# rust-bio/rust-bio

Measured on NVIDIA H100. Metric: GCUPS, higher is better.
Workload: dtype int32

## Files before the change

### rust_bio_b200/csrc/b2a_common.cuh

```cuda
#pragma once
#include <stddef.h>
#include <stdint.h>

#if defined(__CUDACC__)
#define B2A_HD __host__ __device__ __forceinline__
#else
#define B2A_HD inline
struct int4 { int x, y, z, w; };
struct int2 { int x, y; };
struct uint4 { unsigned x, y, z, w; };
inline int4 make_int4(int x, int y, int z, int w) { return int4{x, y, z, w}; }
inline int2 make_int2(int x, int y) { return int2{x, y}; }
#endif

namespace b2a {

#if defined(B2A_HOST_WARP) && !defined(__CUDACC__)
struct HostWarp {
  long long x[32];
  void (*next_lane)(void*);
  void* harness;
  void (*other_warp)(void*);
};
inline HostWarp* host_warp = nullptr;
inline int host_lane = 0;
inline void host_warp_sync() { host_warp->next_lane(host_warp->harness); }
inline void host_spin_yield() {
  if (host_warp && host_warp->other_warp) host_warp->other_warp(host_warp->harness);
}
template <class Pick>
inline long long host_warp_exchange(long long mine, Pick pick) {
  host_warp->x[host_lane] = mine;
  host_warp_sync();
  const long long r = pick(host_warp->x);
  host_warp_sync();
  return r;
}
#endif

constexpr int32_t MIN_SCORE = -858993459;
constexpr int32_t DEAD_CLIP = MIN_SCORE / 2;

enum : uint32_t {
  TB_START = 0, TB_INS = 1, TB_DEL = 2, TB_SUBST = 3, TB_MATCH = 4,
  TB_XCLIP_PREFIX = 5, TB_XCLIP_SUFFIX = 6, TB_YCLIP_PREFIX = 7, TB_YCLIP_SUFFIX = 8
};

enum : uint32_t { NB_DIAG = 3, NB_INS = 2, NB_DEL = 1, NB_CLIP = 0, NB_IEXT = 4, NB_DEXT = 8 };

enum : int {
  F_TRACK_ROWS = 1,
  F_TRACK_COLS = 2,
  F_CLIPX = 4,
  F_LUT = 8,
  F_PACKTRK = 16,
  F_RELU = 32,
  F_PACKREL = 128,
  F_BND8 = 256,
  F_NOTB = 512,
  F_YSTREAM = 1024,
};
#ifndef B2A_KREL_BITS
#define B2A_KREL_BITS 12
#endif
constexpr int32_t KREL_BITS = B2A_KREL_BITS, KREL_MASK = (1 << KREL_BITS) - 1;

struct DevScoring {
  int32_t gap_open, gap_extend;
  int32_t xclip_prefix, xclip_suffix, yclip_prefix, yclip_suffix;
  int32_t match_score, mismatch_score;
  int32_t alpha;
};

struct Block {
  uint32_t first;
  uint32_t npairs;
  uint32_t maxm, maxn;
  uint32_t uniform;
  uint32_t nstrips;
  uint32_t xwords;
  uint32_t ywords;
  uint32_t K;
  uint32_t rows_pad;
  uint64_t seq_off;
  uint64_t bnd_off;
  uint64_t rows_off;
  uint64_t rowm_off;
  uint64_t tb_off;
  uint64_t ops_off;
  uint64_t strip_task_base;
};

enum { ROWS_SN = 0, ROWS_LY = 1, ROWS_SL = 2, ROWS_IL = 3, ROWS_NL = 4, ROWS_ARRAYS = 5 };

B2A_HD int64_t rows_index(int arr, int32_t rows_pad, int32_t slot) {
  return (int64_t)(arr * rows_pad) * 32 + slot;
}

B2A_HD int32_t imax(int32_t a, int32_t b) { return a > b ? a : b; }


B2A_HD int32_t col0_I(const DevScoring& sc, int32_t i) {
  if (i == 1) return sc.gap_open;
  return imax(sc.gap_open + sc.gap_extend * (i - 1), sc.xclip_prefix + sc.gap_open);
}
B2A_HD uint32_t col0_ibits(const DevScoring& sc, int32_t i) {
  if (i == 1) return TB_START;
  return (sc.gap_open + sc.gap_extend * (i - 1) > sc.xclip_prefix + sc.gap_open) ? TB_INS
                                                                                   : TB_XCLIP_PREFIX;
}
B2A_HD int32_t col0_S(const DevScoring& sc, int32_t i) {
  return imax(col0_I(sc, i), sc.xclip_prefix);
}
B2A_HD uint32_t col0_sbits(const DevScoring& sc, int32_t i) {
  return sc.xclip_prefix > col0_I(sc, i) ? TB_XCLIP_PREFIX : TB_INS;
}
B2A_HD int32_t row0_D(const DevScoring& sc, int32_t j) {
  if (j == 1) return sc.gap_open;
  return imax(sc.gap_open + sc.gap_extend * (j - 1), sc.yclip_prefix + sc.gap_open);
}
B2A_HD uint32_t row0_dbits(const DevScoring& sc, int32_t j) {
  if (j == 1) return TB_START;
  return (sc.gap_open + sc.gap_extend * (j - 1) > sc.yclip_prefix + sc.gap_open) ? TB_DEL
                                                                                   : TB_YCLIP_PREFIX;
}
B2A_HD int32_t row0_S(const DevScoring& sc, int32_t j, int32_t n) {
  int32_t s = imax(row0_D(sc, j), sc.yclip_prefix);
  if (j == n && sc.yclip_suffix > s) s = sc.yclip_suffix;
  return s;
}
B2A_HD uint32_t row0_sbits(const DevScoring& sc, int32_t j, int32_t n) {
  if (j == 0) return TB_START;
  const int32_t d = row0_D(sc, j);
  uint32_t b = d > sc.yclip_prefix ? TB_DEL : TB_YCLIP_PREFIX;
  if (j == n && sc.yclip_suffix > imax(d, sc.yclip_prefix)) b = TB_YCLIP_SUFFIX;
  return b;
}
B2A_HD int32_t xclip_score(const DevScoring& sc, int32_t j) {
  return sc.xclip_prefix + imax(sc.yclip_prefix, sc.gap_open + sc.gap_extend * (j - 1));
}

B2A_HD int64_t bnd_index(int32_t G, int32_t j, int32_t pi, int32_t maxn) {
  return G < 32 ? (int64_t)j * 32 + pi : (int64_t)pi * (maxn + 1) + j;
}

B2A_HD int32_t pack_s16x2(int32_t lo, int32_t hi) {
#if defined(__CUDA_ARCH__)
  return (int32_t)__byte_perm((uint32_t)lo, (uint32_t)hi, 0x5410);
#else
  return (int32_t)(((uint32_t)hi << 16) | ((uint32_t)lo & 0xffffu));
#endif
}
B2A_HD int32_t lo_s16(int32_t w) { return (int32_t)(int16_t)(uint16_t)((uint32_t)w & 0xffffu); }
B2A_HD int32_t hi_s16(int32_t w) { return w >> 16; }

#if defined(__CUDACC__)
__host__ __device__
#endif
constexpr int lut_entries(int alpha) { return (alpha + 1) * alpha; }
#if defined(__CUDACC__)
__host__ __device__
#endif
constexpr uint32_t lut_smem_bytes(int alpha) { return ((uint32_t)lut_entries(alpha) * 4u + 127u) & ~127u; }
constexpr int32_t LUT_POISON = 2;

#ifndef B2A_W_8_20
#define B2A_W_8_20 4
#endif
#if defined(__CUDACC__)
__host__ __device__
#endif
constexpr int fill_warps_of(int G, int R) { return (G == 8 && R == 20) ? B2A_W_8_20 : 4; }
#if defined(__CUDACC__)
__host__ __device__
#endif
constexpr bool cap_dispatch_of(int G) { return G == 8; }

#if defined(__CUDACC__)
__host__ __device__
#endif
constexpr int tbw_of(int R) { return (R + 3) / 4; }

}
```

### rust_bio_b200/csrc/b2a_engine.cu

```cuda
#include <cuda_runtime.h>

#include <chrono>
#include <cstdio>
#include <cstdlib>
#include <cstring>
#include <cub/device/device_scan.cuh>
#include <string>
#include <vector>

#define B2A_DEFINE_WALK_KERNEL
#include "../../include/b200align.h"
#include "b2a_fill_launch.h"
#include "b2a_kernels.cuh"
#include "b2a_plan.h"
#include "b2a_walk.cuh"
#include "b2a_banded.cuh"
#include "b2a_banded_strip.cuh"

using namespace b2a;

namespace {

struct DevBuf {
  void* p = nullptr;
  size_t cap = 0;
  cudaError_t reserve(size_t n) {
    if (n <= cap) return cudaSuccess;
    if (p) cudaFree(p);
    p = nullptr;
    cap = 0;
    size_t want = n + n / 8 + 256;
    cudaError_t e = cudaMalloc(&p, want);
    if (e != cudaSuccess) {
      want = n;
      e = cudaMalloc(&p, want);
    }
    if (e == cudaSuccess) cap = want;
    return e;
  }
  void release() {
    if (p) cudaFree(p);
    p = nullptr;
    cap = 0;
  }
  template <class T>
  T* as() const {
    return reinterpret_cast<T*>(p);
  }
};

const FillLaunch kFillShapes[] = {
    {1, 16, launch_fill_1_16, launch_fill_notb_1_16},
    {1, 8, launch_fill_1_8, nullptr},
    {1, 20, launch_fill_1_20, nullptr},
    {2, 16, launch_fill_2_16, nullptr},
    {2, 20, launch_fill_2_20, nullptr},
    {4, 16, launch_fill_4_16, nullptr},
    {8, 16, launch_fill_8_16, launch_fill_notb_8_16},
    {8, 20, launch_fill_8_20, launch_fill_notb_8_20},
    {32, 8, launch_fill_32_8, launch_fill_notb_32_8},
    {32, 16, launch_fill_32_16, launch_fill_notb_32_16},
};

const FillLaunch* find_shape(int G, int R) {
  for (const FillLaunch& f : kFillShapes)
    if (f.G == G && f.R == R) return &f;
  return nullptr;
}

constexpr uint32_t kMaxStageSmem = 200 * 1024;
constexpr uint64_t kWarpWalkMaxPairs = 16384;
constexpr int kMaxAlpha = 64;
constexpr int kMaxAlphaTable = 128;

}

struct b2a_engine {
  int device = 0;
  int num_sms = 0;
  cudaStream_t stream = nullptr, own_stream = nullptr;
  cudaStream_t tail_stream = nullptr;
  cudaStream_t aux_stream = nullptr;
  std::vector<cudaEvent_t> sub_ev;
  bool overlap_small = true;
  bool overlap_big = false;
  bool no_packrel = false;
  bool tail_split = true;
  bool split_timing = false;
  cudaEvent_t split_ev[5] = {nullptr, nullptr, nullptr, nullptr, nullptr};
  bool split_ran = false;
  uint32_t walk_cta_warps = 0;
  cudaEvent_t ev_fill = nullptr;
  bool tail_used = false;
  bool is_slot = false;
  bool stage_nosync = false;
  uint32_t fill_task_limit = 0;
  uint8_t* h_plan = nullptr;
  size_t h_plan_cap = 0;
  cudaStream_t res_stream() const { return tail_used ? tail_stream : stream; }
  uint64_t compact_hdr[8] = {~0ull, 0, 0, 0, 0, 0, 0, 0};
  uint64_t band_wave_lo = 0;
  std::vector<uint64_t> band_roff;
  std::vector<uint32_t> band_ylen;
  std::string err;
  int tune_G = 0, tune_R = 0;
  int walk_mode = 0;
  bool banded_fast = true;
  bool banded_strip = true;
  bool banded_strip_lastcol = true;
  uint64_t strip_pairs = 0;
  uint32_t packed_width = 0;
  std::vector<uint64_t> eff_xoff, eff_yoff;
  bool last_walk_warp = false;
  uint64_t tb_budget = 0;

  bool staged = false, ran = false;
  bool score_only = false;
  Plan plan;
  DevScoring sc{};
  int flags = 0, mode = 0;
  const FillLaunch* shape = nullptr;
  uint64_t n_pairs = 0, blob_bytes = 0;
  uint64_t h2d_bytes = 0;
  std::vector<int32_t> lut_host;
  std::vector<uint8_t> last_syms;
  uint8_t codemap_host[256];

  DevBuf d_blob, d_xoff, d_xlen, d_yoff, d_ylen, d_order, d_pm, d_pn, d_blocks, d_seq, d_bnd, d_rows,
      d_rowm, d_tb, d_opsscratch, d_lut, d_codemap, d_ctl, d_score, d_xs, d_xe, d_ys, d_ye, d_nops,
      d_opssrc, d_clip, d_status, d_nops64, d_opsoff, d_opsdense, d_scan, d_records, d_prog, d_bcells, d_bstatus,
      d_bopsend, d_bslab, d_branges, d_broff, d_bfill, d_bfoff, d_hmoff, d_hmxy, d_hpoff, d_hpidx, d_raw, d_gnops,
      d_gnops64, d_goff, d_bcols, d_bstrip, d_bsoff, d_belig;
  uint32_t* h_nops = nullptr;
  uint64_t h_nops_cap = 0;
  cudaEvent_t ev[6] = {nullptr, nullptr, nullptr, nullptr, nullptr, nullptr};
  std::vector<cudaEvent_t> wave_ev;
  uint32_t launches = 0;
  int last_grid = 0;

  int pipe_chunks = 5;
  struct PipeSlot {
    b2a_engine* eng = nullptr;
    uint64_t* h_opsoff = nullptr;
    uint32_t* h_ctl = nullptr;
    size_t h_cap = 0;
    std::vector<uint64_t> xoff, yoff;
    std::vector<uint8_t> packed;
    uint64_t lo = 0, n = 0;
    bool busy = false;
  } slots[3];
  static constexpr int kSlots = 3;

  int fail(int code, const std::string& what) {
    err = what;
    return code;
  }
  int cuda_fail(const char* what, cudaError_t e) {
    err = std::string(what) + ": " + cudaGetErrorString(e);
    return B2A_E_CUDA;
  }
};

#define CK(expr)                                              \
  do {                                                        \
    cudaError_t _e = (expr);                                  \
    if (_e != cudaSuccess) return e->cuda_fail(#expr, _e);    \
  } while (0)

namespace {

inline uint64_t bitenc_blocks(uint64_t len, uint32_t width) {
  const uint64_t usable = 32 - 32 % width;
  return (len * width + usable - 1) / usable;
}

__global__ void __launch_bounds__(128) unpack_bitenc_kernel(const uint32_t* __restrict__ blocks,
                                                             const uint64_t* __restrict__ x_block,
                                                             const uint64_t* __restrict__ y_block,
                                                             const uint64_t* __restrict__ x_off,
                                                             const uint64_t* __restrict__ y_off,
                                                             const uint32_t* __restrict__ x_len,
                                                             const uint32_t* __restrict__ y_len, uint64_t n_pairs,
                                                             uint32_t width, uint8_t* __restrict__ out) {
  const uint32_t usable = 32 - 32 % width, per_block = usable / width, mask = (1u << width) - 1u;
  const uint32_t lane = threadIdx.x & 31u;
  const uint64_t nwarps = ((uint64_t)gridDim.x * blockDim.x) >> 5;
  for (uint64_t t = ((uint64_t)blockIdx.x * blockDim.x + threadIdx.x) >> 5; t < 2 * n_pairs; t += nwarps) {
    const uint64_t p = t >> 1;
    const bool isy = t & 1;
    const uint32_t* src = blocks + (isy ? y_block[p] : x_block[p]);
    uint8_t* dst = out + (isy ? y_off[p] : x_off[p]);
    const uint32_t len = isy ? y_len[p] : x_len[p];
    for (uint32_t i = lane; i < len; i += 32) {
      const uint32_t blk = i / per_block, bit = (i % per_block) * width;
      dst[i] = (uint8_t)((src[blk] >> bit) & mask);
    }
  }
}

void choose_shape(const b2a_engine* e, uint32_t maxm, uint32_t maxn, uint64_t n_pairs, int* G, int* R) {
  if (e->tune_G && e->tune_R) {
    *G = e->tune_G;
    *R = e->tune_R;
    return;
  }
  const uint64_t stage1 = (uint64_t)((maxm + 15) / 16 * 16 + 64 + (maxn + 15) / 16 * 16 + 64) * 32 * fill_warps_of(1, 16);
  if (n_pairs >= 49152 && stage1 <= kMaxStageSmem && maxm <= 2048) {
    *G = 1;
    *R = 16;
  } else if ((n_pairs >= 4096 && maxm <= 4096) || maxm <= 161) {
    const uint64_t rows = maxm > 1 ? maxm - 1 : 1;
    const uint64_t pad16 = (rows + 127) / 128 * 128, pad20 = (rows + 159) / 160 * 160;
    *G = 8;
    *R = pad20 < pad16 ? 20 : 16;
  } else {
    *G = 32;
    const uint64_t rows = maxm > 1 ? maxm - 1 : 1;
    const uint64_t pad16 = (rows + 511) / 512 * 512, pad8 = (rows + 255) / 256 * 256;
    *R = (pad16 * 100 <= pad8 * 112) ? 16 : 8;
  }
}

int validate_scoring(b2a_engine* e, const b2a_scoring* s) {
  if (s->gap_open > 0) return e->fail(B2A_E_INVALID, "gap_open can't be positive");
  if (s->gap_extend > 0) return e->fail(B2A_E_INVALID, "gap_extend can't be positive");
  if (s->xclip_prefix > 0) return e->fail(B2A_E_INVALID, "Clipping penalty (x prefix) can't be positive");
  if (s->xclip_suffix > 0) return e->fail(B2A_E_INVALID, "Clipping penalty (x suffix) can't be positive");
  if (s->yclip_prefix > 0) return e->fail(B2A_E_INVALID, "Clipping penalty (y prefix) can't be positive");
  if (s->yclip_suffix > 0) return e->fail(B2A_E_INVALID, "Clipping penalty (y suffix) can't be positive");
  const int32_t clips[4] = {s->xclip_prefix, s->xclip_suffix, s->yclip_prefix, s->yclip_suffix};
  for (int32_t c : clips)
    if (c < B2A_MIN_SCORE) return e->fail(B2A_E_RANGE, "clip penalty below MIN_SCORE");
  return B2A_OK;
}

}

extern "C" {

const char* b2a_version(void) { return "b200align 0.1 (sm_90a)"; }

const char* b2a_last_error(const b2a_engine* e) { return e ? e->err.c_str() : "null engine"; }

int32_t b2a_engine_create(b2a_engine** out, int32_t device_id) {
  if (!out) return B2A_E_INVALID;
  *out = nullptr;
  int count = 0;
  cudaError_t ce = cudaGetDeviceCount(&count);
  if (ce != cudaSuccess || count <= 0 || device_id < 0 || device_id >= count) return B2A_E_NO_DEVICE;
  if (cudaSetDevice(device_id) != cudaSuccess) return B2A_E_NO_DEVICE;
  cudaDeviceProp prop;
  if (cudaGetDeviceProperties(&prop, device_id) != cudaSuccess) return B2A_E_NO_DEVICE;
  if (prop.major != 9 || prop.minor != 0) return B2A_E_NO_DEVICE;
  b2a_engine* e = new b2a_engine();
  e->device = device_id;
  e->num_sms = prop.multiProcessorCount;
  e->overlap_small = false;
  if (const char* env = getenv("B2A_BANDED_LITERAL")) e->banded_fast = atoi(env) == 0;
  if (const char* env = getenv("B2A_BANDED_STRIP")) e->banded_strip = atoi(env) != 0;
  if (const char* env = getenv("B2A_BANDED_STRIP_LASTCOL")) e->banded_strip_lastcol = atoi(env) != 0;
  if (const char* env = getenv("B2A_OVERLAP")) e->overlap_small = atoi(env) != 0;
  if (const char* env = getenv("B2A_OVERLAP_BIG")) e->overlap_big = atoi(env) != 0;
  if (const char* env = getenv("B2A_TAIL_SPLIT")) e->tail_split = atoi(env) != 0;
  if (const char* env = getenv("B2A_NO_PACKREL")) e->no_packrel = atoi(env) != 0;
  if (const char* env = getenv("B2A_SPLIT_TIMING")) e->split_timing = atoi(env) != 0;
  if (const char* env = getenv("B2A_WALK_CTA_WARPS")) {
    const int v = atoi(env);
    if (v == 1 || v == 2 || v == 4 || v == 8 || v == 16 || v == 32) e->walk_cta_warps = (uint32_t)v;
  }
  if (cudaStreamCreateWithFlags(&e->own_stream, cudaStreamNonBlocking) != cudaSuccess) {
    delete e;
    return B2A_E_CUDA;
  }
  e->stream = e->own_stream;
  for (auto& v : e->ev) cudaEventCreate(&v);
  *out = e;
  return B2A_OK;
}

int32_t b2a_engine_destroy(b2a_engine* e) {
  if (!e) return B2A_OK;
  cudaSetDevice(e->device);
  for (auto& sl : e->slots) {
    if (sl.h_opsoff) cudaFreeHost(sl.h_opsoff);
    if (sl.h_ctl) cudaFreeHost(sl.h_ctl);
    if (sl.eng) b2a_engine_destroy(sl.eng);
    sl.eng = nullptr;
  }
  cudaStreamSynchronize(e->stream);
  if (e->tail_stream) {
    cudaStreamSynchronize(e->tail_stream);
    cudaStreamDestroy(e->tail_stream);
  }
  if (e->ev_fill) cudaEventDestroy(e->ev_fill);
  if (e->aux_stream) {
    cudaStreamSynchronize(e->aux_stream);
    cudaStreamDestroy(e->aux_stream);
  }
  for (auto& v : e->sub_ev) cudaEventDestroy(v);
  if (e->h_plan) cudaFreeHost(e->h_plan);
  if (e->h_nops) cudaFreeHost(e->h_nops);
  DevBuf* bufs[] = {&e->d_blob, &e->d_xoff, &e->d_xlen, &e->d_yoff, &e->d_ylen, &e->d_order, &e->d_pm,
                    &e->d_pn, &e->d_blocks, &e->d_seq, &e->d_bnd, &e->d_rows, &e->d_rowm, &e->d_tb,
                    &e->d_opsscratch, &e->d_lut, &e->d_codemap, &e->d_ctl, &e->d_score, &e->d_xs,
                    &e->d_xe, &e->d_ys, &e->d_ye, &e->d_nops, &e->d_opssrc, &e->d_clip, &e->d_status,
                    &e->d_nops64, &e->d_opsoff, &e->d_opsdense, &e->d_scan, &e->d_records, &e->d_prog, &e->d_bcells,
                    &e->d_bstatus, &e->d_bopsend, &e->d_bslab, &e->d_branges, &e->d_broff, &e->d_bfill, &e->d_hmoff, &e->d_hmxy,
                    &e->d_hpoff, &e->d_hpidx, &e->d_raw, &e->d_gnops, &e->d_gnops64, &e->d_goff,
                    &e->d_bfoff, &e->d_bcols, &e->d_bstrip, &e->d_bsoff, &e->d_belig};
  for (DevBuf* b : bufs) b->release();
  for (auto& v : e->ev)
    if (v) cudaEventDestroy(v);
  for (auto& v : e->wave_ev) cudaEventDestroy(v);
  if (e->own_stream) cudaStreamDestroy(e->own_stream);
  delete e;
  return B2A_OK;
}

int32_t b2a_engine_set_stream(b2a_engine* e, void* cuda_stream) {
  if (!e) return B2A_E_INVALID;
  e->stream = cuda_stream ? reinterpret_cast<cudaStream_t>(cuda_stream) : e->own_stream;
  return B2A_OK;
}

int32_t b2a_engine_set_traceback_budget(b2a_engine* e, uint64_t bytes) {
  if (!e) return B2A_E_INVALID;
  e->tb_budget = bytes;
  return B2A_OK;
}

int32_t b2a_engine_set_pipeline(b2a_engine* e, int32_t chunks) {
  if (!e) return B2A_E_INVALID;
  e->pipe_chunks = chunks < 2 ? 0 : (chunks > 64 ? 64 : chunks);
  return B2A_OK;
}

int32_t b2a_engine_last_alphabet(const b2a_engine* e, uint8_t* symbols, uint32_t* n_symbols) {
  if (!e || !symbols || !n_symbols) return B2A_E_INVALID;
  *n_symbols = (uint32_t)e->last_syms.size();
  for (size_t k = 0; k < e->last_syms.size() && k < 256; ++k) symbols[k] = e->last_syms[k];
  return B2A_OK;
}

int32_t b2a_engine_set_walk(b2a_engine* e, int32_t mode) {
  if (!e) return B2A_E_INVALID;
  if (mode < 0 || mode > 2) return e->fail(B2A_E_INVALID, "walk mode must be 0 (automatic), 1 (lane per pair) or 2 (warp per pair)");
  e->walk_mode = mode;
  return B2A_OK;
}

int32_t b2a_engine_set_tuning(b2a_engine* e, int32_t G, int32_t R) {
  if (!e) return B2A_E_INVALID;
  if (G == 0 && R == 0) {
    e->tune_G = e->tune_R = 0;
    return B2A_OK;
  }
  if (!find_shape(G, R)) return e->fail(B2A_E_INVALID, "fill shape (G,R) not built into this library");
  e->tune_G = G;
  e->tune_R = R;
  return B2A_OK;
}

}

static int32_t stage_front(b2a_engine* e, int32_t mode, const b2a_scoring* s, const b2a_pairs* pairs,
                           uint32_t& maxm, uint32_t& maxn, int64_t& score_bound) {
  if (!e || !s || !pairs) return B2A_E_INVALID;
  e->staged = e->ran = false;
  e->score_only = false;
  if (mode < 0 || mode > 3) return e->fail(B2A_E_INVALID, "mode must be B2A_MODE_*");
  int rc = validate_scoring(e, s);
  if (rc) return rc;
  if (cudaSetDevice(e->device) != cudaSuccess) return e->fail(B2A_E_NO_DEVICE, "cudaSetDevice failed");
  if (e->stage_nosync) {
    if (cudaStreamSynchronize(e->stream) != cudaSuccess) return e->fail(B2A_E_CUDA, "cudaStreamSynchronize failed");
  }
  const uint64_t n = pairs->n_pairs;
  if (n > 0x7ffffffeull) return e->fail(B2A_E_INVALID, "more than 2^31 - 2 pairs in one batch");
  e->n_pairs = n;
  e->mode = mode;

  DevScoring sc{};
  sc.gap_open = s->gap_open;
  sc.gap_extend = s->gap_extend;
  sc.xclip_prefix = s->xclip_prefix;
  sc.xclip_suffix = s->xclip_suffix;
  sc.yclip_prefix = s->yclip_prefix;
  sc.yclip_suffix = s->yclip_suffix;
  if (mode == B2A_MODE_GLOBAL) sc.xclip_prefix = sc.xclip_suffix = sc.yclip_prefix = sc.yclip_suffix = MIN_SCORE;
  if (mode == B2A_MODE_SEMIGLOBAL) {
    sc.xclip_prefix = sc.xclip_suffix = MIN_SCORE;
    sc.yclip_prefix = sc.yclip_suffix = 0;
  }
  if (mode == B2A_MODE_LOCAL) sc.xclip_prefix = sc.xclip_suffix = sc.yclip_prefix = sc.yclip_suffix = 0;
  sc.match_score = s->match_score;
  sc.mismatch_score = s->mismatch_score;
  sc.alpha = 0;

  maxm = 0;
  maxn = 0;
  const uint32_t pw = e->packed_width;
  const uint64_t unit_total = pw ? pairs->blob_bytes / 4 : pairs->blob_bytes;
  for (uint64_t p = 0; p < n; ++p) {
    const uint64_t bb = unit_total, xo = pairs->x_off[p], yo = pairs->y_off[p];
    const uint64_t xu = pw ? bitenc_blocks(pairs->x_len[p], pw) : pairs->x_len[p];
    const uint64_t yu = pw ? bitenc_blocks(pairs->y_len[p], pw) : pairs->y_len[p];
    if (xo > bb || xu > bb - xo || yo > bb || yu > bb - yo)
      return e->fail(B2A_E_INVALID, "sequence offset/length outside seq_blob");
    maxm = std::max(maxm, pairs->x_len[p]);
    maxn = std::max(maxn, pairs->y_len[p]);
  }
  if (maxm > (1u << 24) || maxn > (1u << 24)) return e->fail(B2A_E_RANGE, "sequence longer than 2^24");

  cudaStream_t st = e->stream;
  e->blob_bytes = pairs->blob_bytes;
  e->h2d_bytes = 0;
  auto up = [&](DevBuf& bf, const void* src, size_t bytes) -> cudaError_t {
    e->h2d_bytes += bytes;
    return bytes ? cudaMemcpyAsync(bf.p, src, bytes, cudaMemcpyHostToDevice, st) : cudaSuccess;
  };
  CK(e->d_ctl.reserve(2048));
  bool present[256] = {false};
  if (pw) {
    e->eff_xoff.resize(n);
    e->eff_yoff.resize(n);
    uint64_t pos = 0;
    for (uint64_t p = 0; p < n; ++p) {
      e->eff_xoff[p] = pos;
      pos += ((uint64_t)pairs->x_len[p] + 15) & ~15ull;
      e->eff_yoff[p] = pos;
      pos += ((uint64_t)pairs->y_len[p] + 15) & ~15ull;
    }
    e->blob_bytes = pos;
    CK(e->d_raw.reserve(pairs->blob_bytes + 16));
    CK(e->d_blob.reserve(pos + 16));
    CK(e->d_xoff.reserve(n * 8 + 8));
    CK(e->d_yoff.reserve(n * 8 + 8));
    CK(e->d_xlen.reserve(n * 4 + 4));
    CK(e->d_ylen.reserve(n * 4 + 4));
    CK(e->d_opssrc.reserve(n * 8 + 8));
    CK(e->d_nops64.reserve((n + 1) * 8));
    CK(up(e->d_raw, pairs->seq_blob, pairs->blob_bytes));
    CK(up(e->d_opssrc, pairs->x_off, n * 8));
    CK(up(e->d_nops64, pairs->y_off, n * 8));
    CK(up(e->d_xoff, e->eff_xoff.data(), n * 8));
    CK(up(e->d_yoff, e->eff_yoff.data(), n * 8));
    CK(up(e->d_xlen, pairs->x_len, n * 4));
    CK(up(e->d_ylen, pairs->y_len, n * 4));
    if (n) {
      unpack_bitenc_kernel<<<(unsigned)std::min<uint64_t>((2 * n + 3) / 4, 1u << 20), 128, 0, st>>>(
          e->d_raw.as<uint32_t>(), e->d_opssrc.as<uint64_t>(), e->d_nops64.as<uint64_t>(), e->d_xoff.as<uint64_t>(),
          e->d_yoff.as<uint64_t>(), e->d_xlen.as<uint32_t>(), e->d_ylen.as<uint32_t>(), n, pw, e->d_blob.as<uint8_t>());
      CK(cudaGetLastError());
    }
    CK(cudaStreamSynchronize(st));
    if (!(s->alphabet && s->alphabet_len))
      for (uint32_t k = 0; k < (1u << pw); ++k) present[k] = true;
  } else {
    CK(e->d_blob.reserve(pairs->blob_bytes + 16));
    CK(up(e->d_blob, pairs->seq_blob, pairs->blob_bytes));
  }
  if (s->alphabet && s->alphabet_len) {
    for (uint32_t k = 0; k < s->alphabet_len; ++k) present[s->alphabet[k]] = true;
  } else if (!pw) {
    uint32_t* flags = e->d_ctl.as<uint32_t>() + 256;
    CK(cudaMemsetAsync(flags, 0, 1024, st));
    if (pairs->blob_bytes) {
      symbols_kernel<<<e->num_sms * 8, 256, 0, st>>>(e->d_blob.as<uint8_t>(), pairs->blob_bytes, flags);
      CK(cudaGetLastError());
    }
    uint32_t hflags[256];
    CK(cudaMemcpyAsync(hflags, flags, 1024, cudaMemcpyDeviceToHost, st));
    CK(cudaStreamSynchronize(st));
    for (int k = 0; k < 256; ++k) present[k] = hflags[k] != 0;
  }
  std::vector<int> syms;
  for (int k = 0; k < 256; ++k)
    if (present[k]) syms.push_back(k);
  if (syms.empty()) syms.push_back(0);
  e->last_syms.assign(syms.begin(), syms.end());
  int64_t maxabs = std::max<int64_t>(std::llabs((long long)s->match_score), std::llabs((long long)s->mismatch_score));
  for (int k = 0; k < 256; ++k) e->codemap_host[k] = (uint8_t)k;
  e->lut_host.clear();
  if (s->table && (int)syms.size() > kMaxAlphaTable)
    return e->fail(B2A_E_UNSUPPORTED, "MatchFunc table over more than 128 distinct symbols");
  if ((int)syms.size() <= (s->table ? kMaxAlphaTable : kMaxAlpha)) {
    sc.alpha = (int32_t)syms.size();
    for (int k = 0; k < 256; ++k) e->codemap_host[k] = 0xFF;
    for (int a = 0; a < sc.alpha; ++a) e->codemap_host[syms[a]] = (uint8_t)a;
    const size_t aa = (size_t)sc.alpha * sc.alpha;
    e->lut_host.resize(aa + (size_t)lut_entries(sc.alpha));
    if (s->table) maxabs = 0;
    for (int a = 0; a < sc.alpha; ++a)
      for (int b = 0; b < sc.alpha; ++b) {
        const int32_t v = s->table ? s->table[syms[a] * 256 + syms[b]]
                                   : (a == b ? s->match_score : s->mismatch_score);
        e->lut_host[(size_t)a * sc.alpha + b] = v;
        maxabs = std::max<int64_t>(maxabs, std::llabs((long long)v));
      }
    if (maxabs > (1ll << 27)) return e->fail(B2A_E_RANGE, "substitution score magnitude above 2^27");
    for (size_t k = 0; k < aa; ++k) e->lut_host[aa + k] = 4 * e->lut_host[k] + 3 - (4 * sc.gap_open + 1);
    for (size_t k = aa; k < (size_t)lut_entries(sc.alpha); ++k) e->lut_host[aa + k] = LUT_POISON;
  }
  score_bound = 0;
  {
    const int64_t unit = std::max<int64_t>(maxabs, std::max<int64_t>(-(int64_t)sc.gap_open, -(int64_t)sc.gap_extend));
    const int64_t bound = ((int64_t)maxm + maxn + 2) * unit - (int64_t)sc.gap_open;
    score_bound = bound;
    if (bound > (1ll << 27)) return e->fail(B2A_E_RANGE, "scores x lengths exceed the i32-safe range (2^27)");
    const int32_t clips[4] = {sc.xclip_prefix, sc.xclip_suffix, sc.yclip_prefix, sc.yclip_suffix};
    for (int32_t c : clips)
      if (c > DEAD_CLIP && -(int64_t)c > (1ll << 27))
        return e->fail(B2A_E_RANGE, "clip penalty between -2^27 and MIN_SCORE/2 is not supported");
  }
  e->sc = sc;
  e->flags = scoring_flags(sc, score_bound, maxm, maxn);
  if (e->no_packrel) e->flags &= ~F_PACKREL;
  if (boundary8_ok(e->flags, score_bound)) e->flags |= F_BND8;

  return B2A_OK;
}

static int32_t compact_ops(b2a_engine* e, uint64_t scratch_bytes, cudaStream_t st) {
  const uint64_t n = e->n_pairs;
  if (n) {
    if (n <= 65536) {
      scan_small_kernel<<<1, 1024, 0, st>>>(e->d_nops.as<uint32_t>(), e->d_opsoff.as<uint64_t>(), (uint32_t)n);
      CK(cudaGetLastError());
    } else {
    const unsigned g1 = (unsigned)((n + 1 + 255) / 256);
    widen_kernel<<<g1, 256, 0, st>>>(e->d_nops.as<uint32_t>(), e->d_nops64.as<uint64_t>(), n);
    CK(cudaGetLastError());
    size_t tmp = 0;
    CK(cub::DeviceScan::ExclusiveSum(nullptr, tmp, e->d_nops64.as<uint64_t>(), e->d_opsoff.as<uint64_t>(),
                                     (int64_t)(n + 1), st));
    CK(e->d_scan.reserve(tmp + 16));
    CK(cub::DeviceScan::ExclusiveSum(e->d_scan.p, tmp, e->d_nops64.as<uint64_t>(),
                                     e->d_opsoff.as<uint64_t>(), (int64_t)(n + 1), st));
    }
    CK(e->d_opsdense.reserve(scratch_bytes + 16));
    const unsigned g2 = (unsigned)((n * 32 + 255) / 256);
    gather_ops_kernel<<<g2, 256, 0, st>>>(e->d_opsscratch.as<uint8_t>(), e->d_opssrc.as<uint64_t>(),
                                          e->d_opsoff.as<uint64_t>(), e->d_opsdense.as<uint8_t>(), n);
    CK(cudaGetLastError());
    e->launches += n <= 65536 ? 2 : 4;
  }
  return B2A_OK;
}

extern "C" {

static int32_t batch_stage_impl(b2a_engine* e, int32_t mode, const b2a_scoring* s, const b2a_pairs* pairs,
                                bool score_only) {
  if (!e || !s || !pairs) return B2A_E_INVALID;
  uint32_t maxm = 0, maxn = 0;
  int64_t score_bound = 0;
  int rc = stage_front(e, mode, s, pairs, maxm, maxn, score_bound);
  if (rc) return rc;
  if (score_only) e->flags |= F_NOTB;
  const uint64_t n = e->n_pairs;
  const DevScoring sc = e->sc;
  cudaStream_t st = e->stream;
  auto up = [&](DevBuf& bf, const void* src, size_t bytes) -> cudaError_t {
    e->h2d_bytes += bytes;
    return bytes ? cudaMemcpyAsync(bf.p, src, bytes, cudaMemcpyHostToDevice, st) : cudaSuccess;
  };
  int G = 1, R = 16;
  choose_shape(e, maxm, maxn, n, &G, &R);
  uint64_t budget = e->tb_budget;
  if (!budget) {
    size_t fr = 0, tot = 0;
    CK(cudaMemGetInfo(&fr, &tot));
    budget = (uint64_t)((double)fr * 0.6);
  }
  const uint32_t lut_bytes = sc.alpha ? lut_smem_bytes(sc.alpha) : 0u;
  for (int attempt = 0;; ++attempt) {
    e->shape = find_shape(G, R);
    if (!e->shape) return e->fail(B2A_E_INVALID, "no fill kernel for the requested shape");
    build_plan(e->plan, pairs->x_len, pairs->y_len, n, G, R, budget, e->flags);
    if (64 + lut_bytes + (uint64_t)fill_warps_of(G, R) * e->plan.smem_seq_bytes <= kMaxStageSmem) break;
    if (G == 32) {
      e->flags |= F_YSTREAM;
      e->plan.smem_seq_bytes = (uint32_t)(G * R);
      break;
    }
    if ((e->tune_G && e->tune_R) || attempt > 0)
      return e->fail(B2A_E_UNSUPPORTED, "sequences too long for on-chip staging with this fill shape");
    G = 32;
    const uint64_t rows = maxm > 1 ? maxm - 1 : 1;
    const uint64_t pad16 = (rows + 511) / 512 * 512, pad8 = (rows + 255) / 256 * 256;
    R = (pad16 * 100 <= pad8 * 112) ? 16 : 8;
  }
  if (score_only && !e->shape->launch_notb)
    return e->fail(B2A_E_UNSUPPORTED, "score-only batches run only the fill shapes the automatic choice picks (1x16, 8x16, "
                                      "8x20, 32x8, 32x16); the forced shape has no score-only fill kernel");
  const Plan& pl = e->plan;
  if (!score_only && pl.G == 32 && pl.max_tb > budget)
    return e->fail(B2A_E_UNSUPPORTED, "a pair's traceback needs " + std::to_string(pl.max_tb) +
                                          " bytes, above the traceback budget of " + std::to_string(budget) +
                                          " bytes; the score-only calls (b2a_align_batch_scores, b2a_batch_stage_scores) "
                                          "align it without a traceback");

  CK(e->d_xoff.reserve(n * 8 + 8));
  CK(e->d_yoff.reserve(n * 8 + 8));
  CK(e->d_xlen.reserve(n * 4 + 4));
  CK(e->d_ylen.reserve(n * 4 + 4));
  CK(e->d_order.reserve(n * 4 + 4));
  CK(e->d_pm.reserve(n * 4 + 4));
  CK(e->d_pn.reserve(n * 4 + 4));
  CK(e->d_blocks.reserve(pl.blocks.size() * sizeof(Block) + 8));
  CK(e->d_seq.reserve(pl.seq_bytes + 16));
  CK(e->d_bnd.reserve(pl.max_bnd + 16));
  CK(e->d_rows.reserve(pl.max_rows + 16));
  CK(e->d_rowm.reserve(pl.max_rowm + 16));
  CK(e->d_tb.reserve(pl.max_tb + 16));
  CK(e->d_prog.reserve(pl.max_strip_tasks * 4 + 16));
  CK(e->d_opsscratch.reserve(pl.ops_bytes + 16));
  CK(e->d_lut.reserve(e->lut_host.size() * 4 + 16));
  CK(e->d_codemap.reserve(256));
  CK(e->d_score.reserve(n * 4 + 4));
  CK(e->d_xs.reserve(n * 4 + 4));
  CK(e->d_xe.reserve(n * 4 + 4));
  CK(e->d_ys.reserve(n * 4 + 4));
  CK(e->d_ye.reserve(n * 4 + 4));
  CK(e->d_nops.reserve(n * 4 + 4));
  CK(e->d_opssrc.reserve(n * 8 + 8));
  CK(e->d_clip.reserve(n * 16 + 16));
  CK(e->d_status.reserve(n * 4 + 4));
  CK(e->d_nops64.reserve((n + 1) * 8));
  CK(e->d_opsoff.reserve((n + 1) * 8));

  if (!e->packed_width) {
    CK(up(e->d_xoff, pairs->x_off, n * 8));
    CK(up(e->d_yoff, pairs->y_off, n * 8));
    CK(up(e->d_xlen, pairs->x_len, n * 4));
    CK(up(e->d_ylen, pairs->y_len, n * 4));
  }
  {
    const size_t blocks_bytes = pl.blocks.size() * sizeof(Block), lut_b = e->lut_host.size() * 4;
    const size_t need = 3 * n * 4 + blocks_bytes + 256 + lut_b + 64;
    if (e->h_plan_cap < need) {
      if (e->h_plan) cudaFreeHost(e->h_plan);
      e->h_plan = nullptr;
      e->h_plan_cap = 0;
      CK(cudaMallocHost(&e->h_plan, need + need / 4));
      e->h_plan_cap = need + need / 4;
    }
    size_t pos = 0;
    auto up_staged = [&](DevBuf& bf, const void* src, size_t bytes) -> cudaError_t {
      if (!bytes) return cudaSuccess;
      std::memcpy(e->h_plan + pos, src, bytes);
      const cudaError_t ce = up(bf, e->h_plan + pos, bytes);
      pos += (bytes + 15) & ~(size_t)15;
      return ce;
    };
    CK(up_staged(e->d_order, pl.order.data(), n * 4));
    CK(up_staged(e->d_pm, pl.pm.data(), n * 4));
    CK(up_staged(e->d_pn, pl.pn.data(), n * 4));
    CK(up_staged(e->d_blocks, pl.blocks.data(), blocks_bytes));
    CK(up_staged(e->d_codemap, e->codemap_host, 256));
    if (lut_b) CK(up_staged(e->d_lut, e->lut_host.data(), lut_b));
  }
  if (!e->stage_nosync) CK(cudaStreamSynchronize(st));
  e->score_only = score_only;
  e->staged = true;
  return B2A_OK;
}

int32_t b2a_batch_stage(b2a_engine* e, int32_t mode, const b2a_scoring* s, const b2a_pairs* pairs) {
  return batch_stage_impl(e, mode, s, pairs, false);
}

int32_t b2a_batch_stage_scores(b2a_engine* e, int32_t mode, const b2a_scoring* s, const b2a_pairs* pairs) {
  return batch_stage_impl(e, mode, s, pairs, true);
}

int32_t b2a_batch_run(b2a_engine* e) {
  if (!e) return B2A_E_INVALID;
  if (!e->staged) return e->fail(B2A_E_STATE, "b2a_batch_run before b2a_batch_stage");
  if (cudaSetDevice(e->device) != cudaSuccess) return e->fail(B2A_E_NO_DEVICE, "cudaSetDevice failed");
  const Plan& pl = e->plan;
  cudaStream_t st = e->stream;
  const FillLaunchFn fill = e->score_only ? e->shape->launch_notb : e->shape->launch;
  void (*const walk_warp_k)(const WalkParams) = e->score_only ? walk_warp_kernel<true> : walk_warp_kernel<false>;
  void (*const walk_lane_k)(const WalkParams) = e->score_only ? walk_kernel<true> : walk_kernel<false>;
  const bool use_tail = e->is_slot && e->tail_stream != nullptr && pl.waves.size() == 1;
  e->tail_used = use_tail;
  e->launches = 0;
  uint32_t* ctl = e->d_ctl.as<uint32_t>();
  CK(cudaMemsetAsync(ctl, 0, 256, st));
  CK(cudaEventRecord(e->ev[0], st));
  if (!pl.blocks.empty()) {
    PackParams pk{};
    pk.blocks = e->d_blocks.as<Block>();
    pk.order = e->d_order.as<uint32_t>();
    pk.blob = e->d_blob.as<uint8_t>();
    pk.x_off = e->d_xoff.as<uint64_t>();
    pk.x_len = e->d_xlen.as<uint32_t>();
    pk.y_off = e->d_yoff.as<uint64_t>();
    pk.y_len = e->d_ylen.as<uint32_t>();
    pk.codemap = e->d_codemap.as<uint8_t>();
    pk.seq = e->d_seq.as<uint8_t>();
    pk.bad_symbol = ctl;
    pk.G = pl.G;
    pack_kernel<<<(unsigned)pl.blocks.size(), 256, 0, st>>>(pk);
    CK(cudaGetLastError());
    ++e->launches;
  }
  CK(cudaEventRecord(e->ev[1], st));
  size_t wi = 0;
  for (const Wave& w : pl.waves) {
    const uint32_t nb = w.block_hi - w.block_lo;
    if (wi >= 60) return e->fail(B2A_E_UNSUPPORTED, "more than 60 traceback waves; raise the budget");
    FillParams fp{};
    fp.blocks = e->d_blocks.as<Block>() + w.block_lo;
    fp.nblocks = nb;
    fp.pm = e->d_pm.as<uint32_t>();
    fp.pn = e->d_pn.as<uint32_t>();
    fp.seq = e->d_seq.as<uint8_t>();
    fp.bnd = e->d_bnd.as<uint8_t>();
    fp.rows = e->d_rows.as<uint8_t>();
    fp.tb = e->score_only ? nullptr : e->d_tb.as<uint8_t>();
    fp.lut = e->d_lut.as<int32_t>() + (size_t)e->sc.alpha * e->sc.alpha;
    fp.task_counter = ctl + 2 + wi;
    fp.smem_seq_bytes = pl.smem_seq_bytes;
    fp.one = 1;
    fp.ge4 = 4 * e->sc.gap_extend;
    uint32_t fill_tasks = nb * (uint32_t)pl.G;
    if (pl.G == 32 && w.strip_tasks >= 0x7fffffffull) return e->fail(B2A_E_RANGE, "too many strip tasks in one wave");
    if (pl.G == 32 && w.strip_tasks > 0) {
      fp.progress = e->d_prog.as<uint32_t>();
      fp.n_strip_tasks = (uint32_t)w.strip_tasks;
      fill_tasks = fp.n_strip_tasks;
      CK(cudaMemsetAsync(fp.progress, 0, (size_t)w.strip_tasks * 4, st));
    }
    fp.sc = e->sc;
    while (e->wave_ev.size() < 3 * (wi + 1)) {
      cudaEvent_t v;
      CK(cudaEventCreate(&v));
      e->wave_ev.push_back(v);
    }
    WalkParams wp{};
    wp.blocks = fp.blocks;
    wp.nblocks = nb;
    wp.pm = fp.pm;
    wp.pn = fp.pn;
    wp.order = e->d_order.as<uint32_t>();
    wp.seq = fp.seq;
    wp.bnd = fp.bnd;
    wp.rows = fp.rows;
    wp.rowm = e->d_rowm.as<uint8_t>();
    wp.tb = fp.tb;
    wp.ops_scratch = e->d_opsscratch.as<uint8_t>();
    wp.lut = e->d_lut.as<int32_t>();
    wp.sc = e->sc;
    wp.G = pl.G;
    wp.R = pl.R;
    wp.packtrk = (e->flags & F_PACKTRK) ? 1 : 0;
    wp.bnd8 = (e->flags & F_BND8) ? 1 : 0;
    wp.filter_clips = (e->mode == B2A_MODE_SEMIGLOBAL || e->mode == B2A_MODE_LOCAL) ? 1 : 0;
    wp.score = e->d_score.as<int32_t>();
    wp.xstart = e->d_xs.as<uint32_t>();
    wp.xend = e->d_xe.as<uint32_t>();
    wp.ystart = e->d_ys.as<uint32_t>();
    wp.yend = e->d_ye.as<uint32_t>();
    wp.n_ops = e->d_nops.as<uint32_t>();
    wp.ops_src = e->d_opssrc.as<uint64_t>();
    wp.clip_len = e->d_clip.as<uint32_t>();
    wp.status = e->d_status.as<uint32_t>();
    wp.err_flag = ctl + 1;
    const bool fuse = false;
    fp.task_limit = (pl.G == 32) ? 0u : e->fill_task_limit;
    const uint64_t wave_pairs = (uint64_t)nb * 32;
    const bool warp_walk = e->walk_mode == 2 || (e->walk_mode == 0 && wave_pairs <= kWarpWalkMaxPairs);
    uint32_t per_warp_smem = 0;
    uint32_t wcta_warps = e->walk_cta_warps;
    if (warp_walk) {
      const uint32_t per_warp = ((pl.maxm + 3) / 4 + (pl.maxn + 3) / 4) * 4 + 16;
      if (!wcta_warps) wcta_warps = (uint64_t)per_warp * 8 <= 96 * 1024 ? 8u : 4u;
      per_warp_smem = (uint64_t)per_warp * wcta_warps <= 96 * 1024 ? per_warp : 0u;
      if ((size_t)per_warp_smem * wcta_warps > 48 * 1024)
        CK(cudaFuncSetAttribute(walk_warp_k, cudaFuncAttributeMaxDynamicSharedMemorySize, (int)(per_warp_smem * wcta_warps)));
    }
    if (!wcta_warps) wcta_warps = 4;
    wp.seq_smem_per_warp = per_warp_smem;
    const bool overlap_big = e->overlap_big && pl.waves.size() == 1 && !warp_walk && pl.G != 32 && nb >= 4096 && !use_tail;
    const bool overlap = overlap_big || (e->overlap_small && pl.waves.size() == 1 && warp_walk && pl.G != 32 && nb >= 64 &&
                                         !use_tail && e->walk_mode != 1);
    uint32_t split_b = 0;
    if (e->tail_split && !overlap && pl.waves.size() == 1 && warp_walk && pl.G != 32 && !use_tail && e->walk_mode != 1 &&
        fp.task_limit == 0) {
      int resident = 0;
      CK(fill(e->flags, fp, fill_tasks, e->num_sms, st, &resident, 1));
      const uint32_t slots = (uint32_t)resident, tasks = fill_tasks;
      if (slots > 0 && tasks > slots) {
        const uint32_t rounds = tasks / slots, rem = tasks % slots;
        const uint32_t a_blocks = (uint32_t)((uint64_t)rounds * slots / (uint32_t)pl.G);
        if (rem > 0 && rounds <= 6 && rem * 4 <= slots && a_blocks > 0 && a_blocks < nb) split_b = a_blocks;
      }
    }
    if (split_b) {
      if (!e->tail_stream) {
        int lo_pri = 0, hi_pri = 0;
        cudaDeviceGetStreamPriorityRange(&lo_pri, &hi_pri);
        CK(cudaStreamCreateWithPriority(&e->tail_stream, cudaStreamNonBlocking, hi_pri));
        CK(cudaEventCreateWithFlags(&e->ev_fill, cudaEventDisableTiming));
      }
      if (!e->aux_stream) CK(cudaStreamCreateWithFlags(&e->aux_stream, cudaStreamNonBlocking));
      while (e->sub_ev.size() < 6) {
        cudaEvent_t v;
        CK(cudaEventCreateWithFlags(&v, cudaEventDisableTiming));
        e->sub_ev.push_back(v);
      }
      CK(cudaEventRecord(e->wave_ev[3 * wi + 0], st));
      FillParams fa = fp, fb = fp;
      fa.nblocks = split_b;
      fb.blocks = fp.blocks + split_b;
      fb.nblocks = nb - split_b;
      fb.task_counter = ctl + 8;
      WalkParams wa = wp, wb = wp;
      wa.nblocks = split_b;
      wb.blocks = wp.blocks + split_b;
      wb.nblocks = nb - split_b;
      if (e->split_timing && !e->split_ev[0])
        for (auto& v : e->split_ev) CK(cudaEventCreate(&v));
      if (e->split_timing) CK(cudaEventRecord(e->split_ev[0], st));
      CK(fill(e->flags, fa, fa.nblocks * (uint32_t)pl.G, e->num_sms, st, &e->last_grid, 0));
      if (e->split_timing) CK(cudaEventRecord(e->split_ev[1], st));
      CK(cudaEventRecord(e->sub_ev[0], st));
      cudaStream_t sB = e->tail_stream, sA = e->aux_stream;
      CK(cudaStreamWaitEvent(sB, e->sub_ev[0], 0));
      CK(cudaStreamWaitEvent(sA, e->sub_ev[0], 0));
      CK(fill(e->flags, fb, fb.nblocks * (uint32_t)pl.G, e->num_sms, sB, nullptr, 0));
      CK(cudaEventRecord(e->wave_ev[3 * wi + 1], sB));
      if (e->split_timing) CK(cudaEventRecord(e->split_ev[2], sB));
      walk_warp_k<<<wa.nblocks * 32 / wcta_warps, wcta_warps * 32, (size_t)per_warp_smem * wcta_warps, sA>>>(wa);
      CK(cudaGetLastError());
      if (e->split_timing) CK(cudaEventRecord(e->split_ev[3], sA));
      walk_warp_k<<<wb.nblocks * 32 / wcta_warps, wcta_warps * 32, (size_t)per_warp_smem * wcta_warps, sB>>>(wb);
      CK(cudaGetLastError());
      if (e->split_timing) CK(cudaEventRecord(e->split_ev[4], sB));
      e->split_ran = true;
      e->launches += 4;
      CK(cudaEventRecord(e->sub_ev[1], e->aux_stream));
      CK(cudaEventRecord(e->sub_ev[2], e->tail_stream));
      CK(cudaStreamWaitEvent(st, e->sub_ev[1], 0));
      CK(cudaStreamWaitEvent(st, e->sub_ev[2], 0));
      e->last_walk_warp = true;
      CK(cudaEventRecord(e->wave_ev[3 * wi + 2], st));
      ++wi;
      continue;
    }
    if (overlap) {
      constexpr int kSub = 4;
      if (!e->tail_stream) {
        int lo_pri = 0, hi_pri = 0;
        cudaDeviceGetStreamPriorityRange(&lo_pri, &hi_pri);
        CK(cudaStreamCreateWithPriority(&e->tail_stream, cudaStreamNonBlocking, hi_pri));
        CK(cudaEventCreateWithFlags(&e->ev_fill, cudaEventDisableTiming));
      }
      if (!e->aux_stream) CK(cudaStreamCreateWithFlags(&e->aux_stream, cudaStreamNonBlocking));
      while (e->sub_ev.size() < kSub + 2) {
        cudaEvent_t v;
        CK(cudaEventCreateWithFlags(&v, cudaEventDisableTiming));
        e->sub_ev.push_back(v);
      }
      CK(cudaEventRecord(e->wave_ev[3 * wi + 0], st));
      CK(cudaEventRecord(e->sub_ev[kSub], st));
      CK(cudaStreamWaitEvent(e->aux_stream, e->sub_ev[kSub], 0));
      CK(cudaStreamWaitEvent(e->tail_stream, e->sub_ev[kSub], 0));
      for (int sidx = 0; sidx < kSub; ++sidx) {
        const uint32_t lo_b = (uint32_t)((uint64_t)nb * sidx / kSub), hi_b = (uint32_t)((uint64_t)nb * (sidx + 1) / kSub);
        if (hi_b <= lo_b) continue;
        cudaStream_t fs = (sidx & 1) ? e->aux_stream : st;
        FillParams f2 = fp;
        f2.blocks = fp.blocks + lo_b;
        f2.nblocks = hi_b - lo_b;
        f2.task_counter = ctl + 8 + sidx;
        f2.task_limit = 1;
        CK(fill(e->flags, f2, f2.nblocks * (uint32_t)pl.G, e->num_sms, fs, &e->last_grid, 0));
        ++e->launches;
        CK(cudaEventRecord(e->sub_ev[sidx], fs));
        CK(cudaStreamWaitEvent(e->tail_stream, e->sub_ev[sidx], 0));
        if (sidx == kSub - 1) CK(cudaEventRecord(e->wave_ev[3 * wi + 1], e->tail_stream));
        WalkParams w2 = wp;
        w2.blocks = wp.blocks + lo_b;
        w2.nblocks = hi_b - lo_b;
        if (warp_walk) walk_warp_k<<<w2.nblocks * 32 / wcta_warps, wcta_warps * 32, (size_t)per_warp_smem * wcta_warps, e->tail_stream>>>(w2);
        else walk_lane_k<<<(w2.nblocks * 32 + 127) / 128, 128, 0, e->tail_stream>>>(w2);
        CK(cudaGetLastError());
        ++e->launches;
      }
      CK(cudaEventRecord(e->sub_ev[kSub + 1], e->tail_stream));
      CK(cudaStreamWaitEvent(st, e->sub_ev[kSub + 1], 0));
      e->last_walk_warp = warp_walk;
      CK(cudaEventRecord(e->wave_ev[3 * wi + 2], st));
      ++wi;
      continue;
    }
    CK(cudaEventRecord(e->wave_ev[3 * wi + 0], st));
    CK(fill(e->flags, fp, fill_tasks, e->num_sms, st, &e->last_grid, 0));
    ++e->launches;
    CK(cudaEventRecord(e->wave_ev[3 * wi + 1], st));
    if (use_tail) {
      CK(cudaEventRecord(e->ev_fill, st));
      CK(cudaStreamWaitEvent(e->tail_stream, e->ev_fill, 0));
      st = e->tail_stream;
    }
    if (!fuse) {
      if (warp_walk) {
        walk_warp_k<<<nb * 32 / wcta_warps, wcta_warps * 32, (size_t)per_warp_smem * wcta_warps, st>>>(wp);
      } else {
        const unsigned wgrid = (nb * 32 + 127) / 128;
        walk_lane_k<<<wgrid, 128, 0, st>>>(wp);
      }
      CK(cudaGetLastError());
      ++e->launches;
      e->last_walk_warp = warp_walk;
    }
    CK(cudaEventRecord(e->wave_ev[3 * wi + 2], st));
    ++wi;
  }
  CK(cudaEventRecord(e->ev[4], st));
  if (!e->score_only) {
    int rc2 = compact_ops(e, pl.ops_bytes, st);
    if (rc2) return rc2;
  }
  CK(cudaEventRecord(e->ev[5], st));
  e->ran = true;
  return B2A_OK;
}

int32_t b2a_batch_fetch(b2a_engine* e, b2a_results* r, b2a_stats* stats) {
  if (!e) return B2A_E_INVALID;
  if (!e->ran) return e->fail(B2A_E_STATE, "b2a_batch_fetch before b2a_batch_run");
  if (e->score_only && r && (r->xstart || r->ystart || r->ops || r->ops_off || r->clip_len))
    return e->fail(B2A_E_INVALID, "a score-only batch has only score, xend, yend and status: xstart, ystart, ops, "
                                  "ops_off and clip_len must be NULL");
  if (cudaSetDevice(e->device) != cudaSuccess) return e->fail(B2A_E_NO_DEVICE, "cudaSetDevice failed");
  cudaStream_t st = e->res_stream();
  const uint64_t n = e->n_pairs;
  uint64_t d2h = 0;
  uint32_t ctl[2] = {0, 0};
  CK(cudaMemcpyAsync(ctl, e->d_ctl.p, 8, cudaMemcpyDeviceToHost, st));
  if (r && n) {
    auto down = [&](void* dst, const DevBuf& b, size_t bytes) -> cudaError_t {
      if (!dst || !bytes) return cudaSuccess;
      d2h += bytes;
      return cudaMemcpyAsync(dst, b.p, bytes, cudaMemcpyDeviceToHost, st);
    };
    CK(down(r->score, e->d_score, n * 4));
    CK(down(r->xstart, e->d_xs, n * 4));
    CK(down(r->xend, e->d_xe, n * 4));
    CK(down(r->ystart, e->d_ys, n * 4));
    CK(down(r->yend, e->d_ye, n * 4));
    CK(down(r->clip_len, e->d_clip, n * 16));
    CK(down(r->status, e->d_status, n * 4));
    uint64_t total = 0;
    if (e->score_only) {
    } else if (r->ops_off) {
      CK(down(r->ops_off, e->d_opsoff, (n + 1) * 8));
      CK(cudaStreamSynchronize(st));
      total = r->ops_off[n];
    } else {
      CK(cudaMemcpyAsync(&total, e->d_opsoff.as<uint64_t>() + n, 8, cudaMemcpyDeviceToHost, st));
      CK(cudaStreamSynchronize(st));
    }
    if (r->ops) {
      if (total > r->ops_capacity) return e->fail(B2A_E_CAPACITY, "ops buffer too small for this batch");
      CK(down(r->ops, e->d_opsdense, total));
    }
  }
  CK(cudaStreamSynchronize(st));
  if (ctl[0]) return e->fail(B2A_E_INVALID, "a sequence byte is outside the scoring alphabet");
  if (ctl[1] & 4u) return e->fail(B2A_E_INVALID, "a sequence byte is outside the scoring alphabet");
  if (!(r && r->status)) {
    if (ctl[1] & 2u) return e->fail(B2A_E_CAPACITY, "banded: more k-mer matches than the per-pair capacity");
    if (ctl[1] & 8u)
      return e->fail(B2A_E_INVALID, "banded: the reference panics on these caller-supplied matches/path (not strictly ascending, index out of range, or outside the matrix)");
    if (ctl[1]) return e->fail(B2A_E_RANGE, "traceback walk met an impossible move or never terminates (the reference panics / hangs here: mod.rs:905, banded.rs:777-831)");
  }
  if (e->split_timing && e->split_ran) {
    float a = 0, b = 0, c = 0, d = 0;
    cudaEventElapsedTime(&a, e->split_ev[0], e->split_ev[1]);
    cudaEventElapsedTime(&b, e->split_ev[1], e->split_ev[2]);
    cudaEventElapsedTime(&c, e->split_ev[1], e->split_ev[3]);
    cudaEventElapsedTime(&d, e->split_ev[1], e->split_ev[4]);
    fprintf(stderr, "[split] fill A %.1f us; after it: fill B done +%.1f, walk A done +%.1f, walk B done +%.1f us\n", a * 1e3,
            b * 1e3, c * 1e3, d * 1e3);
    e->split_ran = false;
  }
  if (stats) {
    std::memset(stats, 0, sizeof(*stats));
    stats->cells = e->plan.cells;
    stats->h2d_bytes = e->h2d_bytes;
    stats->d2h_bytes = d2h;
    stats->traceback_bytes = e->plan.total_tb;
    cudaEventElapsedTime(&stats->pack_ms, e->ev[0], e->ev[1]);
    for (size_t wv = 0; wv < e->plan.waves.size(); ++wv) {
      float a = 0.f, b = 0.f;
      cudaEventElapsedTime(&a, e->wave_ev[3 * wv + 0], e->wave_ev[3 * wv + 1]);
      cudaEventElapsedTime(&b, e->wave_ev[3 * wv + 1], e->wave_ev[3 * wv + 2]);
      stats->fill_ms += a;
      stats->walk_ms += b;
    }
    float tail = 0.f;
    cudaEventElapsedTime(&tail, e->ev[4], e->ev[5]);
    stats->walk_ms += tail;
    stats->kernel_launches = e->launches;
    stats->waves = (uint32_t)e->plan.waves.size();
    stats->fill_lanes_per_pair = (uint32_t)e->plan.G;
    stats->fill_rows_per_lane = (uint32_t)e->plan.R;
  }
  return B2A_OK;
}

static void collect_stats(b2a_engine* e, b2a_stats* stats) {
  stats->cells += e->plan.cells;
  stats->h2d_bytes += e->h2d_bytes;
  stats->traceback_bytes += e->plan.total_tb;
  float v = 0.f;
  cudaEventElapsedTime(&v, e->ev[0], e->ev[1]);
  stats->pack_ms += v;
  for (size_t wv = 0; wv < e->plan.waves.size(); ++wv) {
    float a = 0.f, b = 0.f;
    cudaEventElapsedTime(&a, e->wave_ev[3 * wv + 0], e->wave_ev[3 * wv + 1]);
    cudaEventElapsedTime(&b, e->wave_ev[3 * wv + 1], e->wave_ev[3 * wv + 2]);
    stats->fill_ms += a;
    stats->walk_ms += b;
  }
  cudaEventElapsedTime(&v, e->ev[4], e->ev[5]);
  stats->walk_ms += v;
  stats->kernel_launches += e->launches;
  stats->waves += (uint32_t)e->plan.waves.size();
  stats->fill_lanes_per_pair = (uint32_t)e->plan.G;
  stats->fill_rows_per_lane = (uint32_t)e->plan.R;
}

static int32_t slot_finish(b2a_engine* e, b2a_engine::PipeSlot& sl, b2a_results* r, uint64_t& base,
                           b2a_stats* agg) {
  b2a_engine* c = sl.eng;
  sl.busy = false;
  cudaError_t ce = cudaStreamSynchronize(c->res_stream());
  if (ce != cudaSuccess) return e->cuda_fail("pipeline: cudaStreamSynchronize", ce);
  if (sl.h_ctl[0]) return e->fail(B2A_E_INVALID, "a sequence byte is outside the scoring alphabet");
  if (sl.h_ctl[1] && !r->status) return e->fail(B2A_E_RANGE, "traceback walk met an impossible move (reference panics at mod.rs:905)");
  const uint64_t total = sl.h_opsoff[sl.n];
  if (r->ops) {
    if (base + total > r->ops_capacity) return e->fail(B2A_E_CAPACITY, "ops buffer too small for this batch");
    if (total) {
      ce = cudaMemcpyAsync(r->ops + base, c->d_opsdense.p, total, cudaMemcpyDeviceToHost, c->res_stream());
      if (ce != cudaSuccess) return e->cuda_fail("pipeline: ops D2H", ce);
      agg->d2h_bytes += total;
    }
  }
  if (r->ops_off)
    for (uint64_t i = 0; i < sl.n; ++i) r->ops_off[sl.lo + i] = base + sl.h_opsoff[i];
  base += total;
  ce = cudaStreamSynchronize(c->res_stream());
  if (ce != cudaSuccess) return e->cuda_fail("pipeline: cudaStreamSynchronize", ce);
  collect_stats(c, agg);
  return B2A_OK;
}

static int32_t align_batch_pipelined(b2a_engine* e, int32_t mode, const b2a_scoring* scoring,
                                     const b2a_pairs* pairs, b2a_results* r, b2a_stats* stats) {
  const uint64_t n = pairs->n_pairs;
  uint64_t K = (uint64_t)e->pipe_chunks;
  std::vector<double> wts(K, 6.0);
  wts[0] = 1.0;
  if (K >= 3) wts[1] = 3.0;
  wts[K - 1] = K >= 4 ? 3.0 : 2.0;
  if (K == 5) wts = {1.0, 3.0, 5.0, 5.0, 5.0};
  if (const char* env = getenv("B2A_PIPE_WEIGHTS")) {
    std::vector<double> w2;
    for (const char* q = env; *q;) {
      char* end = nullptr;
      const double v = strtod(q, &end);
      if (end == q) break;
      if (v > 0) w2.push_back(v);
      q = *end ? end + 1 : end;
    }
    if (w2.size() >= 2) {
      wts = w2;
      K = wts.size();
    }
  }
  std::vector<uint64_t> cut(K + 1, 0);
  {
    double tot = 0, acc = 0;
    for (double w : wts) tot += w;
    for (uint64_t c = 0; c < K; ++c) {
      acc += wts[c] / tot * (double)n;
      cut[c + 1] = std::min<uint64_t>(n, ((uint64_t)acc + 31) / 32 * 32);
    }
    cut[K] = n;
  }
  b2a_stats agg;
  std::memset(&agg, 0, sizeof(agg));
  uint64_t base = 0;
  int32_t rc = B2A_OK;
  std::vector<uint8_t> inferred;
  const bool dbg = getenv("B2A_DEBUG_TIMING") != nullptr;
  auto now = []() { return std::chrono::duration<double, std::milli>(std::chrono::steady_clock::now().time_since_epoch()).count(); };
  const double t00 = now();
  for (uint64_t c = 0; c < K && rc == B2A_OK; ++c) {
    const double tc0 = now();
    if (cut[c + 1] <= cut[c]) continue;
    const uint64_t lo = cut[c], hi = cut[c + 1], nc = hi - lo;
    b2a_engine::PipeSlot& sl = e->slots[c % b2a_engine::kSlots];
    if (sl.busy) {
      rc = slot_finish(e, sl, r, base, &agg);
      if (rc) break;
    }
    if (!sl.eng) {
      rc = b2a_engine_create(&sl.eng, e->device);
      if (rc) {
        e->fail(rc, "pipeline: cannot create a slot engine");
        break;
      }
    }
    if (!sl.eng->tail_stream) {
      int lo_pri = 0, hi_pri = 0;
      cudaDeviceGetStreamPriorityRange(&lo_pri, &hi_pri);
      if (cudaStreamCreateWithPriority(&sl.eng->tail_stream, cudaStreamNonBlocking, hi_pri) != cudaSuccess ||
          cudaEventCreateWithFlags(&sl.eng->ev_fill, cudaEventDisableTiming) != cudaSuccess) {
        rc = e->fail(B2A_E_CUDA, "pipeline: cannot create the slot's tail stream");
        break;
      }
    }
    sl.eng->is_slot = true;
    sl.eng->stage_nosync = true;
    sl.eng->fill_task_limit = 1;
    sl.eng->packed_width = e->packed_width;
    sl.eng->tune_G = e->tune_G;
    sl.eng->tune_R = e->tune_R;
    sl.eng->walk_mode = e->walk_mode;
    sl.eng->tb_budget = e->tb_budget;
    sl.eng->pipe_chunks = 0;
    if (sl.h_cap < nc + 1) {
      if (sl.h_opsoff) cudaFreeHost(sl.h_opsoff);
      sl.h_opsoff = nullptr;
      if (cudaMallocHost(&sl.h_opsoff, (nc + 1) * 8) != cudaSuccess) {
        rc = e->fail(B2A_E_CUDA, "pipeline: cudaMallocHost failed");
        break;
      }
      sl.h_cap = nc + 1;
    }
    if (!sl.h_ctl && cudaMallocHost(&sl.h_ctl, 64) != cudaSuccess) {
      rc = e->fail(B2A_E_CUDA, "pipeline: cudaMallocHost failed");
      break;
    }
    const uint32_t pw = e->packed_width;
    const uint64_t unit = pw ? 4 : 1;
    uint64_t bmin = ~0ull, bmax = 0, seq_sum = 0;
    bool inside = true;
    for (uint64_t p = lo; p < hi; ++p) {
      const uint64_t bb = pairs->blob_bytes / unit, xo = pairs->x_off[p], yo = pairs->y_off[p];
      const uint64_t xu = pw ? bitenc_blocks(pairs->x_len[p], pw) : pairs->x_len[p];
      const uint64_t yu = pw ? bitenc_blocks(pairs->y_len[p], pw) : pairs->y_len[p];
      if (xo > bb || xu > bb - xo || yo > bb || yu > bb - yo) {
        inside = false;
        break;
      }
      bmin = std::min(bmin, std::min(xo, yo));
      bmax = std::max(bmax, std::max(xo + xu, yo + yu));
      seq_sum += xu + yu;
    }
    if (!inside) {
      rc = e->fail(B2A_E_INVALID, "sequence offset/length outside seq_blob");
      break;
    }
    if (bmin > bmax) bmin = bmax = 0;
    sl.xoff.resize(nc);
    sl.yoff.resize(nc);
    const uint8_t* chunk_blob = pairs->seq_blob + bmin * unit;
    uint64_t chunk_bytes = (bmax - bmin) * unit;
    if (!pw && chunk_bytes > 2 * seq_sum + (1ull << 20)) {
      uint64_t pos = 0;
      sl.packed.resize(seq_sum + 32 * nc + 16);
      for (uint64_t i = 0; i < nc; ++i) {
        sl.xoff[i] = pos;
        std::memcpy(sl.packed.data() + pos, pairs->seq_blob + pairs->x_off[lo + i], pairs->x_len[lo + i]);
        pos += ((uint64_t)pairs->x_len[lo + i] + 15) & ~15ull;
        sl.yoff[i] = pos;
        std::memcpy(sl.packed.data() + pos, pairs->seq_blob + pairs->y_off[lo + i], pairs->y_len[lo + i]);
        pos += ((uint64_t)pairs->y_len[lo + i] + 15) & ~15ull;
      }
      chunk_blob = sl.packed.data();
      chunk_bytes = pos;
// ... 833 lines not shown
```

### rust_bio_b200/csrc/b2a_fill.cuh

```cuda
#pragma once
#include "b2a_common.cuh"

namespace b2a {

struct FillParams {
  const Block* blocks;
  uint32_t nblocks;
  const uint32_t* pm;
  const uint32_t* pn;
  const uint8_t* seq;
  uint8_t* bnd;
  uint8_t* rows;
  uint8_t* tb;
  const int32_t* lut;
  uint32_t* task_counter;
  uint32_t smem_seq_bytes;
  int32_t one;
  int32_t ge4;
  uint32_t* progress;
  uint32_t n_strip_tasks;
  uint32_t task_limit;
  DevScoring sc;
};

template <int G>
struct LaneCtx {
  DevScoring sc;
  const int32_t* lut;
  const uint32_t* xs;
  const uint32_t* ys;
  int32_t m, n;
  int32_t maxn;
  int32_t maxm;
  int32_t g;
  int32_t l;
  int32_t lane;
  int32_t pi;
  int32_t nstrips;
  int32_t K;
  int32_t rows_pad;
  bool uniform;
  int4* bnd;
  int32_t* rows;
  uint4* tb;
  uint32_t lut_base;
  uint32_t* prog_mine;
  uint32_t* prog_prev;
  int32_t only_strip;
  int32_t one;
  int32_t ge4;
};

#if defined(__CUDA_ARCH__)
#define B2A_SHFL_UP(v, G) __shfl_up_sync(0xffffffffu, (v), 1, (G))
#elif defined(B2A_HOST_WARP) && !defined(__CUDACC__)
inline int32_t host_shfl_up_group(int32_t v, int G) {
  if (!host_warp) return v;
  const int me = host_lane;
  return (int32_t)host_warp_exchange(v, [&](const long long* x) { return (me % G) ? x[me - 1] : x[me]; });
}
#define B2A_SHFL_UP(v, G) host_shfl_up_group((v), (G))
#define B2A_SPIN_YIELD() host_spin_yield()
#else
#define B2A_SHFL_UP(v, G) (v)
#endif
#ifndef B2A_SPIN_YIELD
#define B2A_SPIN_YIELD() ((void)0)
#endif

constexpr int32_t NEG4 = -(1 << 30);

B2A_HD int32_t max3(int32_t a, int32_t b, int32_t c) {
#if defined(__CUDA_ARCH__)
  return __vimax3_s32(a, b, c);
#else
  return imax(a, imax(b, c));
#endif
}
B2A_HD int32_t max3_relu(int32_t a, int32_t b, int32_t c) {
#if defined(__CUDA_ARCH__)
  return __vimax3_s32_relu(a, b, c);
#else
  return imax(imax(a, imax(b, c)), 0);
#endif
}
B2A_HD int32_t imin(int32_t a, int32_t b) { return a < b ? a : b; }
B2A_HD int32_t addmax(int32_t a, int32_t b, int32_t c) {
#if defined(__CUDA_ARCH__)
  return __viaddmax_s32(a, b, c);
#else
  return imax(a + b, c);
#endif
}
B2A_HD int32_t addmin(int32_t a, int32_t b, int32_t c) {
#if defined(__CUDA_ARCH__)
  return __viaddmin_s32(a, b, c);
#else
  return imin(a + b, c);
#endif
}
B2A_HD int32_t scale4(int32_t v) { return v <= DEAD_CLIP ? NEG4 : 4 * v; }

B2A_HD int32_t fmad(int32_t a, int32_t k, int32_t b) {
#if defined(__CUDA_ARCH__)
  int32_t d;
  asm("mad.lo.s32 %0, %1, %2, %3;" : "=r"(d) : "r"(a), "r"(k), "r"(b));
  return d;
#else
  return a * k + b;
#endif
}
B2A_HD int32_t lut_at(const void* host_base, uint32_t byte_addr) {
#if defined(__CUDA_ARCH__)
  int32_t v;
  asm("ld.shared.s32 %0, [%1];" : "=r"(v) : "r"(byte_addr));
  return v;
#else
  return *reinterpret_cast<const int32_t*>(reinterpret_cast<const char*>(host_base) + byte_addr);
#endif
}

B2A_HD uint32_t ld_progress(const uint32_t* p) {
#if defined(__CUDA_ARCH__)
  return *reinterpret_cast<const volatile uint32_t*>(p);
#else
  return *p;
#endif
}
template <class T>
B2A_HD T ld_boundary(const T* p, bool bypass_l1) {
#if defined(__CUDA_ARCH__)
  return bypass_l1 ? __ldcg(p) : *p;
#else
  (void)bypass_l1;
  return *p;
#endif
}
template <int G>
B2A_HD auto rows_at(int arr, int32_t rows_pad, int32_t slot) {
  if constexpr (G == 32) return rows_index(arr, rows_pad, slot);
  else return arr * rows_pad * 32 + slot;
}
#ifndef B2A_HOST_YREAD
#define B2A_HOST_YREAD(c, w) ((void)0)
#endif
template <int G>
B2A_HD uint32_t ld_yword(const LaneCtx<G>& c, int32_t w) {
  B2A_HOST_YREAD(c, w);
#if defined(__CUDA_ARCH__)
  return __ldg(c.ys + w);
#else
  return c.ys[w];
#endif
}
B2A_HD void fence_device() {
#if defined(__CUDA_ARCH__)
  __threadfence();
#endif
}

constexpr int32_t KEY_NONE = (int32_t)0x80000000;

template <int G, int R, int FLAGS, bool MASKED, bool LAST, int CAPQ>
B2A_HD void column_step(const LaneCtx<G>& c, const int32_t j, const int32_t tstep, const int32_t q, const int32_t rowbase,
                        const int32_t rv, int32_t (&Sp)[R], int32_t (&Dp)[R], int32_t (&SnR)[R],
                        int32_t (&LyR)[R], uint32_t (&tbacc)[R], const int32_t (&xc)[R],
                        int32_t sdiag, int32_t& sup, int32_t& iup, int32_t& Tv, int32_t& Ti,
                        int32_t& cap_s, int32_t& cap_i) {
  constexpr bool TR = (FLAGS & F_TRACK_ROWS) != 0;
  constexpr bool TC = (FLAGS & F_TRACK_COLS) != 0;
  constexpr bool CX = (FLAGS & F_CLIPX) != 0;
  constexpr bool LUT = (FLAGS & F_LUT) != 0;
  constexpr bool PR = (FLAGS & F_PACKREL) != 0;
  constexpr bool PK = (FLAGS & F_PACKTRK) != 0 || PR;
  constexpr bool RELU = (FLAGS & F_RELU) != 0;
  constexpr bool NOTB = (FLAGS & F_NOTB) != 0;
  constexpr bool TMASK = MASKED && !LUT;
  const int32_t go4i = 4 * c.sc.gap_open + 2, go4d = 4 * c.sc.gap_open + 1, ge4 = c.ge4;
  const int32_t ma4 = 4 * c.sc.match_score + 3 - go4d, mi4 = 4 * c.sc.mismatch_score + 3 - go4d;
  const int32_t x4 = CX ? scale4(xclip_score(c.sc, j)) : 0;
  const int32_t xs4 = scale4(c.sc.xclip_suffix), ys4 = scale4(c.sc.yclip_suffix);
  const int32_t cj = 4095 - (PR ? (tstep & KREL_MASK) : j);
  const int32_t one = c.one, k2 = one + one, k16 = k2 * 8, k1024 = k16 * 64;
  const int32_t q4 = q * 4;
  const uint32_t capbit = (MASKED && rv >= 1) ? 1u << (rv - 1) : 0u;
  int32_t Tl = KEY_NONE;
  int32_t key_even = KEY_NONE;
  int32_t sdo = fmad(sdiag, one, go4d);
  int32_t iop = fmad(sup, one, go4i);
  int32_t s4 = sup;
#pragma unroll
  for (int r = 0; r < R; ++r) {
    int32_t sub4;
    if (LUT) {
      sub4 = lut_at(c.lut, (uint32_t)fmad(q4, one, xc[r]));
    } else {
      sub4 = (xc[r] == q) ? ma4 : mi4;
    }
    const int32_t m4 = fmad(sdo, one, sub4);
    const int32_t i4 = addmax(iup, ge4, iop);
    const int32_t dop = Sp[r];
    const int32_t d4 = addmax(Dp[r], ge4, dop);
    int32_t sP;
    if (CX && RELU) {
      sP = max3_relu(m4, i4, d4);
    } else {
      sP = max3(m4, i4, d4);
      if (CX) sP = imax(sP, x4);
    }
    s4 = sP & ~3;
    const int32_t fi = addmin(i4, -iop, 4), fd = addmin(d4, -dop, 4);
    const int32_t nib = fmad(fd, k2, fi) + sP - s4;
    if (!NOTB) tbacc[r] = (uint32_t)(fmad((int32_t)tbacc[r], k16, fmad(fd, k2, fi)) + sP - s4);
    if (TC) {
      if (PK) {
        if (TMASK) {
          if (r < rv) Tl = imax(Tl, fmad(s4, k1024, 4095 - r));
        } else {
          const int32_t key = fmad(s4, k1024, 4095 - r);
          if (r & 1) Tl = max3(Tl, key_even, key);
          else key_even = key;
        }
      } else {
        const int32_t v = s4 + xs4;
        if ((!TMASK || r < rv) && v > Tv) {
          Tv = v;
          Ti = rowbase + 1 + r;
        }
      }
    }
    if (TR) {
      if (PK) {
        SnR[r] = imax(SnR[r], fmad(s4, k1024, cj));
      } else {
        const int32_t v = s4 + ys4;
        if (v > SnR[r]) {
          SnR[r] = v;
          LyR[r] = j;
        }
      }
    }
    if (LAST) {
      const int32_t slot = (rowbase + 1 + r) * 32 + c.pi;
      c.rows[rows_at<G>(ROWS_SL, c.rows_pad, slot)] = s4 >> 2;
      c.rows[rows_at<G>(ROWS_IL, c.rows_pad, slot)] = i4 >> 2;
      c.rows[rows_at<G>(ROWS_NL, c.rows_pad, slot)] = nib;
    }
    if (MASKED && (CAPQ < 0 || (r >> 2) == CAPQ)) {
      if ((capbit >> r) & 1u) {
        cap_s = s4;
        cap_i = i4;
      }
    }
    sdo = dop;
    Sp[r] = fmad(s4, one, go4d);
    iop = fmad(s4, one, go4i);
    Dp[r] = d4;
    iup = i4;
  }
  sup = s4;
  if (TC && PK) {
    if (Tl != KEY_NONE) Tv = imax(Tv, Tl - ((PR ? c.l * R : rowbase) + 1));
  }
}

template <int G, int R, int FLAGS, bool MASKED, int CAPQ>
B2A_HD void run_strip(const LaneCtx<G>& c, const int32_t s) {
  constexpr bool TR = (FLAGS & F_TRACK_ROWS) != 0;
  constexpr bool TC = (FLAGS & F_TRACK_COLS) != 0;
  constexpr bool LUT = (FLAGS & F_LUT) != 0;
  constexpr bool PR = (FLAGS & F_PACKREL) != 0;
  constexpr bool PK = (FLAGS & F_PACKTRK) != 0 || PR;
  constexpr bool B8 = (FLAGS & F_BND8) != 0;
  constexpr bool NOTB = (FLAGS & F_NOTB) != 0;
  constexpr bool YS = (FLAGS & F_YSTREAM) != 0;
  static_assert(!YS || G == 32, "F_YSTREAM is a warp-per-pair form");
  static_assert(!B8 || ((FLAGS & F_PACKTRK) != 0 && !PR), "F_BND8 needs the packed column tracker with absolute rows");
  constexpr int P = 32 / G;
  constexpr int TBW = tbw_of(R);
  int2* const bnd8 = reinterpret_cast<int2*>(c.bnd);
  const int32_t m = c.m, n = c.n;
  const int32_t rowbase = s * (G * R) + c.l * R;
  int32_t rv = m - 1 - rowbase;
  rv = rv < 0 ? 0 : (rv > R ? R : rv);
  const int32_t ys = c.sc.yclip_suffix;

  int32_t Sp[R], Dp[R], SnR[R], LyR[R], xc[R];
  uint32_t tbacc[R];
#pragma unroll
  for (int w = 0; w < R / 4; ++w) {
    const uint32_t xw = c.xs[(rowbase / 4 + w) * P + c.g];
#pragma unroll
    for (int b = 0; b < 4; ++b) {
      const int32_t sym = (int32_t)((xw >> (8 * b)) & 0xffu);
      xc[w * 4 + b] = LUT ? (int32_t)(c.lut_base + (uint32_t)(sym * c.sc.alpha * 4)) : sym;
      if (MASKED && LUT && w * 4 + b >= rv) xc[w * 4 + b] = (int32_t)(c.lut_base + (uint32_t)(c.sc.alpha * c.sc.alpha * 4));
    }
  }
#pragma unroll
  for (int r = 0; r < R; ++r) {
    const int32_t i = rowbase + 1 + r;
    const int32_t s0 = col0_S(c.sc, i);
    Sp[r] = 4 * s0 + (4 * c.sc.gap_open + 1);
    Dp[r] = NEG4;
    tbacc[r] = 0;
    LyR[r] = 0;
    if (TR) {
      if (PK) {
        SnR[r] = s0 * 4096 + 4095;
      } else {
        const int32_t v = s0 + ys;
        SnR[r] = (ys > DEAD_CLIP && v > MIN_SCORE) ? 4 * v : NEG4;
      }
    } else {
      SnR[r] = 0;
    }
  }
  int32_t sup_prev = rowbase == 0 ? 0 : 4 * col0_S(c.sc, rowbase);
  const int32_t t_none = PK ? KEY_NONE : NEG4;
  int32_t in_s = 0, in_i = NEG4, in_tv = t_none, in_ti = m;
  int32_t up_tv = NEG4, up_ti = m;
  const int32_t xs4_pr = scale4(c.sc.xclip_suffix);
  auto flush_rows = [&](const int32_t chunk, int32_t (&SnRr)[R]) {
#pragma unroll
    for (int r = 0; r < R; ++r) {
      const int32_t slot = (rowbase + 1 + r) * 32 + c.pi;
      if (SnRr[r] != KEY_NONE) {
        const int32_t sn = (SnRr[r] >> 12) + ys;
        const int32_t step = (chunk << KREL_BITS) + (4095 - (SnRr[r] & 4095));
        if (sn > c.rows[rows_at<G>(ROWS_SN, c.rows_pad, slot)]) {
          c.rows[rows_at<G>(ROWS_SN, c.rows_pad, slot)] = sn;
          c.rows[rows_at<G>(ROWS_LY, c.rows_pad, slot)] = step - c.l + 1;
        }
      }
      SnRr[r] = KEY_NONE;
    }
  };
  int4 pre = make_int4(0, 0, 0, 0);
  int2 pre8 = make_int2(0, 0);
  const bool top_from_mem = (c.l == 0) && (s > 0);
  const bool top_from_row0 = (c.l == 0) && (s == 0);
  uint32_t avail = 0;
  const bool piped = c.prog_mine != nullptr;
  auto wait_col = [&](int32_t col) {
    if (piped && c.prog_prev && (int32_t)avail < col) {
      do {
        avail = ld_progress(c.prog_prev);
        B2A_SPIN_YIELD();
      } while ((int32_t)avail < col);
      fence_device();
    }
  };
  const bool top_valid = top_from_mem && rv >= 1;
  if (top_valid && n >= 1) {
    wait_col(1);
    if (B8) pre8 = ld_boundary(&bnd8[bnd_index(G, 1, c.pi, c.maxn)], piped);
    else pre = ld_boundary(&c.bnd[bnd_index(G, 1, c.pi, c.maxn)], piped);
  }
  const bool writer =
      MASKED ? (rv >= 1 && (c.l == G - 1 || rowbase + R >= m - 1)) : (c.l == G - 1);
  int32_t cap_s = 0, cap_i = 0;
  uint32_t yw = 0;
  int32_t nyw = 0;
  uint32_t ynext = 0;
  if constexpr (YS) {
    nyw = (n + 3) >> 2;
    if (nyw > 0) ynext = ld_yword(c, 0);
  }
  uint4* tbs = NOTB ? nullptr : c.tb + (size_t)s * c.K * TBW * 32;
  const int32_t nsteps = c.K * 8;

  if (PR && TR) {
#pragma unroll
    for (int r = 0; r < R; ++r) {
      const int32_t slot = (rowbase + 1 + r) * 32 + c.pi;
      c.rows[rows_at<G>(ROWS_SN, c.rows_pad, slot)] = col0_S(c.sc, rowbase + 1 + r) + ys;
      c.rows[rows_at<G>(ROWS_LY, c.rows_pad, slot)] = 0;
      SnR[r] = KEY_NONE;
    }
  }
  for (int32_t t0 = 0; t0 < nsteps; t0 += (PR ? (1 << KREL_BITS) : nsteps)) {
  const int32_t t1 = PR ? ((t0 + (1 << KREL_BITS) < nsteps) ? t0 + (1 << KREL_BITS) : nsteps) : nsteps;
  for (int32_t t = t0; t < t1; ++t) {
    const int32_t j = t - c.l + 1;
    const bool active = (j >= 1) && (j <= n);
    if (active) {
      int32_t q;
      if (G == 1) {
        if ((t & 3) == 0) yw = c.ys[(t >> 2) * P + c.g];
        q = (int32_t)(yw & 0xffu);
        yw >>= 8;
      } else if (YS) {
        if ((j & 3) == 1) {
          yw = ynext;
          const int32_t wn = ((j - 1) >> 2) + 1;
          if (wn < nyw) ynext = ld_yword(c, wn);
        }
        q = (int32_t)(yw & 0xffu);
        yw >>= 8;
      } else {
        const int32_t jb = j - 1;
        q = (int32_t)((c.ys[(jb >> 2) * P + c.g] >> (8 * (jb & 3))) & 0xffu);
      }
      if (top_from_row0) {
        in_s = 4 * row0_S(c.sc, j, n);
        in_i = NEG4;
        in_tv = t_none;
        in_ti = m;
        if (PR) {
          up_tv = NEG4;
          up_ti = m;
        }
      } else if (top_from_mem) {
        if (B8) {
          in_s = lo_s16(pre8.x);
          in_i = hi_s16(pre8.x);
          if (TC) in_tv = fmad(pre8.y, c.one, 0);
        } else {
          in_s = pre.x;
          in_i = pre.y;
        }
        if (TC && !B8) {
          if (PR) {
            up_tv = pre.z;
            up_ti = pre.w;
            in_tv = KEY_NONE;
          } else {
            in_tv = pre.z;
            in_ti = pre.w;
          }
        }
        if (j < n && top_valid) {
          wait_col(j + 1);
          if (B8) pre8 = ld_boundary(&bnd8[bnd_index(G, j + 1, c.pi, c.maxn)], piped);
          else pre = ld_boundary(&c.bnd[bnd_index(G, j + 1, c.pi, c.maxn)], piped);
        }
      }
      int32_t sup = in_s, iup = in_i, Tv = in_tv, Ti = in_ti;
      if (j == n) {
        column_step<G, R, FLAGS, MASKED, true, CAPQ>(c, j, t, q, rowbase, rv, Sp, Dp, SnR, LyR, tbacc, xc,
                                               sup_prev, sup, iup, Tv, Ti, cap_s, cap_i);
      } else {
        column_step<G, R, FLAGS, MASKED, false, CAPQ>(c, j, t, q, rowbase, rv, Sp, Dp, SnR, LyR, tbacc, xc,
                                                sup_prev, sup, iup, Tv, Ti, cap_s, cap_i);
      }
      sup_prev = in_s;
      if (writer) {
        if (B8) {
          const int32_t s4 = (MASKED && rv < R) ? cap_s : sup, i4 = (MASKED && rv < R) ? cap_i : iup;
          bnd8[bnd_index(G, j, c.pi, c.maxn)] = make_int2(pack_s16x2(s4, i4), TC ? Tv : t_none);
        } else {
          int4 o;
          o.x = (MASKED && rv < R) ? cap_s : sup;
          o.y = (MASKED && rv < R) ? cap_i : iup;
          o.z = TC ? Tv : t_none;
          o.w = TC ? Ti : m;
          if (PR) {
            o.z = NEG4;
            o.w = m;
            if (TC) {
              o.z = up_tv;
              o.w = up_ti;
              if (Tv != KEY_NONE) {
                const int32_t loc_v = ((Tv >> 12) << 2) + xs4_pr;
                if (loc_v > up_tv) {
                  o.z = loc_v;
                  o.w = s * (G * R) + (4095 - (Tv & 4095));
                }
              }
            }
          }
          c.bnd[bnd_index(G, j, c.pi, c.maxn)] = o;
        }
        if (piped && ((j & 15) == 0 || j == n)) {
          fence_device();
          *reinterpret_cast<volatile uint32_t*>(c.prog_mine) = (uint32_t)j;
          B2A_SPIN_YIELD();
        }
      }
      in_s = sup;
      in_i = iup;
      in_tv = Tv;
      in_ti = Ti;
    } else if (!NOTB) {
#pragma unroll
      for (int r = 0; r < R; ++r) tbacc[r] <<= 4;
    }
    if (G > 1) {
      in_s = B2A_SHFL_UP(in_s, G);
      in_i = B2A_SHFL_UP(in_i, G);
      if (TC) {
        in_tv = B2A_SHFL_UP(in_tv, G);
        if (!PK) in_ti = B2A_SHFL_UP(in_ti, G);
        if (PR) {
          up_tv = B2A_SHFL_UP(up_tv, G);
          up_ti = B2A_SHFL_UP(up_ti, G);
        }
      }
    }
    if (!NOTB && (t & 7) == 7) {
      uint4* dst = tbs + (size_t)(t >> 3) * TBW * 32 + c.lane;
#pragma unroll
      for (int qd = 0; qd < TBW; ++qd) {
        uint4 v;
        v.x = tbacc[qd * 4 + 0];
        v.y = (qd * 4 + 1 < R) ? tbacc[qd * 4 + 1] : 0u;
        v.z = (qd * 4 + 2 < R) ? tbacc[qd * 4 + 2] : 0u;
        v.w = (qd * 4 + 3 < R) ? tbacc[qd * 4 + 3] : 0u;
        dst[qd * 32] = v;
      }
    }
  }
  if (PR && TR) flush_rows(t0 >> KREL_BITS, SnR);
  }
  if (TR && !PR) {
#pragma unroll
    for (int r = 0; r < R; ++r) {
      const int32_t slot = (rowbase + 1 + r) * 32 + c.pi;
      int32_t sn, ly;
      if (PK) {
        sn = (SnR[r] >> 12) + ys;
        ly = 4095 - (SnR[r] & 4095);
      } else {
        sn = (SnR[r] <= NEG4 / 2) ? MIN_SCORE : (SnR[r] >> 2);
        ly = LyR[r];
      }
      c.rows[rows_at<G>(ROWS_SN, c.rows_pad, slot)] = sn;
      c.rows[rows_at<G>(ROWS_LY, c.rows_pad, slot)] = ly;
    }
  }
}

template <int G, int R, int FLAGS>
B2A_HD void fill_lane(const LaneCtx<G>& c) {
  if (G == 32 && c.m == 0) return;
  const int32_t s_lo = c.only_strip >= 0 ? c.only_strip : 0;
  const int32_t s_hi = c.only_strip >= 0 ? c.only_strip + 1 : c.nstrips;
  for (int32_t s = s_lo; s < s_hi; ++s) {
    const bool full = c.uniform && ((s + 1) * (G * R) <= c.maxm - 1);
    if (full) {
      run_strip<G, R, FLAGS, false, -1>(c, s);
    } else if (cap_dispatch_of(G) && c.uniform) {
      const int32_t left = c.maxm - 1 - s * (G * R);
      const int32_t part = (left > 0 && left < G * R) ? left % R : 0;
      switch (part ? (part - 1) >> 2 : R / 4) {
        case 0: run_strip<G, R, FLAGS, true, 0>(c, s); break;
        case 1: run_strip<G, R, FLAGS, true, (1 <= R / 4 ? 1 : -1)>(c, s); break;
        case 2: run_strip<G, R, FLAGS, true, (2 <= R / 4 ? 2 : -1)>(c, s); break;
        case 3: run_strip<G, R, FLAGS, true, (3 <= R / 4 ? 3 : -1)>(c, s); break;
        case 4: run_strip<G, R, FLAGS, true, (4 <= R / 4 ? 4 : -1)>(c, s); break;
        case 5: run_strip<G, R, FLAGS, true, (5 <= R / 4 ? 5 : -1)>(c, s); break;
        default: run_strip<G, R, FLAGS, true, -1>(c, s); break;
      }
    } else {
      run_strip<G, R, FLAGS, true, -1>(c, s);
    }
  }
}

#if defined(__CUDACC__)

__device__ __forceinline__ uint32_t smem_u32(const void* p) {
  return (uint32_t)__cvta_generic_to_shared(p);
}
__device__ __forceinline__ void mbar_init(uint64_t* bar, uint32_t count) {
  asm volatile("mbarrier.init.shared::cta.b64 [%0], %1;" ::"r"(smem_u32(bar)), "r"(count));
}
__device__ __forceinline__ void mbar_expect_tx(uint64_t* bar, uint32_t bytes) {
  asm volatile("mbarrier.arrive.expect_tx.shared::cta.b64 _, [%0], %1;" ::"r"(smem_u32(bar)),
               "r"(bytes)
               : "memory");
}
__device__ __forceinline__ void tma_bulk_g2s(void* dst_smem, const void* src_gmem, uint32_t bytes,
                                             uint64_t* bar) {
  asm volatile(
      "cp.async.bulk.shared::cluster.global.mbarrier::complete_tx::bytes [%0], [%1], %2, [%3];" ::"r"(
          smem_u32(dst_smem)),
      "l"(src_gmem), "r"(bytes), "r"(smem_u32(bar))
      : "memory");
}
__device__ __forceinline__ bool mbar_try_wait(uint64_t* bar, uint32_t parity) {
  uint32_t done;
  asm volatile(
      "{\n\t.reg .pred p;\n\t"
      "mbarrier.try_wait.parity.shared::cta.b64 p, [%1], %2;\n\t"
      "selp.b32 %0, 1, 0, p;\n\t}"
      : "=r"(done)
      : "r"(smem_u32(bar)), "r"(parity)
      : "memory");
  return done != 0;
}

#ifndef B2A_MINB
#define B2A_MINB 1
#endif

template <int G, int R, int FLAGS>
__global__ void __launch_bounds__(fill_warps_of(G, R) * 32, B2A_MINB) fill_kernel(const FillParams prm) {
  extern __shared__ __align__(128) uint8_t smem[];
  constexpr int P = 32 / G;
  constexpr int FILL_WARPS = fill_warps_of(G, R);
  constexpr bool LUT = (FLAGS & F_LUT) != 0;
  constexpr int TBW = tbw_of(R);
  const int warp = threadIdx.x >> 5, lane = threadIdx.x & 31;
  uint64_t* bars = reinterpret_cast<uint64_t*>(smem);
  int32_t* lut_s = reinterpret_cast<int32_t*>(smem + 64);
  const uint32_t lut_bytes = LUT ? lut_smem_bytes(prm.sc.alpha) : 0u;
  uint8_t* stage = smem + 64 + lut_bytes + (size_t)warp * prm.smem_seq_bytes;
  uint64_t* bar = &bars[warp];
  if (threadIdx.x < FILL_WARPS) mbar_init(&bars[threadIdx.x], 1);
  if (LUT) {
    for (int k = threadIdx.x; k < lut_entries(prm.sc.alpha); k += blockDim.x) lut_s[k] = prm.lut[k];
  }
  asm volatile("fence.mbarrier_init.release.cluster;" ::: "memory");
  __syncthreads();

  const bool strip_tasks = (G == 32) && prm.progress != nullptr;
  const uint32_t ntasks = strip_tasks ? prm.n_strip_tasks : prm.nblocks * G;
  uint32_t parity = 0;

  for (uint32_t done = 0; prm.task_limit == 0 || done < prm.task_limit; ++done) {
    uint32_t task = 0;
    if (lane == 0) task = atomicAdd(prm.task_counter, 1u);
    task = __shfl_sync(0xffffffffu, task, 0);
    if (task >= ntasks) break;
    uint32_t b, sub;
    int32_t only_strip = -1;
    if (strip_tasks) {
      uint32_t lo = 0, hi = prm.nblocks;
      while (hi - lo > 1) {
        const uint32_t mid = (lo + hi) / 2;
        if (prm.blocks[mid].strip_task_base <= task) lo = mid;
        else hi = mid;
      }
      b = lo;
      const uint32_t rel = task - (uint32_t)prm.blocks[b].strip_task_base;
      const uint32_t ns = prm.blocks[b].nstrips;
      sub = rel / ns;
      only_strip = (int32_t)(rel % ns);
    } else {
      b = task / G;
      sub = task % G;
    }
    const Block blk = prm.blocks[b];
    if (strip_tasks && sub >= blk.npairs) continue;
    const uint32_t xbytes = blk.xwords * P * 4, ybytes = blk.ywords * P * 4;
    const uint32_t xoff = strip_tasks ? (uint32_t)only_strip * G * R : 0u;
    const uint32_t xstage = strip_tasks ? (uint32_t)(G * R) : xbytes;
    constexpr bool YS = (FLAGS & F_YSTREAM) != 0;
    if (lane == 0) {
      asm volatile("fence.proxy.async.shared::cta;" ::: "memory");
      mbar_expect_tx(bar, xstage + (YS ? 0u : ybytes));
      const uint8_t* src = prm.seq + blk.seq_off;
      tma_bulk_g2s(stage, src + (size_t)sub * xbytes + xoff, xstage, bar);
      if (!YS) tma_bulk_g2s(stage + xstage, src + (size_t)G * xbytes + (size_t)sub * ybytes, ybytes, bar);
    }
    LaneCtx<G> c;
    c.sc = prm.sc;
    c.lut = lut_s;
    c.lut_base = smem_u32(lut_s);
    c.one = prm.one;
    c.ge4 = prm.ge4;
    c.only_strip = only_strip;
    c.prog_mine = strip_tasks ? prm.progress + task : nullptr;
    c.prog_prev = (strip_tasks && only_strip > 0) ? prm.progress + task - 1 : nullptr;
    c.xs = reinterpret_cast<const uint32_t*>(stage) - xoff / 4;
    c.ys = YS ? reinterpret_cast<const uint32_t*>(prm.seq + blk.seq_off + (size_t)G * xbytes + (size_t)sub * ybytes)
              : reinterpret_cast<const uint32_t*>(stage + xstage);
    c.g = lane / G;
    c.l = lane % G;
    c.lane = lane;
    c.pi = (int32_t)(sub * P) + c.g;
    const bool valid = (uint32_t)c.pi < blk.npairs;
    c.m = valid ? (int32_t)prm.pm[blk.first + c.pi] : 0;
    c.n = valid ? (int32_t)prm.pn[blk.first + c.pi] : 0;
    c.maxn = (int32_t)blk.maxn;
    c.maxm = (int32_t)blk.maxm;
    c.nstrips = (int32_t)blk.nstrips;
    c.K = (int32_t)blk.K;
    c.rows_pad = (int32_t)blk.rows_pad;
    c.uniform = blk.uniform != 0;
    c.bnd = reinterpret_cast<int4*>(prm.bnd + blk.bnd_off);
    c.rows = reinterpret_cast<int32_t*>(prm.rows + blk.rows_off);
    c.tb = (FLAGS & F_NOTB) ? nullptr
                            : reinterpret_cast<uint4*>(prm.tb + blk.tb_off) + (size_t)sub * blk.nstrips * blk.K * TBW * 32;
    while (!mbar_try_wait(bar, parity)) {
    }
    parity ^= 1u;
    fill_lane<G, R, FLAGS>(c);
    __syncwarp();
  }
}

#endif

}
```

### rust_bio_b200/csrc/b2a_fill_inst.cu

```cuda
#include "b2a_fill_launch.h"

#ifndef B2A_G
#error "compile with -DB2A_G=... -DB2A_R=..."
#endif

#ifdef B2A_NOTB
#define B2A_LAUNCH_NAME launch_fill_notb_
#else
#define B2A_LAUNCH_NAME launch_fill_
#endif

namespace b2a {

namespace {

template <int FLAGS>
cudaError_t go(const FillParams& prm, uint32_t ntasks, int num_sms, cudaStream_t stream,
               int* grid_out, int dry) {
  auto kern = fill_kernel<B2A_G, B2A_R, FLAGS>;
  constexpr int FILL_WARPS = fill_warps_of(B2A_G, B2A_R);
  const uint32_t lut_bytes = (FLAGS & F_LUT) ? lut_smem_bytes(prm.sc.alpha) : 0u;
  const size_t smem = 64 + lut_bytes + (size_t)FILL_WARPS * prm.smem_seq_bytes;
  cudaError_t err =
      cudaFuncSetAttribute(kern, cudaFuncAttributeMaxDynamicSharedMemorySize, (int)smem);
  if (err != cudaSuccess) return err;
  int per_sm = 0;
  err = cudaOccupancyMaxActiveBlocksPerMultiprocessor(&per_sm, kern, FILL_WARPS * 32, smem);
  if (err != cudaSuccess) return err;
  if (per_sm < 1) return cudaErrorLaunchOutOfResources;
  if (dry) {
    if (grid_out) *grid_out = num_sms * per_sm * FILL_WARPS;
    return cudaSuccess;
  }
  const uint32_t want = (ntasks + FILL_WARPS - 1) / FILL_WARPS;
  uint32_t grid = (uint32_t)(num_sms * per_sm);
  if (grid > want) grid = want;
  if (prm.task_limit) grid = (want + prm.task_limit - 1) / prm.task_limit;
  if (grid < 1) grid = 1;
  if (grid_out) *grid_out = (int)grid;
  kern<<<grid, FILL_WARPS * 32, smem, stream>>>(prm);
  return cudaGetLastError();
}

}

#define B2A_CAT2(a, b, c) a##b##_##c
#define B2A_CAT(a, b, c) B2A_CAT2(a, b, c)

cudaError_t B2A_CAT(B2A_LAUNCH_NAME, B2A_G, B2A_R)(int flags, const FillParams& prm, uint32_t ntasks,
                                                   int num_sms, cudaStream_t stream, int* grid_out, int dry) {
  constexpr int ALL = F_TRACK_ROWS | F_TRACK_COLS | F_CLIPX;
#ifdef B2A_NOTB
  constexpr int NOTB = F_NOTB;
#else
  constexpr int NOTB = 0;
#endif
#if B2A_G == 32
#define B2A_CASE(F)                                                                    \
  case (NOTB | (F)): return go<(NOTB | (F))>(prm, ntasks, num_sms, stream, grid_out, dry); \
  case (NOTB | F_YSTREAM | (F)): return go<(NOTB | F_YSTREAM | (F))>(prm, ntasks, num_sms, stream, grid_out, dry);
#else
#define B2A_CASE(F) \
  case (NOTB | (F)): return go<(NOTB | (F))>(prm, ntasks, num_sms, stream, grid_out, dry);
#endif
  switch (flags) {
    B2A_CASE(0)
    B2A_CASE(F_TRACK_ROWS)
    B2A_CASE(F_TRACK_ROWS | F_PACKTRK)
    B2A_CASE(ALL)
    B2A_CASE(ALL | F_PACKTRK)
    B2A_CASE(ALL | F_RELU)
    B2A_CASE(ALL | F_PACKTRK | F_RELU)
    B2A_CASE(F_LUT)
    B2A_CASE(F_LUT | F_TRACK_ROWS)
    B2A_CASE(F_LUT | F_TRACK_ROWS | F_PACKTRK)
    B2A_CASE(F_LUT | ALL)
    B2A_CASE(F_LUT | ALL | F_PACKTRK)
    B2A_CASE(F_LUT | ALL | F_RELU)
    B2A_CASE(F_LUT | ALL | F_PACKTRK | F_RELU)
    B2A_CASE(F_TRACK_ROWS | F_PACKTRK | F_BND8)
    B2A_CASE(ALL | F_PACKTRK | F_BND8)
    B2A_CASE(ALL | F_PACKTRK | F_RELU | F_BND8)
    B2A_CASE(F_LUT | F_TRACK_ROWS | F_PACKTRK | F_BND8)
    B2A_CASE(F_LUT | ALL | F_PACKTRK | F_BND8)
    B2A_CASE(F_LUT | ALL | F_PACKTRK | F_RELU | F_BND8)
    B2A_CASE(F_TRACK_ROWS | F_PACKREL)
    B2A_CASE(ALL | F_PACKREL)
    B2A_CASE(ALL | F_PACKREL | F_RELU)
    B2A_CASE(F_LUT | F_TRACK_ROWS | F_PACKREL)
    B2A_CASE(F_LUT | ALL | F_PACKREL)
    B2A_CASE(F_LUT | ALL | F_PACKREL | F_RELU)
    default: return cudaErrorInvalidValue;
  }
}

}
```

### rust_bio_b200/csrc/b2a_plan.h

```cpp
#pragma once
#include <algorithm>
#include <cstdint>
#include <numeric>
#include <vector>

#include "b2a_common.cuh"

namespace b2a {

struct Wave {
  uint32_t block_lo, block_hi;
  uint64_t bnd_bytes, rows_bytes, rowm_bytes, tb_bytes;
  uint64_t strip_tasks;
};

struct Plan {
  int G = 1, R = 16;
  uint64_t n_pairs = 0;
  std::vector<uint32_t> order;
  std::vector<uint32_t> pm, pn;
  std::vector<Block> blocks;
  std::vector<Wave> waves;
  uint64_t seq_bytes = 0, ops_bytes = 0;
  uint64_t max_bnd = 0, max_rows = 0, max_rowm = 0, max_tb = 0;
  uint64_t max_strip_tasks = 0;
  uint64_t total_tb = 0;
  uint64_t cells = 0;
  uint32_t smem_seq_bytes = 0;
  uint32_t maxm = 0, maxn = 0;
};

inline uint64_t align_up(uint64_t v, uint64_t a) { return (v + a - 1) / a * a; }

inline void build_plan(Plan& p, const uint32_t* x_len, const uint32_t* y_len, uint64_t n_pairs, int G,
                       int R, uint64_t tb_budget, int flags = 0) {
  const uint64_t bnd_rec = (flags & F_BND8) ? 8 : 16;
  const bool notb = (flags & F_NOTB) != 0;
  p.G = G;
  p.R = R;
  p.n_pairs = n_pairs;
  p.order.resize(n_pairs);
  std::iota(p.order.begin(), p.order.end(), 0u);
  bool uniform_all = true;
  for (uint64_t i = 1; i < n_pairs && uniform_all; ++i)
    uniform_all = (x_len[i] == x_len[0]) && (y_len[i] == y_len[0]);
  if (!uniform_all) {
    std::stable_sort(p.order.begin(), p.order.end(), [&](uint32_t a, uint32_t b) {
      if (x_len[a] != x_len[b]) return x_len[a] > x_len[b];
      return y_len[a] > y_len[b];
    });
  }
  p.pm.resize(n_pairs);
  p.pn.resize(n_pairs);
  p.cells = 0;
  for (uint64_t i = 0; i < n_pairs; ++i) {
    p.pm[i] = x_len[p.order[i]];
    p.pn[i] = y_len[p.order[i]];
    p.cells += (uint64_t)p.pm[i] * p.pn[i];
  }
  const int P = 32 / G, TBW = tbw_of(R);
  auto task_tb = [&](uint32_t maxm, uint32_t maxn) -> uint64_t {
    const uint64_t nstrips = maxm >= 2 ? (maxm - 1 + G * R - 1) / (G * R) : 0;
    const uint64_t K = maxn ? (maxn + G - 1 + 7) / 8 : 0;
    return nstrips * K * TBW * 512;
  };
  const bool per_pair = G == 32 && !notb;
  p.blocks.clear();
  for (uint64_t first = 0; first < n_pairs;) {
    uint32_t q = 0, mm = 0, mn = 0;
    while (q < 32 && first + q < n_pairs) {
      const uint32_t m2 = std::max(mm, p.pm[first + q]), n2 = std::max(mn, p.pn[first + q]);
      if (per_pair && q > 0 && (uint64_t)(q + 1) * task_tb(m2, n2) > tb_budget) break;
      mm = m2;
      mn = n2;
      ++q;
    }
    Block k{};
    k.first = (uint32_t)first;
    k.npairs = q;
    p.blocks.push_back(k);
    first += q;
  }
  const uint32_t nblocks = (uint32_t)p.blocks.size();
  p.waves.clear();
  p.seq_bytes = p.ops_bytes = 0;
  p.max_bnd = p.max_rows = p.max_rowm = p.max_tb = 0;
  p.max_strip_tasks = 0;
  p.total_tb = 0;
  p.smem_seq_bytes = 0;
  p.maxm = p.maxn = 0;
  Wave w{0, 0, 0, 0, 0, 0, 0};
  for (uint32_t b = 0; b < nblocks; ++b) {
    Block& k = p.blocks[b];
    k.maxm = k.maxn = 0;
    for (uint32_t q = 0; q < k.npairs; ++q) {
      k.maxm = std::max(k.maxm, p.pm[k.first + q]);
      k.maxn = std::max(k.maxn, p.pn[k.first + q]);
    }
    k.uniform = 1;
    for (uint32_t q = 0; q < k.npairs; ++q)
      if (p.pm[k.first + q] != k.maxm || p.pn[k.first + q] != k.maxn) k.uniform = 0;
    k.nstrips = k.maxm >= 2 ? (k.maxm - 1 + G * R - 1) / (G * R) : 0;
    const uint32_t xw = std::max<uint32_t>((k.maxm + 3) / 4, k.nstrips * G * R / 4);
    k.xwords = (uint32_t)align_up(std::max<uint32_t>(xw, 4), 4);
    k.ywords = (uint32_t)align_up(std::max<uint32_t>((k.maxn + 3) / 4, 4), 4);
    k.K = k.maxn ? (k.maxn + G - 1 + 7) / 8 : 0;
    k.rows_pad = k.nstrips * G * R + 2;
    p.maxm = std::max(p.maxm, k.maxm);
    p.maxn = std::max(p.maxn, k.maxn);
    const uint32_t stage_x = G == 32 ? (uint32_t)(G * R) : k.xwords * P * 4;
    p.smem_seq_bytes = std::max<uint32_t>(p.smem_seq_bytes, stage_x + k.ywords * P * 4);
    const uint64_t bnd = align_up((uint64_t)(k.maxn + 1) * 32 * bnd_rec, 256);
    const uint64_t rows = align_up((uint64_t)ROWS_ARRAYS * k.rows_pad * 32 * 4, 256);
    const uint64_t rowm = align_up((uint64_t)(k.maxn + 1) * 32 * 2, 256);
    const uint32_t tasks = G == 32 ? k.npairs : (uint32_t)G;
    const uint64_t tb = notb ? 0 : align_up((uint64_t)tasks * k.nstrips * k.K * TBW * 512, 256);
    const bool full = notb ? w.bnd_bytes + w.rows_bytes + w.rowm_bytes + bnd + rows + rowm > tb_budget
                           : w.tb_bytes + tb > tb_budget;
    if (b > w.block_lo && full) {
      w.block_hi = b;
      p.waves.push_back(w);
      w = Wave{b, b, 0, 0, 0, 0, 0};
    }
    k.seq_off = p.seq_bytes;
    p.seq_bytes += align_up((uint64_t)32 * (k.xwords + k.ywords) * 4, 256);
    k.ops_off = p.ops_bytes;
    p.ops_bytes += align_up((uint64_t)32 * (k.maxm + k.maxn + 4), 256);
    k.strip_task_base = w.strip_tasks;
    w.strip_tasks += (uint64_t)(G == 32 ? k.npairs : 32) * k.nstrips;
    k.bnd_off = w.bnd_bytes;
    k.rows_off = w.rows_bytes;
    k.rowm_off = w.rowm_bytes;
    k.tb_off = w.tb_bytes;
    w.bnd_bytes += bnd;
    w.rows_bytes += rows;
    w.rowm_bytes += rowm;
    w.tb_bytes += tb;
    if (!notb) p.total_tb += (uint64_t)tasks * k.nstrips * k.K * TBW * 512;
  }
  if (nblocks) {
    w.block_hi = nblocks;
    p.waves.push_back(w);
  }
  for (const Wave& v : p.waves) {
    p.max_bnd = std::max(p.max_bnd, v.bnd_bytes);
    p.max_rows = std::max(p.max_rows, v.rows_bytes);
    p.max_rowm = std::max(p.max_rowm, v.rowm_bytes);
    p.max_tb = std::max(p.max_tb, v.tb_bytes);
    p.max_strip_tasks = std::max(p.max_strip_tasks, v.strip_tasks);
  }
}

inline int scoring_flags(const DevScoring& sc, int64_t score_bound = (1ll << 40), uint32_t maxm = ~0u,
                         uint32_t maxn = ~0u) {
  const bool xp = sc.xclip_prefix > DEAD_CLIP, xs = sc.xclip_suffix > DEAD_CLIP;
  const bool yp = sc.yclip_prefix > DEAD_CLIP, ys = sc.yclip_suffix > DEAD_CLIP;
  int f = 0;
  if (xs || (xp && yp)) {
    f = F_TRACK_ROWS | F_TRACK_COLS | F_CLIPX;
  } else if (ys) {
    f = F_TRACK_ROWS;
  }
  if (sc.alpha) f |= F_LUT;
  if ((f & F_CLIPX) && sc.xclip_prefix == 0 && sc.yclip_prefix == 0) f |= F_RELU;
  if ((f & (F_TRACK_ROWS | F_TRACK_COLS)) && score_bound < (1ll << 17) && maxm <= 4095 && maxn <= 4095)
    f |= F_PACKTRK;
  else if ((f & (F_TRACK_ROWS | F_TRACK_COLS)) && score_bound < (1ll << 18))
    f |= F_PACKREL;
  return f;
}

inline bool boundary8_ok(int flags, int64_t score_bound) {
  return (flags & F_PACKTRK) != 0 && 4 * score_bound + 3 < (1ll << 15);
}

inline bool banded_strip_gate(const DevScoring& sc, int64_t score_bound, uint32_t maxm) {
  const bool xs_dead = sc.xclip_suffix <= DEAD_CLIP, ys_dead = sc.yclip_suffix <= DEAD_CLIP;
  const bool yp_live = sc.yclip_prefix > DEAD_CLIP;
  const bool trackers_ok = (xs_dead && ys_dead) || (yp_live && score_bound < (1ll << 17) && (xs_dead || maxm <= 4095));
  return score_bound < (1ll << 26) && trackers_ok;
}

}
```

### rust_bio_b200/csrc/b2a_walk.cuh

```cuda
#pragma once
#include "b2a_common.cuh"
#include "b2a_coop.cuh"

namespace b2a {

struct WalkParams {
  const Block* blocks;
  uint32_t nblocks;
  const uint32_t* pm;
  const uint32_t* pn;
  const uint32_t* order;
  const uint8_t* seq;
  const uint8_t* bnd;
  uint8_t* rows;
  uint8_t* rowm;
  const uint8_t* tb;
  uint8_t* ops_scratch;
  const int32_t* lut;
  DevScoring sc;
  int32_t G, R;
  int32_t filter_clips;
  int32_t packtrk;
  int32_t bnd8;
  uint32_t seq_smem_per_warp;
  int32_t* score;
  uint32_t* xstart;
  uint32_t* xend;
  uint32_t* ystart;
  uint32_t* yend;
  uint32_t* n_ops;
  uint64_t* ops_src;
  uint32_t* clip_len;
  uint32_t* status;
  uint32_t* err_flag;
};

constexpr uint32_t LAZY = 15;

template <class T>
B2A_HD T ldg_ro(const T* p) {
#if defined(__CUDA_ARCH__)
  return __ldg(p);
#else
  return *p;
#endif
}

struct PairView {
  DevScoring sc;
  const int32_t* lut;
  const uint32_t* xw;
  const uint32_t* yw;
  int32_t P;
  int32_t m, n, pi;
  int32_t G, R, TBW, nstrips, K;
  const int4* bnd;
  int32_t* rows;
  int32_t rows_pad;
  uint16_t* rowm;
  const uint32_t* tb;
  int32_t sub, g;
  int32_t packtrk;
  int32_t bnd8 = 0;
  int32_t maxn;
  int64_t bnd_base;
  int32_t bnd_stride;
  const uint8_t* xs8 = nullptr;
  const uint8_t* ys8 = nullptr;
  uint64_t mulR = 0, mulGR = 0;
  B2A_HD void set_shape(int32_t G_, int32_t R_) {
    G = G_;
    R = R_;
    TBW = (R_ + 3) / 4;
    mulR = ((1ull << 40) + (uint64_t)R_ - 1) / (uint64_t)R_;
    mulGR = ((1ull << 40) + (uint64_t)(G_ * R_) - 1) / (uint64_t)(G_ * R_);
  }

  B2A_HD int32_t xsym(int32_t i) const {
    const int32_t b = i - 1;
    if (xs8) return (int32_t)xs8[b];
    return (int32_t)((xw[(b >> 2) * P] >> (8 * (b & 3))) & 0xffu);
  }
  B2A_HD int32_t ysym(int32_t j) const {
    const int32_t b = j - 1;
    if (ys8) return (int32_t)ys8[b];
    return (int32_t)((yw[(b >> 2) * P] >> (8 * (b & 3))) & 0xffu);
  }
  B2A_HD int32_t score(int32_t p, int32_t q) const {
    if (sc.alpha) return lut[p * sc.alpha + q];
    return p == q ? sc.match_score : sc.mismatch_score;
  }
  B2A_HD int32_t& row(int arr, int32_t i) const { return rows[rows_index(arr, rows_pad, i * 32 + pi)]; }
  B2A_HD int4 load_bnd(int32_t j) const {
    const int64_t k = bnd_base + (int64_t)j * bnd_stride;
    if (bnd8) {
      const int2 r = ldg_ro(&reinterpret_cast<const int2*>(bnd)[k]);
      return make_int4(r.x, r.y, 0, 0);
    }
    return ldg_ro(&bnd[k]);
  }
  B2A_HD uint32_t nib(int32_t i, int32_t j) const {
    const int32_t GR = G * R;
    const int32_t s = (int32_t)(((uint64_t)(uint32_t)(i - 1) * mulGR) >> 40), rem = (i - 1) - s * GR;
    const int32_t l = (int32_t)(((uint64_t)(uint32_t)rem * mulR) >> 40), r = rem - l * R;
    const int32_t lane = g * G + l;
    const int32_t t = (j - 1) + l;
    const size_t word =
        ((((size_t)(sub * nstrips + s) * K + (t >> 3)) * TBW + (r >> 2)) * 32 + lane) * 4 + (r & 3);
    return (tb[word] >> (4 * (7 - (t & 7)))) & 15u;
  }
  B2A_HD uint32_t nib_scode(uint32_t nb, int32_t i, int32_t j) const {
    switch (nb & 3u) {
      case NB_DIAG: return xsym(i) == ysym(j) ? TB_MATCH : TB_SUBST;
      case NB_INS: return TB_INS;
      case NB_DEL: return TB_DEL;
      default: return TB_XCLIP_PREFIX;
    }
  }
};

struct Boundary {
  int32_t S, I, Tv, Ti;
};
B2A_HD Boundary decode_boundary(const int4 b, const bool packtrk, const bool bnd8, const int32_t xs, const int32_t m) {
  Boundary o;
  o.S = (bnd8 ? lo_s16(b.x) : b.x) >> 2;
  o.I = (bnd8 ? hi_s16(b.x) : b.y) >> 2;
  o.Tv = MIN_SCORE;
  o.Ti = m;
  const int32_t key = bnd8 ? b.y : b.z;
  if (packtrk) {
    if (key != (int32_t)0x80000000) {
      o.Tv = (key >> 12) + xs;
      o.Ti = 4095 - (key & 4095);
    }
  } else if (b.z > -(1 << 29)) {
    o.Tv = b.z >> 2;
    o.Ti = b.w;
  }
  return o;
}

B2A_HD uint32_t cell_make(uint32_t i, uint32_t d, uint32_t s) { return i | (d << 4) | (s << 8); }
B2A_HD uint32_t cell_i(uint32_t c) { return c & 15u; }
B2A_HD uint32_t cell_d(uint32_t c) { return (c >> 4) & 15u; }
B2A_HD uint32_t cell_s(uint32_t c) { return (c >> 8) & 15u; }
B2A_HD uint32_t cell_set_s(uint32_t c, uint32_t s) { return (c & ~0xF00u) | (s << 8); }
B2A_HD uint32_t cell_set_i(uint32_t c, uint32_t i) { return (c & ~0x00Fu) | i; }

struct WalkOut {
  int32_t score;
  uint32_t xstart, xend, ystart, yend, n_ops, status;
  uint32_t clip[4];
};

struct EndState {
  int32_t SmN, ImN;
  uint32_t cmN;
  int32_t Snm, Lym;
  int32_t Lx0, LxN;
};

B2A_HD void finish_matrix_seq(const PairView& v, EndState& es) {
  const DevScoring& sc = v.sc;
  const int32_t m = v.m, n = v.n;
  const int32_t go = sc.gap_open, ge = sc.gap_extend;
  const int32_t xp = sc.xclip_prefix, xs = sc.xclip_suffix, yp = sc.yclip_prefix,
                ys = sc.yclip_suffix;

  int32_t SmN = 0, ImN = MIN_SCORE;
  uint32_t cmN = 0;
  int32_t Snm = MIN_SCORE, Lym = 0;
  int32_t Lx0 = 0, LxN = 0;
  if (m >= 1) {
    int32_t T = MIN_SCORE;
    for (int32_t i = 1; i < m; ++i) {
      const int32_t val = col0_S(sc, i) + xs;
      if (val > T) {
        T = val;
        Lx0 = m - i;
      }
    }
    int32_t Im = col0_I(sc, m);
    uint32_t ib = col0_ibits(sc, m);
    int32_t Sm = T;
    uint32_t sb = TB_XCLIP_SUFFIX;
    if (Im > Sm) {
      Sm = Im;
      sb = TB_INS;
    }
    if (xp > Sm) {
      Sm = xp;
      sb = TB_XCLIP_PREFIX;
    }
    if (Sm + ys > Snm) {
      Snm = Sm + ys;
      Lym = n;
    }
    int32_t Dm = MIN_SCORE;
    uint32_t cell = cell_make(ib, TB_START, sb);
    v.rowm[0 * 32 + v.pi] = (uint16_t)cell;
    LxN = Lx0;
    const int32_t p = v.xsym(m);
    const int32_t yclip_score = yp + go + ge * (m - 1);
    int32_t sdiag = (m == 1) ? 0 : col0_S(sc, m - 1);
    constexpr int UB = 4;
    for (int32_t j0 = 1; j0 <= n; j0 += UB) {
      int4 braw[UB];
      int32_t qv[UB];
#pragma unroll
      for (int u = 0; u < UB; ++u) {
        const int32_t jj = j0 + u;
        braw[u] = make_int4(0, 0, 0, 0);
        qv[u] = 0;
        if (jj <= n) {
          if (m != 1) braw[u] = v.load_bnd(jj);
          qv[u] = v.ysym(jj);
        }
      }
#pragma unroll
      for (int u = 0; u < UB; ++u) {
      const int32_t j = j0 + u;
      if (j > n) break;
      int32_t sup, iup, Tv, Ti;
      if (m == 1) {
        sup = row0_S(sc, j, n);
        iup = MIN_SCORE;
        Tv = MIN_SCORE;
        Ti = m;
      } else {
        const Boundary b = decode_boundary(braw[u], v.packtrk != 0, v.bnd8 != 0, xs, m);
        sup = b.S;
        iup = b.I;
        Tv = b.Tv;
        Ti = b.Ti;
      }
      const int32_t q = qv[u];
      const int32_t m_score = sdiag + v.score(p, q);
      int32_t best_i, best_d;
      {
        const int32_t i_score = iup + ge, s_score = sup + go;
        if (i_score > s_score) {
          best_i = i_score;
          ib = TB_INS;
        } else {
          best_i = s_score;
          ib = LAZY;
        }
      }
      uint32_t db;
      {
        const int32_t d_score = Dm + ge, s_score = Sm + go;
        if (d_score > s_score) {
          best_d = d_score;
          db = TB_DEL;
        } else {
          best_d = s_score;
          db = sb;
        }
      }
      int32_t best = Tv;
      sb = TB_XCLIP_SUFFIX;
      if (m_score > best) {
        best = m_score;
        sb = (p == q) ? TB_MATCH : TB_SUBST;
      }
      if (best_i > best) {
        best = best_i;
        sb = TB_INS;
      }
      if (best_d > best) {
        best = best_d;
        sb = TB_DEL;
      }
      const int32_t xcs = xclip_score(sc, j);
      if (xcs > best) {
        best = xcs;
        sb = TB_XCLIP_PREFIX;
      }
      if (yclip_score > best) {
        best = yclip_score;
        sb = TB_YCLIP_PREFIX;
      }
      Sm = best;
      Im = best_i;
      Dm = best_d;
      if (Sm + ys > Snm) {
        Snm = Sm + ys;
        Lym = n - j;
      }
      if (j == n) {
        LxN = m - Ti;
        if (ib == LAZY) {
          ib = (m == 1) ? row0_sbits(sc, n, n)
                        : v.nib_scode((uint32_t)v.row(ROWS_NL, m - 1), m - 1, n);
        }
      }
      cell = cell_make(ib, db, sb);
      v.rowm[j * 32 + v.pi] = (uint16_t)cell;
      sdiag = sup;
          }
    }
    SmN = Sm;
    ImN = Im;
    cmN = cell;
  }

  const bool ys_live = ys > DEAD_CLIP;
  {
    int32_t s0, c0;
    if (n == 0) {
      s0 = 0;
      c0 = (int32_t)cell_make(TB_START, TB_START, TB_START);
    } else {
      s0 = row0_S(sc, n, n);
      c0 = (int32_t)cell_make(TB_START, row0_dbits(sc, n), row0_sbits(sc, n, n));
    }
    if (m == 0) {
      SmN = s0;
      cmN = (uint32_t)c0;
      Snm = ys;
      Lym = n;
    } else {
      uint32_t s_above = cell_s((uint32_t)c0);
      {
        int32_t S = s0;
        uint32_t cell = (uint32_t)c0;
        if (ys > S) {
          S = ys;
          cell = cell_set_s(cell, TB_YCLIP_SUFFIX);
        }
        v.row(ROWS_SL, 0) = S;
        v.row(ROWS_IL, 0) = MIN_SCORE;
        v.row(ROWS_NL, 0) = (int32_t)cell;
        if (S + xs > SmN) {
          SmN = S + xs;
          LxN = m;
          cmN = cell_set_s(cmN, TB_XCLIP_SUFFIX);
        }
      }
      constexpr int UB = 4;
      for (int32_t i0 = 1; i0 < m; i0 += UB) {
        int32_t nbv[UB], Sv[UB], Snv[UB];
#pragma unroll
        for (int u = 0; u < UB; ++u) {
          const int32_t i = i0 + u;
          nbv[u] = Sv[u] = 0;
          Snv[u] = MIN_SCORE;
          if (i < m && n != 0) {
            nbv[u] = v.row(ROWS_NL, i);
            Sv[u] = v.row(ROWS_SL, i);
            if (ys_live) Snv[u] = v.row(ROWS_SN, i);
          }
        }
#pragma unroll
        for (int u = 0; u < UB; ++u) {
          const int32_t i = i0 + u;
          if (i >= m) break;
          uint32_t cell;
          int32_t S, Sn;
          if (n == 0) {
            S = col0_S(sc, i);
            v.row(ROWS_IL, i) = col0_I(sc, i);
            cell = cell_make(col0_ibits(sc, i), TB_START, col0_sbits(sc, i));
            const int32_t val = S + ys;
            Sn = val > MIN_SCORE ? val : MIN_SCORE;
            if (!ys_live) Sn = MIN_SCORE;
            v.row(ROWS_LY, i) = 0;
          } else {
            const uint32_t nb = (uint32_t)nbv[u];
            cell = cell_make((nb & NB_IEXT) ? (uint32_t)TB_INS : s_above, (nb & NB_DEXT) ? (uint32_t)TB_DEL : LAZY,
                             v.nib_scode(nb, i, n));
            S = Sv[u];
            Sn = Snv[u];
          }
          s_above = cell_s(cell);
          if (Sn > S) {
            S = Sn;
            cell = cell_set_s(cell, TB_YCLIP_SUFFIX);
          }
          v.row(ROWS_SL, i) = S;
          v.row(ROWS_NL, i) = (int32_t)cell;
          if (S + xs > SmN) {
            SmN = S + xs;
            LxN = m - i;
            cmN = cell_set_s(cmN, TB_XCLIP_SUFFIX);
          }
        }
      }
      if (Snm > SmN) {
        SmN = Snm;
        cmN = cell_set_s(cmN, TB_YCLIP_SUFFIX);
      }
      int32_t S_prev = v.row(ROWS_SL, 0);
      uint32_t cell_prev = (uint32_t)v.row(ROWS_NL, 0);
      for (int32_t i0 = 1; i0 <= m; i0 += UB) {
        int32_t Iv[UB], Sv[UB], Cv[UB];
#pragma unroll
        for (int u = 0; u < UB; ++u) {
          const int32_t i = i0 + u;
          Iv[u] = Sv[u] = Cv[u] = 0;
          if (i < m) {
            Iv[u] = v.row(ROWS_IL, i);
            Sv[u] = v.row(ROWS_SL, i);
            Cv[u] = v.row(ROWS_NL, i);
          }
        }
#pragma unroll
        for (int u = 0; u < UB; ++u) {
          const int32_t i = i0 + u;
          if (i > m) break;
          const int32_t s_score = S_prev + go;
          int32_t I = (i == m) ? ImN : Iv[u];
          int32_t S = (i == m) ? SmN : Sv[u];
          uint32_t cell = (i == m) ? cmN : (uint32_t)Cv[u];
          bool dirty = false;
          if (s_score > I) {
            I = s_score;
            cell = cell_set_i(cell, cell_s(cell_prev));
            dirty = true;
          }
          if (s_score > S) {
            S = s_score;
            cell = cell_set_s(cell, TB_INS);
            dirty = true;
            if (i != m && S + xs > SmN) {
              SmN = S + xs;
              LxN = m - i;
              cmN = cell_set_s(cmN, TB_XCLIP_SUFFIX);
            }
          }
          if (i == m) {
            ImN = I;
            SmN = S;
            cmN = cell;
          } else if (dirty) {
            v.row(ROWS_IL, i) = I;
            v.row(ROWS_SL, i) = S;
            v.row(ROWS_NL, i) = (int32_t)cell;
          }
          S_prev = S;
          cell_prev = cell;
        }
      }
    }
  }

  es.SmN = SmN;
  es.ImN = ImN;
  es.cmN = cmN;
  es.Snm = Snm;
  es.Lym = Lym;
  es.Lx0 = Lx0;
  es.LxN = LxN;
}

struct WalkState {
  int32_t i, j;
  uint32_t layer;
  uint32_t xstart, ystart, xend, yend;
  uint32_t nops, nclip, status;
  uint32_t clips[4];
  int32_t guard;
  uint8_t* ops_end;
};

B2A_HD void walk_begin(const PairView& v, const EndState& es, uint8_t* ops_end, WalkState& w) {
  w.i = v.m;
  w.j = v.n;
  w.layer = cell_s(es.cmN);
  w.xstart = w.ystart = 0;
  w.xend = (uint32_t)v.m;
  w.yend = (uint32_t)v.n;
  w.nops = w.nclip = w.status = 0;
  w.clips[0] = w.clips[1] = w.clips[2] = w.clips[3] = 0;
  w.guard = v.m + v.n + 8;
  w.ops_end = ops_end;
}

template <bool SCORES = false>
B2A_HD bool walk_run(const PairView& v, const EndState& es, const bool filter_clips, WalkState& w, int32_t max_steps) {
  const DevScoring& sc = v.sc;
  const int32_t m = v.m, n = v.n;
  const int32_t xs = sc.xclip_suffix;
  const uint32_t cmN = es.cmN;
  const int32_t LxN = es.LxN, Lx0 = es.Lx0, Lym = es.Lym;
  auto get_cell_n = [&](int32_t i) -> uint32_t {
    return (i == m) ? cmN : (uint32_t)v.row(ROWS_NL, i);
  };
  auto get_s = [&](int32_t i, int32_t j) -> uint32_t {
    if (j == n) return cell_s(get_cell_n(i));
    if (i == 0) return row0_sbits(sc, j, n);
    if (i == m) return cell_s((uint32_t)v.rowm[j * 32 + v.pi]);
    if (j == 0) return col0_sbits(sc, i);
    if (SCORES) return TB_START;
    return v.nib_scode(v.nib(i, j), i, j);
  };
  int32_t i = w.i, j = w.j;
  uint32_t xstart = w.xstart, ystart = w.ystart, xend = w.xend, yend = w.yend;
  uint32_t nops = w.nops, nclip = w.nclip, status = w.status;
  uint32_t clips[4] = {w.clips[0], w.clips[1], w.clips[2], w.clips[3]};
  uint32_t layer = w.layer;
  int32_t guard = w.guard;
  uint8_t* ops_end = w.ops_end;
  while (layer != TB_START && status == 0) {
    if (SCORES && i < m && j < n) break;
    if (max_steps-- <= 0) break;
    if (--guard < 0) {
      status = 1;
      break;
    }
    uint32_t next;
    if (layer == TB_INS) {
      if (!SCORES) *(--ops_end) =3;
      ++nops;
      uint32_t c;
      if (j == n) {
        c = cell_i(get_cell_n(i));
      } else if (i == m) {
        c = cell_i((uint32_t)v.rowm[j * 32 + v.pi]);
        if (c == LAZY) c = get_s(m - 1, j);
      } else if (j == 0) {
        c = col0_ibits(sc, i);
      } else {
        c = (v.nib(i, j) & NB_IEXT) ? (uint32_t)TB_INS : get_s(i - 1, j);
      }
      next = c;
      i -= 1;
    } else if (layer == TB_DEL) {
      if (!SCORES) *(--ops_end) =2;
      ++nops;
      uint32_t c;
      if (i == 0) {
        c = row0_dbits(sc, j);
      } else if (i == m) {
        c = cell_d((uint32_t)v.rowm[j * 32 + v.pi]);
      } else if (j == n) {
        c = cell_d(get_cell_n(i));
        if (c == LAZY) c = get_s(i, n - 1);
      } else {
        c = (v.nib(i, j) & NB_DEXT) ? (uint32_t)TB_DEL : get_s(i, j - 1);
      }
      next = c;
      j -= 1;
    } else if (layer == TB_MATCH || layer == TB_SUBST) {
      if (!SCORES) *(--ops_end) =(layer == TB_MATCH) ? 0 : 1;
      ++nops;
      next = get_s(i - 1, j - 1);
      i -= 1;
      j -= 1;
    } else if (layer == TB_XCLIP_PREFIX) {
      if (!filter_clips) {
        if (!SCORES) *(--ops_end) =4;
        ++nops;
        if (nclip < 4) clips[nclip] = (uint32_t)i;
        ++nclip;
      }
      xstart = (uint32_t)i;
      i = 0;
      next = get_s(0, j);
    } else if (layer == TB_XCLIP_SUFFIX) {
      int32_t lx;
      if (j == n) lx = LxN;
      else if (j == 0) lx = Lx0;
      else lx = (m >= 2) ? m - decode_boundary(v.load_bnd(j), v.packtrk != 0, v.bnd8 != 0, xs, m).Ti : 0;
      if (!filter_clips) {
        if (!SCORES) *(--ops_end) =4;
        ++nops;
        if (nclip < 4) clips[nclip] = (uint32_t)lx;
        ++nclip;
      }
      i -= lx;
      xend = (uint32_t)i;
      next = get_s(i, j);
    } else if (layer == TB_YCLIP_PREFIX) {
      if (!filter_clips) {
        if (!SCORES) *(--ops_end) =5;
        ++nops;
        if (nclip < 4) clips[nclip] = (uint32_t)j;
        ++nclip;
      }
      ystart = (uint32_t)j;
      j = 0;
      next = get_s(i, 0);
    } else if (layer == TB_YCLIP_SUFFIX) {
      int32_t ly;
      if (i == m) ly = Lym;
      else if (i == 0 || n == 0) ly = n;
      else ly = n - v.row(ROWS_LY, i);
      if (!filter_clips) {
        if (!SCORES) *(--ops_end) =5;
        ++nops;
        if (nclip < 4) clips[nclip] = (uint32_t)ly;
        ++nclip;
      }
      j -= ly;
      yend = (uint32_t)j;
      next = get_s(i, j);
    } else {
      status = 1;
      break;
    }
    if (i < 0 || j < 0) {
      status = 1;
      break;
    }
    layer = next;
  }
  w.i = i;
  w.j = j;
  w.layer = layer;
  w.xstart = xstart;
  w.ystart = ystart;
  w.xend = xend;
  w.yend = yend;
  w.nops = nops;
  w.nclip = nclip;
  w.status = status;
  for (int k = 0; k < 4; ++k) w.clips[k] = clips[k];
  w.guard = guard;
  w.ops_end = ops_end;
  return layer == TB_START || status != 0 || (SCORES && i < m && j < n);
}

B2A_HD void walk_finish(const EndState& es, const WalkState& w, WalkOut& out) {
  out.score = es.SmN;
  out.xstart = w.xstart;
  out.xend = w.xend;
  out.ystart = w.ystart;
  out.yend = w.yend;
  out.n_ops = w.nops;
  out.status = (w.nclip > 4) ? 1u : w.status;
  const uint32_t nc = w.nclip > 4 ? 4 : w.nclip;
  for (uint32_t k = 0; k < 4; ++k) out.clip[k] = (k < nc) ? w.clips[nc - 1 - k] : 0u;
}

template <bool SCORES = false>
B2A_HD void walk_pair(const PairView& v, const bool filter_clips, uint8_t* ops_end, WalkOut& out) {
  EndState es;
  finish_matrix_seq(v, es);
  WalkState w;
  walk_begin(v, es, ops_end, w);
  walk_run<SCORES>(v, es, filter_clips, w, 0x7fffffff);
  walk_finish(es, w, out);
}

B2A_HD int32_t imin32(int32_t a, int32_t b) { return a < b ? a : b; }

template <int W>
B2A_HD int32_t coop_scan_max(int lane, int32_t v) {
  using C = Coop<W>;
  for (int d = 1; d < W; d <<= 1) {
    const int32_t t = C::up(v, d);
    if (lane >= d) v = imax(v, t);
  }
  return v;
}

template <int W>
B2A_HD bool coop_argmax_first(int lane, bool has, int32_t val, int32_t idx, int32_t& best_val, int32_t& best_idx,
                              bool packed = false) {
  using C = Coop<W>;
  (void)lane;
  if (C::ballot(has) == 0u) return false;
  if (packed) {
    const int32_t key = C::all_max32(has ? val * 4096 + (4095 - idx) : (int32_t)0x80000000);
    best_val = key >> 12;
    best_idx = 4095 - (key & 4095);
    return true;
  }
  const long long none = (long long)0x8000000000000000ull;
  long long key = has ? (long long)(((unsigned long long)(long long)val << 32) | (unsigned long long)(uint32_t)(0x7fffffff - idx))
                      : none;
  key = C::all_max(key);
  best_val = (int32_t)(key >> 32);
  best_idx = 0x7fffffff - (int32_t)(uint32_t)(key & 0xffffffffll);
  return true;
}

template <int W>
B2A_HD void finish_matrix_coop(const int lane, const PairView& v, EndState& es) {
  using C = Coop<W>;
  const DevScoring& sc = v.sc;
  const int32_t m = v.m, n = v.n;
  if (m < 2 || n < 1) {
    if (lane == 0) finish_matrix_seq(v, es);
    C::sync();
    es.SmN = C::from(es.SmN, 0);
    es.ImN = C::from(es.ImN, 0);
    es.cmN = (uint32_t)C::from((int32_t)es.cmN, 0);
    es.Snm = C::from(es.Snm, 0);
    es.Lym = C::from(es.Lym, 0);
    es.Lx0 = C::from(es.Lx0, 0);
    es.LxN = C::from(es.LxN, 0);
    return;
  }
  const int32_t go = sc.gap_open, ge = sc.gap_extend;
  const int32_t xp = sc.xclip_prefix, xs = sc.xclip_suffix, yp = sc.yclip_prefix, ys = sc.yclip_suffix;
  const int32_t gs = imax(ge, go);
  const bool pk = v.packtrk != 0;

  int32_t T = MIN_SCORE, Lx0 = 0;
  if (col0_S(sc, 1) + xs > MIN_SCORE) {
    T = col0_S(sc, 1) + xs;
    Lx0 = m - 1;
  }
  int32_t Im0 = col0_I(sc, m);
  const uint32_t ib0 = col0_ibits(sc, m);
  int32_t Sm0 = T;
  uint32_t sb0 = TB_XCLIP_SUFFIX;
  if (Im0 > Sm0) {
    Sm0 = Im0;
    sb0 = TB_INS;
  }
  if (xp > Sm0) {
    Sm0 = xp;
    sb0 = TB_XCLIP_PREFIX;
  }
  int32_t Snm = MIN_SCORE, Lym = 0;
  if (Sm0 + ys > Snm) {
    Snm = Sm0 + ys;
    Lym = n;
  }
  if (lane == 0) v.rowm[0 * 32 + v.pi] = (uint16_t)cell_make(ib0, TB_START, sb0);
  int32_t LxN = Lx0;
  const int32_t p = v.xsym(m);
  const int32_t yclip_score = yp + go + ge * (m - 1);
  int32_t cSup = col0_S(sc, m - 1);
  int32_t cD = MIN_SCORE, cS = Sm0;
  uint32_t csb = sb0;
  int32_t SmN = 0, ImN = MIN_SCORE;
  uint32_t cmN = 0;
  int4 braw_next = v.load_bnd(imin32(1 + lane, n));
  for (int32_t base = 1; base <= n; base += W) {
    const int32_t j = base + lane;
    const bool act = j <= n;
    const int32_t jc = act ? j : n;
    const int4 braw = braw_next;
    if (base + W <= n) braw_next = v.load_bnd(imin32(base + W + lane, n));
    const Boundary b = decode_boundary(braw, pk, v.bnd8 != 0, xs, m);
    const int32_t q = v.ysym(jc);
    int32_t sdiag = C::up(b.S, 1);
    if (lane == 0) sdiag = cSup;
    const int32_t m_score = sdiag + v.score(p, q);
    uint32_t ib;
    int32_t best_i;
    {
      const int32_t i_score = b.I + ge, s_score = b.S + go;
      if (i_score > s_score) {
        best_i = i_score;
        ib = TB_INS;
      } else {
        best_i = s_score;
        ib = LAZY;
      }
    }
    const int32_t xcs = xclip_score(sc, jc);
    const int32_t A = imax(imax(imax(b.Tv, m_score), imax(best_i, xcs)), yclip_score);
    int32_t t;
    {
      const int32_t aprev = C::up(A, 1);
      if (lane == 0) t = imax(cD + ge, cS + go) - gs * jc;
      else t = aprev + go - gs * jc;
    }
    const int32_t best_d = coop_scan_max<W>(lane, t) + gs * jc;
    int32_t best = b.Tv;
    uint32_t sb = TB_XCLIP_SUFFIX;
    if (m_score > best) {
      best = m_score;
      sb = (p == q) ? TB_MATCH : TB_SUBST;
    }
    if (best_i > best) {
      best = best_i;
      sb = TB_INS;
    }
    if (best_d > best) {
      best = best_d;
      sb = TB_DEL;
    }
    if (xcs > best) {
      best = xcs;
      sb = TB_XCLIP_PREFIX;
    }
    if (yclip_score > best) {
      best = yclip_score;
      sb = TB_YCLIP_PREFIX;
    }
    int32_t pD = C::up(best_d, 1), pS = C::up(best, 1);
    uint32_t psb = (uint32_t)C::up((int32_t)sb, 1);
    if (lane == 0) {
      pD = cD;
      pS = cS;
      psb = csb;
    }
    const uint32_t db = (pD + ge > pS + go) ? (uint32_t)TB_DEL : psb;
    {
      int32_t gv, gj;
      if (coop_argmax_first<W>(lane, act && best + ys > Snm, best, j, gv, gj, pk)) {
        Snm = gv + ys;
        Lym = n - gj;
      }
    }
    if (act && j == n) {
      if (ib == LAZY) ib = v.nib_scode((uint32_t)v.row(ROWS_NL, m - 1), m - 1, n);
    }
    const uint32_t cell = cell_make(ib, db, sb);
    if (act) v.rowm[j * 32 + v.pi] = (uint16_t)cell;
    const int32_t left = n - base;
    const int src = left < W - 1 ? left : W - 1;
    cSup = C::from(b.S, src);
    cD = C::from(best_d, src);
    cS = C::from(best, src);
    csb = (uint32_t)C::from((int32_t)sb, src);
    if (base + W > n) {
      SmN = cS;
      ImN = C::from(best_i, src);
      cmN = (uint32_t)C::from((int32_t)cell, src);
      LxN = m - C::from(b.Ti, src);
    }
  }

  C::sync();

  const bool ys_live = ys > DEAD_CLIP;
  const int32_t s0 = row0_S(sc, n, n);
  const uint32_t c0 = cell_make(TB_START, row0_dbits(sc, n), row0_sbits(sc, n, n));
  {
    int32_t S = s0;
    uint32_t cell = c0;
    if (ys > S) {
      S = ys;
      cell = cell_set_s(cell, TB_YCLIP_SUFFIX);
    }
    if (lane == 0) {
      v.row(ROWS_SL, 0) = S;
      v.row(ROWS_IL, 0) = MIN_SCORE;
      v.row(ROWS_NL, 0) = (int32_t)cell;
    }
    if (S + xs > SmN) {
      SmN = S + xs;
      LxN = m;
      cmN = cell_set_s(cmN, TB_XCLIP_SUFFIX);
    }
  }
  {
    uint32_t c_above = cell_s(c0);
    const int32_t yn = v.ysym(n);
    int32_t nb_next, S_next, Sn_next = MIN_SCORE;
    {
      const int32_t i0 = imin32(1 + lane, m - 1);
      nb_next = v.row(ROWS_NL, i0);
      S_next = v.row(ROWS_SL, i0);
      if (ys_live) Sn_next = v.row(ROWS_SN, i0);
    }
    for (int32_t base = 1; base < m; base += W) {
      const int32_t i = base + lane;
      const bool act = i < m;
      const int32_t ic = act ? i : m - 1;
      const uint32_t nb = (uint32_t)nb_next;
      int32_t S = S_next;
      const int32_t Sn = Sn_next;
      if (base + W < m) {
        const int32_t i1 = imin32(base + W + lane, m - 1);
        nb_next = v.row(ROWS_NL, i1);
        S_next = v.row(ROWS_SL, i1);
        if (ys_live) Sn_next = v.row(ROWS_SN, i1);
      }
      uint32_t sbi;
      switch (nb & 3u) {
        case NB_DIAG: sbi = v.xsym(ic) == yn ? TB_MATCH : TB_SUBST; break;
        case NB_INS: sbi = TB_INS; break;
        case NB_DEL: sbi = TB_DEL; break;
        default: sbi = TB_XCLIP_PREFIX; break;
      }
      uint32_t s_above = (uint32_t)C::up((int32_t)sbi, 1);
      if (lane == 0) s_above = c_above;
      uint32_t cell = cell_make((nb & NB_IEXT) ? (uint32_t)TB_INS : s_above, (nb & NB_DEXT) ? (uint32_t)TB_DEL : LAZY, sbi);
      if (Sn > S) {
        S = Sn;
        cell = cell_set_s(cell, TB_YCLIP_SUFFIX);
      }
      if (act) {
        v.row(ROWS_SL, i) = S;
        v.row(ROWS_NL, i) = (int32_t)cell;
      }
      int32_t gv, gi;
      if (coop_argmax_first<W>(lane, act && S + xs > SmN, S, i, gv, gi, pk)) {
        SmN = gv + xs;
        LxN = m - gi;
        cmN = cell_set_s(cmN, TB_XCLIP_SUFFIX);
      }
      const int32_t left = m - 1 - base;
      c_above = (uint32_t)C::from((int32_t)sbi, left < W - 1 ? left : W - 1);
    }
  }
  if (Snm > SmN) {
    SmN = Snm;
    cmN = cell_set_s(cmN, TB_YCLIP_SUFFIX);
  }
  C::sync();

  int32_t cSp;
  uint32_t ccell;
  {
    int32_t S = s0;
    uint32_t cell = c0;
    if (ys > S) {
      S = ys;
      cell = cell_set_s(cell, TB_YCLIP_SUFFIX);
    }
    cSp = S;
    ccell = cell;
  }
  int32_t I_next, S2_next, c_next;
  {
    const int32_t i0 = imin32(1 + lane, m - 1);
    I_next = v.row(ROWS_IL, i0);
    S2_next = v.row(ROWS_SL, i0);
    c_next = v.row(ROWS_NL, i0);
  }
  for (int32_t base = 1; base < m; base += W) {
    const int32_t i = base + lane;
    const bool act = i < m;
    const int32_t ic = act ? i : m - 1;
    int32_t I = I_next, S = S2_next;
    uint32_t cell = (uint32_t)c_next;
    if (base + W < m) {
      const int32_t i1 = imin32(base + W + lane, m - 1);
      I_next = v.row(ROWS_IL, i1);
      S2_next = v.row(ROWS_SL, i1);
      c_next = v.row(ROWS_NL, i1);
    }
    int32_t Sprev = C::up(S, 1);
    if (lane == 0) Sprev = cSp;
    if (C::ballot(Sprev + go > S) != 0u) {
      int32_t t = S - go * ic;
      if (lane == 0) t = imax(t, cSp + go - go * ic);
      const int32_t Snew = coop_scan_max<W>(lane, t) + go * ic;
      Sprev = C::up(Snew, 1);
      if (lane == 0) Sprev = cSp;
    }
    const int32_t s_score = Sprev + go;
    const bool raised = s_score > S;
    uint32_t my_s_after = raised ? (uint32_t)TB_INS : cell_s(cell);
    uint32_t prev_s_after = (uint32_t)C::up((int32_t)my_s_after, 1);
    if (lane == 0) prev_s_after = cell_s(ccell);
    bool dirty = false;
    if (s_score > I) {
      I = s_score;
      cell = cell_set_i(cell, prev_s_after);
      dirty = true;
    }
    if (raised) {
      S = s_score;
      cell = cell_set_s(cell, TB_INS);
      dirty = true;
    }
    if (act && dirty) {
      v.row(ROWS_IL, i) = I;
      v.row(ROWS_SL, i) = S;
      v.row(ROWS_NL, i) = (int32_t)cell;
    }
    int32_t gv, gi;
    if (coop_argmax_first<W>(lane, act && raised && S + xs > SmN, S, i, gv, gi, pk)) {
      SmN = gv + xs;
      LxN = m - gi;
      cmN = cell_set_s(cmN, TB_XCLIP_SUFFIX);
    }
    const int32_t left = m - 1 - base;
    const int src = left < W - 1 ? left : W - 1;
    cSp = C::from(S, src);
    ccell = (uint32_t)C::from((int32_t)cell, src);
  }
  {
    const int32_t s_score = cSp + go;
    if (s_score > ImN) {
      ImN = s_score;
      cmN = cell_set_i(cmN, cell_s(ccell));
    }
    if (s_score > SmN) {
      SmN = s_score;
      cmN = cell_set_s(cmN, TB_INS);
    }
  }
  C::sync();
  es.SmN = SmN;
  es.ImN = ImN;
  es.cmN = cmN;
  es.Snm = Snm;
  es.Lym = Lym;
  es.Lx0 = Lx0;
  es.LxN = LxN;
}

B2A_HD void prefetch_tb(const PairView& v, int32_t i, int32_t j) {
#if defined(__CUDA_ARCH__)
  if (i >= 1 && i <= v.m - 1 && j >= 1 && j <= v.n) {
    const int32_t GR = v.G * v.R;
    const int32_t s = (int32_t)(((uint64_t)(uint32_t)(i - 1) * v.mulGR) >> 40), rem = (i - 1) - s * GR;
    const int32_t l = (int32_t)(((uint64_t)(uint32_t)rem * v.mulR) >> 40), r = rem - l * v.R;
    const int32_t ln = v.g * v.G + l;
    const int32_t t = (j - 1) + l;
    const size_t word =
        ((((size_t)(v.sub * v.nstrips + s) * v.K + (t >> 3)) * v.TBW + (r >> 2)) * 32 + ln) * 4 + (r & 3);
    asm volatile("prefetch.global.L1 [%0];" ::"l"(v.tb + word));
  }
#else
  (void)v;
  (void)i;
  (void)j;
#endif
}

template <int W, bool SCORES = false>
B2A_HD void walk_pair_coop(const int lane, const PairView& v, const bool filter_clips, uint8_t* ops_end, WalkOut& out) {
  using C = Coop<W>;
  EndState es;
  finish_matrix_coop<W>(lane, v, es);
  WalkState w;
  walk_begin(v, es, ops_end, w);
  constexpr int32_t kBurst = 24;
  for (;;) {
    if (!SCORES) {
      const int32_t ci = C::from(w.i, 0), cj = C::from(w.j, 0);
      prefetch_tb(v, ci - 1 - lane, cj - 1 - lane);
    }
    int32_t done = 0;
    if (lane == 0) done = walk_run<SCORES>(v, es, filter_clips, w, kBurst) ? 1 : 0;
    if (C::from(done, 0)) break;
  }
  walk_finish(es, w, out);
}

#if defined(__CUDACC__)

template <bool SCORES>
__device__ __forceinline__ void walk_store(const WalkParams& prm, const Block& blk, const uint32_t sp, const int pi,
                                           const uint32_t cap, WalkOut& o) {
  if (o.status) {
    o.score = MIN_SCORE;
    o.n_ops = 0;
    o.xstart = o.xend = o.ystart = o.yend = 0;
    o.clip[0] = o.clip[1] = o.clip[2] = o.clip[3] = 0;
  }
  const uint32_t dst = prm.order[sp];
  prm.score[dst] = o.score;
  if (!SCORES) prm.xstart[dst] = o.xstart;
  prm.xend[dst] = o.xend;
  if (!SCORES) prm.ystart[dst] = o.ystart;
  prm.yend[dst] = o.yend;
  if (!SCORES) {
    prm.n_ops[dst] = o.n_ops;
    prm.ops_src[dst] = blk.ops_off + (uint64_t)(pi + 1) * cap - o.n_ops;
  }
  prm.status[dst] = o.status;
  if (o.status) atomicOr(prm.err_flag, 1u);
  if (!SCORES) {
#pragma unroll
    for (int k = 0; k < 4; ++k) prm.clip_len[4 * (size_t)dst + k] = o.clip[k];
  }
}

template <bool SCORES>
__device__ __forceinline__ void walk_lane(const WalkParams& prm, const Block& blk, const int lane) {
  if ((uint32_t)lane >= blk.npairs) return;
  const uint32_t sp = blk.first + lane;
  const int32_t P = 32 / prm.G;
  PairView v;
  v.sc = prm.sc;
  v.lut = prm.lut;
  v.P = P;
  v.m = (int32_t)prm.pm[sp];
  v.n = (int32_t)prm.pn[sp];
  v.pi = lane;
  v.set_shape(prm.G, prm.R);
  v.nstrips = (int32_t)blk.nstrips;
  v.K = (int32_t)blk.K;
  v.sub = lane / P;
  v.g = lane % P;
  v.packtrk = prm.packtrk;
  v.bnd8 = prm.bnd8;
  v.maxn = (int32_t)blk.maxn;
  v.bnd_base = bnd_index(prm.G, 0, lane, v.maxn);
  v.bnd_stride = (int32_t)(bnd_index(prm.G, 1, lane, v.maxn) - v.bnd_base);
  const uint32_t* seqw = reinterpret_cast<const uint32_t*>(prm.seq + blk.seq_off);
  v.xw = seqw + (size_t)v.sub * blk.xwords * P + v.g;
  v.yw = seqw + (size_t)prm.G * blk.xwords * P + (size_t)v.sub * blk.ywords * P + v.g;
  v.bnd = reinterpret_cast<const int4*>(prm.bnd + blk.bnd_off);
  v.rows = reinterpret_cast<int32_t*>(prm.rows + blk.rows_off);
  v.rows_pad = (int32_t)blk.rows_pad;
  v.rowm = reinterpret_cast<uint16_t*>(prm.rowm + blk.rowm_off);
  v.tb = reinterpret_cast<const uint32_t*>(prm.tb + blk.tb_off);
  const uint32_t cap = blk.maxm + blk.maxn + 4;
  uint8_t* ops_end = SCORES ? nullptr : prm.ops_scratch + blk.ops_off + (size_t)(lane + 1) * cap;
  WalkOut o;
  walk_pair<SCORES>(v, prm.filter_clips != 0, ops_end, o);
  walk_store<SCORES>(prm, blk, sp, lane, cap, o);
}

template <bool SCORES>
__device__ __forceinline__ void walk_warp(const WalkParams& prm, const Block& blk, const int pi, const int lane,
                                          uint8_t* seq_smem) {
  const uint32_t sp = blk.first + pi;
  const int32_t P = 32 / prm.G;
  PairView v;
  v.sc = prm.sc;
  v.lut = prm.lut;
  v.P = P;
  v.m = (int32_t)prm.pm[sp];
  v.n = (int32_t)prm.pn[sp];
  v.pi = pi;
  v.set_shape(prm.G, prm.R);
  v.nstrips = (int32_t)blk.nstrips;
  v.K = (int32_t)blk.K;
  v.sub = pi / P;
  v.g = pi % P;
  v.packtrk = prm.packtrk;
  v.bnd8 = prm.bnd8;
  v.maxn = (int32_t)blk.maxn;
  v.bnd_base = bnd_index(prm.G, 0, pi, v.maxn);
  v.bnd_stride = (int32_t)(bnd_index(prm.G, 1, pi, v.maxn) - v.bnd_base);
  const uint32_t* seqw = reinterpret_cast<const uint32_t*>(prm.seq + blk.seq_off);
  v.xw = seqw + (size_t)v.sub * blk.xwords * P + v.g;
  v.yw = seqw + (size_t)prm.G * blk.xwords * P + (size_t)v.sub * blk.ywords * P + v.g;
  v.bnd = reinterpret_cast<const int4*>(prm.bnd + blk.bnd_off);
  v.rows = reinterpret_cast<int32_t*>(prm.rows + blk.rows_off);
  v.rows_pad = (int32_t)blk.rows_pad;
  v.rowm = reinterpret_cast<uint16_t*>(prm.rowm + blk.rowm_off);
  v.tb = reinterpret_cast<const uint32_t*>(prm.tb + blk.tb_off);
  if (seq_smem) {
    const int32_t xwn = (v.m + 3) >> 2, ywn = (v.n + 3) >> 2;
    uint32_t* xs = reinterpret_cast<uint32_t*>(seq_smem);
    uint32_t* ys = xs + ((blk.maxm + 3) >> 2);
    for (int32_t w = lane; w < xwn; w += 32) xs[w] = v.xw[(size_t)w * P];
    for (int32_t w = lane; w < ywn; w += 32) ys[w] = v.yw[(size_t)w * P];
    __syncwarp();
    v.xs8 = reinterpret_cast<const uint8_t*>(xs);
    v.ys8 = reinterpret_cast<const uint8_t*>(ys);
  }
  const uint32_t cap = blk.maxm + blk.maxn + 4;
  uint8_t* ops_end = SCORES ? nullptr : prm.ops_scratch + blk.ops_off + (size_t)(pi + 1) * cap;
  WalkOut o;
  walk_pair_coop<32, SCORES>(lane, v, prm.filter_clips != 0, ops_end, o);
  if (lane != 0) return;
  walk_store<SCORES>(prm, blk, sp, pi, cap, o);
}

#if defined(B2A_DEFINE_WALK_KERNEL)
template <bool SCORES>
__global__ void __launch_bounds__(1024, 1) walk_warp_kernel(const WalkParams prm) {
  extern __shared__ __align__(16) uint8_t walk_smem[];
  const uint32_t gw = (blockIdx.x * blockDim.x + threadIdx.x) >> 5;
  const int lane = threadIdx.x & 31;
  const uint32_t b = gw >> 5, pi = gw & 31u;
  if (b >= prm.nblocks) return;
  const Block blk = prm.blocks[b];
  if (pi >= blk.npairs) return;
  uint8_t* mine = prm.seq_smem_per_warp ? walk_smem + (size_t)(threadIdx.x >> 5) * prm.seq_smem_per_warp : nullptr;
  walk_warp<SCORES>(prm, blk, (int)pi, lane, mine);
}

template <bool SCORES>
__global__ void __launch_bounds__(128, 8) walk_kernel(const WalkParams prm) {
  const uint32_t gw = (blockIdx.x * blockDim.x + threadIdx.x) >> 5;
  const int lane = threadIdx.x & 31;
  if (gw >= prm.nblocks) return;
  const Block blk = prm.blocks[gw];
  walk_lane<SCORES>(prm, blk, lane);
}
#endif

#endif

}
```

Before: 787.5.

## Fuse last-column and last-row finishing into fill kernel for thread-per-pair shape

For the G==1 shape without packed-relative rows, the fill kernel now finishes the last column (column n) and the last row m inline as it computes them. It writes the final traceback cells and a small per-pair end state into a new fin buffer, so the walk kernel loads that state instead of redoing the sequential finish_matrix pass. The aim is to remove a serial per-pair pass from the walk phase and the row-array traffic it needs. In exchange the fill kernel does extra per-column branching and stores, with more register pressure.

```diff
diff --git a/rust_bio_b200/csrc/b2a_common.cuh b/rust_bio_b200/csrc/b2a_common.cuh
--- a/rust_bio_b200/csrc/b2a_common.cuh
+++ b/rust_bio_b200/csrc/b2a_common.cuh
@@ -59,7 +59,9 @@
   F_BND8 = 256,
   F_NOTB = 512,
   F_YSTREAM = 1024,
+  F_FINISH = 2048,
 };
+enum { FIN_SMN = 0, FIN_IMN, FIN_CMN, FIN_SNM, FIN_LYM, FIN_LX0, FIN_LXN, FIN_FIELDS };
 #ifndef B2A_KREL_BITS
 #define B2A_KREL_BITS 12
 #endif
diff --git a/rust_bio_b200/csrc/b2a_engine.cu b/rust_bio_b200/csrc/b2a_engine.cu
--- a/rust_bio_b200/csrc/b2a_engine.cu
+++ b/rust_bio_b200/csrc/b2a_engine.cu
@@ -127,7 +127,7 @@
   uint8_t codemap_host[256];
 
   DevBuf d_blob, d_xoff, d_xlen, d_yoff, d_ylen, d_order, d_pm, d_pn, d_blocks, d_seq, d_bnd, d_rows,
-      d_rowm, d_tb, d_opsscratch, d_lut, d_codemap, d_ctl, d_score, d_xs, d_xe, d_ys, d_ye, d_nops,
+      d_rowm, d_fin, d_tb, d_opsscratch, d_lut, d_codemap, d_ctl, d_score, d_xs, d_xe, d_ys, d_ye, d_nops,
       d_opssrc, d_clip, d_status, d_nops64, d_opsoff, d_opsdense, d_scan, d_records, d_prog, d_bcells, d_bstatus,
       d_bopsend, d_bslab, d_branges, d_broff, d_bfill, d_bfoff, d_hmoff, d_hmxy, d_hpoff, d_hpidx, d_raw, d_gnops,
       d_gnops64, d_goff, d_bcols, d_bstrip, d_bsoff, d_belig;
@@ -301,7 +301,7 @@
   if (e->h_plan) cudaFreeHost(e->h_plan);
   if (e->h_nops) cudaFreeHost(e->h_nops);
   DevBuf* bufs[] = {&e->d_blob, &e->d_xoff, &e->d_xlen, &e->d_yoff, &e->d_ylen, &e->d_order, &e->d_pm,
-                    &e->d_pn, &e->d_blocks, &e->d_seq, &e->d_bnd, &e->d_rows, &e->d_rowm, &e->d_tb,
+                    &e->d_pn, &e->d_blocks, &e->d_seq, &e->d_bnd, &e->d_rows, &e->d_rowm, &e->d_fin, &e->d_tb,
                     &e->d_opsscratch, &e->d_lut, &e->d_codemap, &e->d_ctl, &e->d_score, &e->d_xs,
                     &e->d_xe, &e->d_ys, &e->d_ye, &e->d_nops, &e->d_opssrc, &e->d_clip, &e->d_status,
                     &e->d_nops64, &e->d_opsoff, &e->d_opsdense, &e->d_scan, &e->d_records, &e->d_prog, &e->d_bcells,
@@ -521,6 +521,8 @@
   return B2A_OK;
 }
 
+static int32_t* fin_from(int32_t* fin, uint32_t lo) { return fin ? fin + (size_t)lo * FIN_FIELDS * 32 : nullptr; }
+
 static int32_t compact_ops(b2a_engine* e, uint64_t scratch_bytes, cudaStream_t st) {
   const uint64_t n = e->n_pairs;
   if (n) {
@@ -577,6 +579,8 @@
   for (int attempt = 0;; ++attempt) {
     e->shape = find_shape(G, R);
     if (!e->shape) return e->fail(B2A_E_INVALID, "no fill kernel for the requested shape");
+    if (G == 1 && !(e->flags & F_PACKREL)) e->flags |= F_FINISH;
+    else e->flags &= ~F_FINISH;
     build_plan(e->plan, pairs->x_len, pairs->y_len, n, G, R, budget, e->flags);
     if (64 + lut_bytes + (uint64_t)fill_warps_of(G, R) * e->plan.smem_seq_bytes <= kMaxStageSmem) break;
     if (G == 32) {
@@ -613,6 +617,7 @@
   CK(e->d_bnd.reserve(pl.max_bnd + 16));
   CK(e->d_rows.reserve(pl.max_rows + 16));
   CK(e->d_rowm.reserve(pl.max_rowm + 16));
+  CK(e->d_fin.reserve(pl.max_fin + 16));
   CK(e->d_tb.reserve(pl.max_tb + 16));
   CK(e->d_prog.reserve(pl.max_strip_tasks * 4 + 16));
   CK(e->d_opsscratch.reserve(pl.ops_bytes + 16));
@@ -721,6 +726,8 @@
     fp.bnd = e->d_bnd.as<uint8_t>();
     fp.rows = e->d_rows.as<uint8_t>();
     fp.tb = e->score_only ? nullptr : e->d_tb.as<uint8_t>();
+    fp.rowm = e->d_rowm.as<uint8_t>();
+    fp.fin = (e->flags & F_FINISH) ? e->d_fin.as<int32_t>() : nullptr;
     fp.lut = e->d_lut.as<int32_t>() + (size_t)e->sc.alpha * e->sc.alpha;
     fp.task_counter = ctl + 2 + wi;
     fp.smem_seq_bytes = pl.smem_seq_bytes;
@@ -758,6 +765,7 @@
     wp.R = pl.R;
     wp.packtrk = (e->flags & F_PACKTRK) ? 1 : 0;
     wp.bnd8 = (e->flags & F_BND8) ? 1 : 0;
+    wp.fin = fp.fin;
     wp.filter_clips = (e->mode == B2A_MODE_SEMIGLOBAL || e->mode == B2A_MODE_LOCAL) ? 1 : 0;
     wp.score = e->d_score.as<int32_t>();
     wp.xstart = e->d_xs.as<uint32_t>();
@@ -817,11 +825,13 @@
       fa.nblocks = split_b;
       fb.blocks = fp.blocks + split_b;
       fb.nblocks = nb - split_b;
+      fb.fin = fin_from(fp.fin, split_b);
       fb.task_counter = ctl + 8;
       WalkParams wa = wp, wb = wp;
       wa.nblocks = split_b;
       wb.blocks = wp.blocks + split_b;
       wb.nblocks = nb - split_b;
+      wb.fin = fb.fin;
       if (e->split_timing && !e->split_ev[0])
         for (auto& v : e->split_ev) CK(cudaEventCreate(&v));
       if (e->split_timing) CK(cudaEventRecord(e->split_ev[0], st));
@@ -876,6 +886,7 @@
         FillParams f2 = fp;
         f2.blocks = fp.blocks + lo_b;
         f2.nblocks = hi_b - lo_b;
+        f2.fin = fin_from(fp.fin, lo_b);
         f2.task_counter = ctl + 8 + sidx;
         f2.task_limit = 1;
         CK(fill(e->flags, f2, f2.nblocks * (uint32_t)pl.G, e->num_sms, fs, &e->last_grid, 0));
@@ -886,6 +897,7 @@
         WalkParams w2 = wp;
         w2.blocks = wp.blocks + lo_b;
         w2.nblocks = hi_b - lo_b;
+        w2.fin = f2.fin;
         if (warp_walk) walk_warp_k<<<w2.nblocks * 32 / wcta_warps, wcta_warps * 32, (size_t)per_warp_smem * wcta_warps, e->tail_stream>>>(w2);
         else walk_lane_k<<<(w2.nblocks * 32 + 127) / 128, 128, 0, e->tail_stream>>>(w2);
         CK(cudaGetLastError());
diff --git a/rust_bio_b200/csrc/b2a_fill.cuh b/rust_bio_b200/csrc/b2a_fill.cuh
--- a/rust_bio_b200/csrc/b2a_fill.cuh
+++ b/rust_bio_b200/csrc/b2a_fill.cuh
@@ -1,5 +1,6 @@
 #pragma once
 #include "b2a_common.cuh"
+#include "b2a_walk.cuh"
 
 namespace b2a {
 
@@ -12,6 +13,8 @@
   uint8_t* bnd;
   uint8_t* rows;
   uint8_t* tb;
+  uint8_t* rowm;
+  int32_t* fin;
   const int32_t* lut;
   uint32_t* task_counter;
   uint32_t smem_seq_bytes;
@@ -49,7 +52,18 @@
   int32_t only_strip;
   int32_t one;
   int32_t ge4;
+  uint16_t* rowm = nullptr;
+  int32_t* fin = nullptr;
 };
+
+struct ColN {
+  int32_t S2;
+  uint32_t c2;
+  uint32_t sp;
+  int32_t va, ia;
+  int32_t vb, ib;
+};
+
 
 #if defined(__CUDA_ARCH__)
 #define B2A_SHFL_UP(v, G) __shfl_up_sync(0xffffffffu, (v), 1, (G))
@@ -166,7 +180,7 @@
                         const int32_t rv, int32_t (&Sp)[R], int32_t (&Dp)[R], int32_t (&SnR)[R],
                         int32_t (&LyR)[R], uint32_t (&tbacc)[R], const int32_t (&xc)[R],
                         int32_t sdiag, int32_t& sup, int32_t& iup, int32_t& Tv, int32_t& Ti,
-                        int32_t& cap_s, int32_t& cap_i) {
+                        int32_t& cap_s, int32_t& cap_i, ColN& cn) {
   constexpr bool TR = (FLAGS & F_TRACK_ROWS) != 0;
   constexpr bool TC = (FLAGS & F_TRACK_COLS) != 0;
   constexpr bool CX = (FLAGS & F_CLIPX) != 0;
@@ -175,6 +189,7 @@
   constexpr bool PK = (FLAGS & F_PACKTRK) != 0 || PR;
   constexpr bool RELU = (FLAGS & F_RELU) != 0;
   constexpr bool NOTB = (FLAGS & F_NOTB) != 0;
+  constexpr bool FIN = (FLAGS & F_FINISH) != 0;
   constexpr bool TMASK = MASKED && !LUT;
   const int32_t go4i = 4 * c.sc.gap_open + 2, go4d = 4 * c.sc.gap_open + 1, ge4 = c.ge4;
   const int32_t ma4 = 4 * c.sc.match_score + 3 - go4d, mi4 = 4 * c.sc.mismatch_score + 3 - go4d;
@@ -183,6 +198,7 @@
   const int32_t cj = 4095 - (PR ? (tstep & KREL_MASK) : j);
   const int32_t one = c.one, k2 = one + one, k16 = k2 * 8, k1024 = k16 * 64;
   const int32_t q4 = q * 4;
+  const int32_t qrow = LUT ? (int32_t)(c.lut_base + (uint32_t)(q * c.sc.alpha * 4)) : q;
   const uint32_t capbit = (MASKED && rv >= 1) ? 1u << (rv - 1) : 0u;
   int32_t Tl = KEY_NONE;
   int32_t key_even = KEY_NONE;
@@ -242,9 +258,42 @@
     }
     if (LAST) {
       const int32_t slot = (rowbase + 1 + r) * 32 + c.pi;
-      c.rows[rows_at<G>(ROWS_SL, c.rows_pad, slot)] = s4 >> 2;
-      c.rows[rows_at<G>(ROWS_IL, c.rows_pad, slot)] = i4 >> 2;
-      c.rows[rows_at<G>(ROWS_NL, c.rows_pad, slot)] = nib;
+      if (!FIN) {
+        c.rows[rows_at<G>(ROWS_SL, c.rows_pad, slot)] = s4 >> 2;
+        c.rows[rows_at<G>(ROWS_IL, c.rows_pad, slot)] = i4 >> 2;
+        c.rows[rows_at<G>(ROWS_NL, c.rows_pad, slot)] = nib;
+      } else if (!MASKED || r < rv) {
+        const int32_t i = rowbase + 1 + r;
+        const uint32_t scode = (nib & 3) == NB_DIAG ? ((LUT ? xc[r] == qrow : xc[r] == q) ? TB_MATCH : TB_SUBST)
+                                                    : nib_scode_other((uint32_t)nib);
+        uint32_t cell = cell_make((nib & NB_IEXT) ? (uint32_t)TB_INS : cn.sp, (nib & NB_DEXT) ? (uint32_t)TB_DEL : LAZY, scode);
+        cn.sp = scode;
+        int32_t S = s4 >> 2;
+        int32_t Sn = MIN_SCORE;
+        if (TR && c.sc.yclip_suffix > DEAD_CLIP) Sn = PK ? (SnR[r] >> 12) + c.sc.yclip_suffix
+                                                         : ((SnR[r] <= NEG4 / 2) ? MIN_SCORE : (SnR[r] >> 2));
+        if (Sn > S) {
+          S = Sn;
+          cell = cell_set_s(cell, TB_YCLIP_SUFFIX);
+        }
+        if (S + c.sc.xclip_suffix > cn.va) {
+          cn.va = S + c.sc.xclip_suffix;
+          cn.ia = i;
+        }
+        const int32_t s_score = cn.S2 + c.sc.gap_open;
+        if (s_score > (i4 >> 2)) cell = cell_set_i(cell, cell_s(cn.c2));
+        if (s_score > S) {
+          S = s_score;
+          cell = cell_set_s(cell, TB_INS);
+          if (S + c.sc.xclip_suffix > cn.vb) {
+            cn.vb = S + c.sc.xclip_suffix;
+            cn.ib = i;
+          }
+        }
+        cn.S2 = S;
+        cn.c2 = cell;
+        c.rows[rows_at<G>(ROWS_NL, c.rows_pad, slot)] = (int32_t)cell;
+      }
     }
     if (MASKED && (CAPQ < 0 || (r >> 2) == CAPQ)) {
       if ((capbit >> r) & 1u) {
@@ -264,8 +313,140 @@
   }
 }
 
+template <int G>
+B2A_HD void fin_column_n_begin(const LaneCtx<G>& c, ColN& cn) {
+  const DevScoring& sc = c.sc;
+  const int32_t n = c.n;
+  {
+    uint32_t c0 = cell_make(TB_START, row0_dbits(sc, n), row0_sbits(sc, n, n));
+    cn.sp = cell_s(c0);
+    int32_t S = row0_S(sc, n, n);
+    if (sc.yclip_suffix > S) {
+      S = sc.yclip_suffix;
+      c0 = cell_set_s(c0, TB_YCLIP_SUFFIX);
+    }
+    c.rows[rows_at<G>(ROWS_NL, c.rows_pad, c.pi)] = (int32_t)c0;
+    cn.S2 = S;
+    cn.c2 = c0;
+    cn.va = S + sc.xclip_suffix;
+    cn.ia = 0;
+    cn.vb = (int32_t)0x80000000;
+    cn.ib = 0;
+  }
+}
+template <int G>
+B2A_HD void fin_end_state(const LaneCtx<G>& c, const ColN& cn, const RowM& rm, int32_t ImN, uint32_t cmN,
+                          const int32_t Lx0, int32_t LxN) {
+  const int32_t m = c.m;
+  int32_t SmN = rm.Sm;
+  if (cn.va > SmN) {
+    SmN = cn.va;
+    LxN = m - cn.ia;
+    cmN = cell_set_s(cmN, TB_XCLIP_SUFFIX);
+  }
+  if (rm.Snm > SmN) {
+    SmN = rm.Snm;
+    cmN = cell_set_s(cmN, TB_YCLIP_SUFFIX);
+  }
+  if (cn.vb > SmN) {
+    SmN = cn.vb;
+    LxN = m - cn.ib;
+    cmN = cell_set_s(cmN, TB_XCLIP_SUFFIX);
+  }
+  const int32_t s_score = cn.S2 + c.sc.gap_open;
+  if (s_score > ImN) {
+    ImN = s_score;
+    cmN = cell_set_i(cmN, cell_s(cn.c2));
+  }
+  if (s_score > SmN) {
+    SmN = s_score;
+    cmN = cell_set_s(cmN, TB_INS);
+  }
+  int32_t* f = c.fin + c.pi;
+  f[FIN_SMN * 32] = SmN;
+  f[FIN_IMN * 32] = ImN;
+  f[FIN_CMN * 32] = (int32_t)cmN;
+  f[FIN_SNM * 32] = rm.Snm;
+  f[FIN_LYM * 32] = rm.Lym;
+  f[FIN_LX0 * 32] = Lx0;
+  f[FIN_LXN * 32] = LxN;
+}
+
+template <int G, int FLAGS>
+B2A_HD void fin_row_m(const LaneCtx<G>& c, const ColN& cn) {
+  constexpr bool LUT = (FLAGS & F_LUT) != 0;
+  constexpr bool PK = (FLAGS & F_PACKTRK) != 0;
+  constexpr bool B8 = (FLAGS & F_BND8) != 0;
+  constexpr int P = 32 / G;
+  const DevScoring& sc = c.sc;
+  const int32_t m = c.m, n = c.n, xs = sc.xclip_suffix;
+  int32_t T = MIN_SCORE, Lx0 = 0;
+  if (col0_S(sc, 1) + xs > MIN_SCORE) {
+    T = col0_S(sc, 1) + xs;
+    Lx0 = m - 1;
+  }
+  int32_t Im = col0_I(sc, m);
+  RowM rm{T, MIN_SCORE, TB_XCLIP_SUFFIX, MIN_SCORE, 0};
+  if (Im > rm.Sm) {
+    rm.Sm = Im;
+    rm.sb = TB_INS;
+  }
+  if (sc.xclip_prefix > rm.Sm) {
+    rm.Sm = sc.xclip_prefix;
+    rm.sb = TB_XCLIP_PREFIX;
+  }
+  if (rm.Sm + sc.yclip_suffix > rm.Snm) {
+    rm.Snm = rm.Sm + sc.yclip_suffix;
+    rm.Lym = n;
+  }
+  uint32_t cell = cell_make(col0_ibits(sc, m), TB_START, rm.sb);
+  c.rowm[0 * 32 + c.pi] = (uint16_t)cell;
+  const int32_t p = (int32_t)((c.xs[((m - 1) >> 2) * P + c.g] >> (8 * ((m - 1) & 3))) & 0xffu);
+  const uint32_t prow = LUT ? c.lut_base + (uint32_t)(p * sc.alpha * 4) : 0u;
+  const int32_t yclip_score = sc.yclip_prefix + sc.gap_open + sc.gap_extend * (m - 1);
+  int32_t sdiag = col0_S(sc, m - 1), Ti = m;
+  const int2* bnd8 = reinterpret_cast<const int2*>(c.bnd);
+  constexpr int UB = 4;
+  for (int32_t j0 = 1; j0 <= n; j0 += UB) {
+    int4 braw[UB];
+    int32_t qv[UB];
+#pragma unroll
+    for (int u = 0; u < UB; ++u) {
+      const int32_t j = j0 + u;
+      braw[u] = make_int4(0, 0, 0, 0);
+      qv[u] = 0;
+      if (j <= n) {
+        if (B8) {
+          const int2 r8 = bnd8[bnd_index(G, j, c.pi, c.maxn)];
+          braw[u] = make_int4(r8.x, r8.y, 0, 0);
+        } else {
+          braw[u] = c.bnd[bnd_index(G, j, c.pi, c.maxn)];
+        }
+        qv[u] = (int32_t)((c.ys[((j - 1) >> 2) * P + c.g] >> (8 * ((j - 1) & 3))) & 0xffu);
+      }
+    }
+#pragma unroll
+    for (int u = 0; u < UB; ++u) {
+      const int32_t j = j0 + u;
+      if (j > n) break;
+      const Boundary b = decode_boundary(braw[u], PK, B8, xs, m);
+      const int32_t q = qv[u];
+      const int32_t sub = LUT ? (lut_at(c.lut, prow + (uint32_t)(q * 4)) + 4 * sc.gap_open - 2) >> 2
+                              : (p == q ? sc.match_score : sc.mismatch_score);
+      cell = rowm_cell(sc, n, j, sub, p == q, sdiag, b.S, b.I, b.Tv, yclip_score, rm, Im);
+      if (j == n) {
+        Ti = b.Ti;
+        if (cell_i(cell) == LAZY) cell = cell_set_i(cell, cn.sp);
+      }
+      c.rowm[j * 32 + c.pi] = (uint16_t)cell;
+      sdiag = b.S;
+    }
+  }
+  fin_end_state(c, cn, rm, Im, cell, Lx0, m - Ti);
+}
+
 template <int G, int R, int FLAGS, bool MASKED, int CAPQ>
-B2A_HD void run_strip(const LaneCtx<G>& c, const int32_t s) {
+B2A_HD void run_strip(const LaneCtx<G>& c, const int32_t s, ColN& cn) {
   constexpr bool TR = (FLAGS & F_TRACK_ROWS) != 0;
   constexpr bool TC = (FLAGS & F_TRACK_COLS) != 0;
   constexpr bool LUT = (FLAGS & F_LUT) != 0;
@@ -274,7 +455,9 @@
   constexpr bool B8 = (FLAGS & F_BND8) != 0;
   constexpr bool NOTB = (FLAGS & F_NOTB) != 0;
   constexpr bool YS = (FLAGS & F_YSTREAM) != 0;
+  constexpr bool FIN = (FLAGS & F_FINISH) != 0;
   static_assert(!YS || G == 32, "F_YSTREAM is a warp-per-pair form");
+  static_assert(!FIN || (G == 1 && !PR), "F_FINISH is a thread-per-pair form, without F_PACKREL");
   static_assert(!B8 || ((FLAGS & F_PACKTRK) != 0 && !PR), "F_BND8 needs the packed column tracker with absolute rows");
   constexpr int P = 32 / G;
   constexpr int TBW = tbw_of(R);
@@ -369,7 +552,6 @@
   }
   uint4* tbs = NOTB ? nullptr : c.tb + (size_t)s * c.K * TBW * 32;
   const int32_t nsteps = c.K * 8;
-
   if (PR && TR) {
 #pragma unroll
     for (int r = 0; r < R; ++r) {
@@ -438,12 +620,14 @@
       }
       int32_t sup = in_s, iup = in_i, Tv = in_tv, Ti = in_ti;
       if (j == n) {
+        if (FIN && s == 0 && rv >= 1) fin_column_n_begin(c, cn);
         column_step<G, R, FLAGS, MASKED, true, CAPQ>(c, j, t, q, rowbase, rv, Sp, Dp, SnR, LyR, tbacc, xc,
-                                               sup_prev, sup, iup, Tv, Ti, cap_s, cap_i);
+                                               sup_prev, sup, iup, Tv, Ti, cap_s, cap_i, cn);
       } else {
         column_step<G, R, FLAGS, MASKED, false, CAPQ>(c, j, t, q, rowbase, rv, Sp, Dp, SnR, LyR, tbacc, xc,
-                                                sup_prev, sup, iup, Tv, Ti, cap_s, cap_i);
-      }
+                                                sup_prev, sup, iup, Tv, Ti, cap_s, cap_i, cn);
+      }
+
       sup_prev = in_s;
       if (writer) {
         if (B8) {
@@ -525,7 +709,7 @@
         sn = (SnR[r] <= NEG4 / 2) ? MIN_SCORE : (SnR[r] >> 2);
         ly = LyR[r];
       }
-      c.rows[rows_at<G>(ROWS_SN, c.rows_pad, slot)] = sn;
+      if (!FIN) c.rows[rows_at<G>(ROWS_SN, c.rows_pad, slot)] = sn;
       c.rows[rows_at<G>(ROWS_LY, c.rows_pad, slot)] = ly;
     }
   }
@@ -534,27 +718,29 @@
 template <int G, int R, int FLAGS>
 B2A_HD void fill_lane(const LaneCtx<G>& c) {
   if (G == 32 && c.m == 0) return;
+  ColN cn;
   const int32_t s_lo = c.only_strip >= 0 ? c.only_strip : 0;
   const int32_t s_hi = c.only_strip >= 0 ? c.only_strip + 1 : c.nstrips;
   for (int32_t s = s_lo; s < s_hi; ++s) {
     const bool full = c.uniform && ((s + 1) * (G * R) <= c.maxm - 1);
     if (full) {
-      run_strip<G, R, FLAGS, false, -1>(c, s);
+      run_strip<G, R, FLAGS, false, -1>(c, s, cn);
     } else if (cap_dispatch_of(G) && c.uniform) {
       const int32_t left = c.maxm - 1 - s * (G * R);
       const int32_t part = (left > 0 && left < G * R) ? left % R : 0;
       switch (part ? (part - 1) >> 2 : R / 4) {
-        case 0: run_strip<G, R, FLAGS, true, 0>(c, s); break;
-        case 1: run_strip<G, R, FLAGS, true, (1 <= R / 4 ? 1 : -1)>(c, s); break;
-        case 2: run_strip<G, R, FLAGS, true, (2 <= R / 4 ? 2 : -1)>(c, s); break;
-        case 3: run_strip<G, R, FLAGS, true, (3 <= R / 4 ? 3 : -1)>(c, s); break;
-        case 4: run_strip<G, R, FLAGS, true, (4 <= R / 4 ? 4 : -1)>(c, s); break;
-        case 5: run_strip<G, R, FLAGS, true, (5 <= R / 4 ? 5 : -1)>(c, s); break;
-        default: run_strip<G, R, FLAGS, true, -1>(c, s); break;
+        case 0: run_strip<G, R, FLAGS, true, 0>(c, s, cn); break;
+        case 1: run_strip<G, R, FLAGS, true, (1 <= R / 4 ? 1 : -1)>(c, s, cn); break;
+        case 2: run_strip<G, R, FLAGS, true, (2 <= R / 4 ? 2 : -1)>(c, s, cn); break;
+        case 3: run_strip<G, R, FLAGS, true, (3 <= R / 4 ? 3 : -1)>(c, s, cn); break;
+        case 4: run_strip<G, R, FLAGS, true, (4 <= R / 4 ? 4 : -1)>(c, s, cn); break;
+        case 5: run_strip<G, R, FLAGS, true, (5 <= R / 4 ? 5 : -1)>(c, s, cn); break;
+        default: run_strip<G, R, FLAGS, true, -1>(c, s, cn); break;
       }
     } else {
-      run_strip<G, R, FLAGS, true, -1>(c, s);
-    }
+      run_strip<G, R, FLAGS, true, -1>(c, s, cn);
+    }
+    if ((FLAGS & F_FINISH) && c.m >= 2 && c.n >= 1 && (c.m - 2) / (G * R) == s) fin_row_m<G, FLAGS>(c, cn);
   }
 }
 
@@ -682,6 +868,10 @@
     c.uniform = blk.uniform != 0;
     c.bnd = reinterpret_cast<int4*>(prm.bnd + blk.bnd_off);
     c.rows = reinterpret_cast<int32_t*>(prm.rows + blk.rows_off);
+    if (FLAGS & F_FINISH) {
+      c.rowm = reinterpret_cast<uint16_t*>(prm.rowm + blk.rowm_off);
+      c.fin = prm.fin + (size_t)b * FIN_FIELDS * 32;
+    }
     c.tb = (FLAGS & F_NOTB) ? nullptr
                             : reinterpret_cast<uint4*>(prm.tb + blk.tb_off) + (size_t)sub * blk.nstrips * blk.K * TBW * 32;
     while (!mbar_try_wait(bar, parity)) {
diff --git a/rust_bio_b200/csrc/b2a_fill_inst.cu b/rust_bio_b200/csrc/b2a_fill_inst.cu
--- a/rust_bio_b200/csrc/b2a_fill_inst.cu
+++ b/rust_bio_b200/csrc/b2a_fill_inst.cu
@@ -59,6 +59,10 @@
 #define B2A_CASE(F)                                                                    \
   case (NOTB | (F)): return go<(NOTB | (F))>(prm, ntasks, num_sms, stream, grid_out, dry); \
   case (NOTB | F_YSTREAM | (F)): return go<(NOTB | F_YSTREAM | (F))>(prm, ntasks, num_sms, stream, grid_out, dry);
+#elif B2A_G == 1
+#define B2A_FIN(F) (((F) & F_PACKREL) ? (F) : ((F) | F_FINISH))
+#define B2A_CASE(F) \
+  case (NOTB | B2A_FIN(F)): return go<(NOTB | B2A_FIN(F))>(prm, ntasks, num_sms, stream, grid_out, dry);
 #else
 #define B2A_CASE(F) \
   case (NOTB | (F)): return go<(NOTB | (F))>(prm, ntasks, num_sms, stream, grid_out, dry);
diff --git a/rust_bio_b200/csrc/b2a_plan.h b/rust_bio_b200/csrc/b2a_plan.h
--- a/rust_bio_b200/csrc/b2a_plan.h
+++ b/rust_bio_b200/csrc/b2a_plan.h
@@ -24,6 +24,7 @@
   uint64_t seq_bytes = 0, ops_bytes = 0;
   uint64_t max_bnd = 0, max_rows = 0, max_rowm = 0, max_tb = 0;
   uint64_t max_strip_tasks = 0;
+  uint64_t max_fin = 0;
   uint64_t total_tb = 0;
   uint64_t cells = 0;
   uint32_t smem_seq_bytes = 0;
@@ -86,6 +87,7 @@
   p.seq_bytes = p.ops_bytes = 0;
   p.max_bnd = p.max_rows = p.max_rowm = p.max_tb = 0;
   p.max_strip_tasks = 0;
+  p.max_fin = 0;
   p.total_tb = 0;
   p.smem_seq_bytes = 0;
   p.maxm = p.maxn = 0;
@@ -148,6 +150,8 @@
     p.max_rowm = std::max(p.max_rowm, v.rowm_bytes);
     p.max_tb = std::max(p.max_tb, v.tb_bytes);
     p.max_strip_tasks = std::max(p.max_strip_tasks, v.strip_tasks);
+    if (flags & F_FINISH)
+      p.max_fin = std::max<uint64_t>(p.max_fin, (uint64_t)(v.block_hi - v.block_lo) * FIN_FIELDS * 32 * 4);
   }
 }
 
diff --git a/rust_bio_b200/csrc/b2a_walk.cuh b/rust_bio_b200/csrc/b2a_walk.cuh
--- a/rust_bio_b200/csrc/b2a_walk.cuh
+++ b/rust_bio_b200/csrc/b2a_walk.cuh
@@ -22,6 +22,7 @@
   int32_t filter_clips;
   int32_t packtrk;
   int32_t bnd8;
+  const int32_t* fin;
   uint32_t seq_smem_per_warp;
   int32_t* score;
   uint32_t* xstart;
@@ -44,6 +45,10 @@
 #else
   return *p;
 #endif
+}
+
+B2A_HD uint32_t nib_scode_other(uint32_t nb) {
+  return (nb & 3u) == NB_INS ? (uint32_t)TB_INS : (nb & 3u) == NB_DEL ? (uint32_t)TB_DEL : (uint32_t)TB_XCLIP_PREFIX;
 }
 
 struct PairView {
@@ -65,6 +70,7 @@
   int32_t maxn;
   int64_t bnd_base;
   int32_t bnd_stride;
+  const int32_t* fin = nullptr;
   const uint8_t* xs8 = nullptr;
   const uint8_t* ys8 = nullptr;
   uint64_t mulR = 0, mulGR = 0;
@@ -110,13 +116,9 @@
     return (tb[word] >> (4 * (7 - (t & 7)))) & 15u;
   }
   B2A_HD uint32_t nib_scode(uint32_t nb, int32_t i, int32_t j) const {
-    switch (nb & 3u) {
-      case NB_DIAG: return xsym(i) == ysym(j) ? TB_MATCH : TB_SUBST;
-      case NB_INS: return TB_INS;
-      case NB_DEL: return TB_DEL;
-      default: return TB_XCLIP_PREFIX;
-    }
-  }
+    return (nb & 3u) == NB_DIAG ? (xsym(i) == ysym(j) ? TB_MATCH : TB_SUBST) : nib_scode_other(nb);
+  }
+  B2A_HD bool finished() const { return fin != nullptr && m >= 2 && n >= 1; }
 };
 
 struct Boundary {
@@ -161,6 +163,86 @@
   int32_t Lx0, LxN;
 };
 
+struct RowM {
+  int32_t Sm, Dm;
+  uint32_t sb;
+  int32_t Snm, Lym;
+};
+
+B2A_HD uint32_t rowm_cell(const DevScoring& sc, const int32_t n, const int32_t j, const int32_t sub, const bool same,
+                          const int32_t sdiag, const int32_t sup, const int32_t iup, const int32_t Tv,
+                          const int32_t yclip_score, RowM& st, int32_t& Im) {
+  const int32_t go = sc.gap_open, ge = sc.gap_extend;
+  const int32_t m_score = sdiag + sub;
+  int32_t best_i;
+  uint32_t ib;
+  {
+    const int32_t i_score = iup + ge, s_score = sup + go;
+    if (i_score > s_score) {
+      best_i = i_score;
+      ib = TB_INS;
+    } else {
+      best_i = s_score;
+      ib = LAZY;
+    }
+  }
+  int32_t best_d;
+  uint32_t db;
+  {
+    const int32_t d_score = st.Dm + ge, s_score = st.Sm + go;
+    if (d_score > s_score) {
+      best_d = d_score;
+      db = TB_DEL;
+    } else {
+      best_d = s_score;
+      db = st.sb;
+    }
+  }
+  int32_t best = Tv;
+  uint32_t sb = TB_XCLIP_SUFFIX;
+  if (m_score > best) {
+    best = m_score;
+    sb = same ? TB_MATCH : TB_SUBST;
+  }
+  if (best_i > best) {
+    best = best_i;
+    sb = TB_INS;
+  }
+  if (best_d > best) {
+    best = best_d;
+    sb = TB_DEL;
+  }
+  const int32_t xcs = xclip_score(sc, j);
+  if (xcs > best) {
+    best = xcs;
+    sb = TB_XCLIP_PREFIX;
+  }
+  if (yclip_score > best) {
+    best = yclip_score;
+    sb = TB_YCLIP_PREFIX;
+  }
+  st.Sm = best;
+  st.Dm = best_d;
+  st.sb = sb;
+  Im = best_i;
+  if (best + sc.yclip_suffix > st.Snm) {
+    st.Snm = best + sc.yclip_suffix;
+    st.Lym = n - j;
+  }
+  return cell_make(ib, db, sb);
+}
+
+B2A_HD void load_end_state(const PairView& v, EndState& es) {
+  const int32_t* f = v.fin + v.pi;
+  es.SmN = ldg_ro(f + FIN_SMN * 32);
+  es.ImN = ldg_ro(f + FIN_IMN * 32);
+  es.cmN = (uint32_t)ldg_ro(f + FIN_CMN * 32);
+  es.Snm = ldg_ro(f + FIN_SNM * 32);
+  es.Lym = ldg_ro(f + FIN_LYM * 32);
+  es.Lx0 = ldg_ro(f + FIN_LX0 * 32);
+  es.LxN = ldg_ro(f + FIN_LXN * 32);
+}
+
 B2A_HD void finish_matrix_seq(const PairView& v, EndState& es) {
   const DevScoring& sc = v.sc;
   const int32_t m = v.m, n = v.n;
@@ -197,7 +279,7 @@
       Snm = Sm + ys;
       Lym = n;
     }
-    int32_t Dm = MIN_SCORE;
+    RowM st{Sm, MIN_SCORE, sb, Snm, Lym};
     uint32_t cell = cell_make(ib, TB_START, sb);
     v.rowm[0 * 32 + v.pi] = (uint16_t)cell;
     LxN = Lx0;
@@ -236,74 +318,23 @@
         Ti = b.Ti;
       }
       const int32_t q = qv[u];
-      const int32_t m_score = sdiag + v.score(p, q);
-      int32_t best_i, best_d;
-      {
-        const int32_t i_score = iup + ge, s_score = sup + go;
-        if (i_score > s_score) {
-          best_i = i_score;
-          ib = TB_INS;
-        } else {
-          best_i = s_score;
-          ib = LAZY;
-        }
-      }
-      uint32_t db;
-      {
-        const int32_t d_score = Dm + ge, s_score = Sm + go;
-        if (d_score > s_score) {
-          best_d = d_score;
-          db = TB_DEL;
-        } else {
-          best_d = s_score;
-          db = sb;
-        }
-      }
-      int32_t best = Tv;
-      sb = TB_XCLIP_SUFFIX;
-      if (m_score > best) {
-        best = m_score;
-        sb = (p == q) ? TB_MATCH : TB_SUBST;
-      }
-      if (best_i > best) {
-        best = best_i;
-        sb = TB_INS;
-      }
-      if (best_d > best) {
-        best = best_d;
-        sb = TB_DEL;
-      }
-      const int32_t xcs = xclip_score(sc, j);
-      if (xcs > best) {
-        best = xcs;
-        sb = TB_XCLIP_PREFIX;
-      }
-      if (yclip_score > best) {
-        best = yclip_score;
-        sb = TB_YCLIP_PREFIX;
-      }
-      Sm = best;
-      Im = best_i;
-      Dm = best_d;
-      if (Sm + ys > Snm) {
-        Snm = Sm + ys;
-        Lym = n - j;
-      }
+      cell = rowm_cell(sc, n, j, v.score(p, q), p == q, sdiag, sup, iup, Tv, yclip_score, st, Im);
       if (j == n) {
         LxN = m - Ti;
-        if (ib == LAZY) {
-          ib = (m == 1) ? row0_sbits(sc, n, n)
-                        : v.nib_scode((uint32_t)v.row(ROWS_NL, m - 1), m - 1, n);
+        if (cell_i(cell) == LAZY) {
+          cell = cell_set_i(cell, (m == 1) ? row0_sbits(sc, n, n)
+                                           : v.nib_scode((uint32_t)v.row(ROWS_NL, m - 1), m - 1, n));
         }
       }
-      cell = cell_make(ib, db, sb);
       v.rowm[j * 32 + v.pi] = (uint16_t)cell;
       sdiag = sup;
           }
     }
-    SmN = Sm;
+    SmN = st.Sm;
     ImN = Im;
     cmN = cell;
+    Snm = st.Snm;
+    Lym = st.Lym;
   }
 
   const bool ys_live = ys > DEAD_CLIP;
@@ -638,7 +669,8 @@
 template <bool SCORES = false>
 B2A_HD void walk_pair(const PairView& v, const bool filter_clips, uint8_t* ops_end, WalkOut& out) {
   EndState es;
-  finish_matrix_seq(v, es);
+  if (v.finished()) load_end_state(v, es);
+  else finish_matrix_seq(v, es);
   WalkState w;
   walk_begin(v, es, ops_end, w);
   walk_run<SCORES>(v, es, filter_clips, w, 0x7fffffff);
@@ -683,6 +715,10 @@
   using C = Coop<W>;
   const DevScoring& sc = v.sc;
   const int32_t m = v.m, n = v.n;
+  if (v.finished()) {
+    load_end_state(v, es);
+    return;
+  }
   if (m < 2 || n < 1) {
     if (lane == 0) finish_matrix_seq(v, es);
     C::sync();
@@ -1062,7 +1098,7 @@
 }
 
 template <bool SCORES>
-__device__ __forceinline__ void walk_lane(const WalkParams& prm, const Block& blk, const int lane) {
+__device__ __forceinline__ void walk_lane(const WalkParams& prm, const Block& blk, const uint32_t b, const int lane) {
   if ((uint32_t)lane >= blk.npairs) return;
   const uint32_t sp = blk.first + lane;
   const int32_t P = 32 / prm.G;
@@ -1080,6 +1116,7 @@
   v.g = lane % P;
   v.packtrk = prm.packtrk;
   v.bnd8 = prm.bnd8;
+  v.fin = prm.fin ? prm.fin + (size_t)b * FIN_FIELDS * 32 : nullptr;
   v.maxn = (int32_t)blk.maxn;
   v.bnd_base = bnd_index(prm.G, 0, lane, v.maxn);
   v.bnd_stride = (int32_t)(bnd_index(prm.G, 1, lane, v.maxn) - v.bnd_base);
@@ -1099,7 +1136,7 @@
 }
 
 template <bool SCORES>
-__device__ __forceinline__ void walk_warp(const WalkParams& prm, const Block& blk, const int pi, const int lane,
+__device__ __forceinline__ void walk_warp(const WalkParams& prm, const Block& blk, const uint32_t b, const int pi, const int lane,
                                           uint8_t* seq_smem) {
   const uint32_t sp = blk.first + pi;
   const int32_t P = 32 / prm.G;
@@ -1117,6 +1154,7 @@
   v.g = pi % P;
   v.packtrk = prm.packtrk;
   v.bnd8 = prm.bnd8;
+  v.fin = prm.fin ? prm.fin + (size_t)b * FIN_FIELDS * 32 : nullptr;
   v.maxn = (int32_t)blk.maxn;
   v.bnd_base = bnd_index(prm.G, 0, pi, v.maxn);
   v.bnd_stride = (int32_t)(bnd_index(prm.G, 1, pi, v.maxn) - v.bnd_base);
@@ -1157,7 +1195,7 @@
   const Block blk = prm.blocks[b];
   if (pi >= blk.npairs) return;
   uint8_t* mine = prm.seq_smem_per_warp ? walk_smem + (size_t)(threadIdx.x >> 5) * prm.seq_smem_per_warp : nullptr;
-  walk_warp<SCORES>(prm, blk, (int)pi, lane, mine);
+  walk_warp<SCORES>(prm, blk, b, (int)pi, lane, mine);
 }
 
 template <bool SCORES>
@@ -1166,7 +1204,7 @@
   const int lane = threadIdx.x & 31;
   if (gw >= prm.nblocks) return;
   const Block blk = prm.blocks[gw];
-  walk_lane<SCORES>(prm, blk, lane);
+  walk_lane<SCORES>(prm, blk, gw, lane);
 }
 #endif
 
```

New measurement: 852.2, median of 6. 1.08x the previous value.
